# apache/datafusion-comet

Measured on AMD Instinct MI355X. Metric: rows/sec, TPC-H SF100 Q1 scan->filter->agg (HBM-resident Arrow columns), higher is better.
Workload: dtype i128 (Decimal128; 256-bit products) / i32 (Date32) / u8 (Utf8 keys); 1 GPU; TPC-H SF100 Q1 stage 1 (Filter -> Project, 3 decimal ops incl. one 256-bit multiply -> partial HashAggregate, 2 Utf8 keys, 8 aggregates) per GPU; rows_per_gpu=600037902, bytes_per_row_algorithmic=78, parallelism=row-range shards x1, jit_toolchain=hiprtc 9.0; comgr 3.0 /opt/rocm/lib/libamd_comgr.so.3

## Files before the change

### datafusion-comet_amd/csrc/codegen.hpp

```cpp
#pragma once
#include <map>
#include <memory>
#include <string>
#include <vector>

#include "plan.hpp"

namespace comet {

enum class SinkKind { Output, AggNoGroup, AggGrouped };

struct OutCol {
  DType type;
  bool nullable = true;
  bool packed_string = false;
  int gather_src = -1;
  int view_src = -1;
  enum FmtKind { FmtNone = 0, FmtInt = 1, FmtBool = 2, FmtDecimal = 3, FmtDecimalJava = 4, FmtDate = 5, FmtTimestamp = 6, FmtFloat64 = 7, FmtFloat32 = 8 };
  int fmt_kind = FmtNone;
  long long fmt_arg = 0;
  std::vector<int> concat_cols;
  std::vector<std::string> concat_lits;
  int case_mode = 0;
  std::string pad_pattern;
  bool pad_left = false;
};

struct DerivedCol {
  int kind = 0;
  int op = 0;
  std::string arg_a, arg_b;
  long long arg_k = 0;
  int columns() const { return kind == 3 ? 1 : 2; }
  int src = -1;
  std::vector<uint32_t> prog;
  std::vector<uint32_t> prog2;
  int limit = -1;
  DType type;
};

struct PipelineDesc {
  SinkKind sink = SinkKind::Output;
  bool has_filter = false;
  int R = 4;
  int NW = 0;
  int NK = 0;
  int NPW = 0;
  int lds_cap = 0;
  std::vector<DType> in_types;
  std::vector<DerivedCol> derived;
  std::vector<bool> in_used;
  std::vector<OutCol> out_cols;
  std::vector<std::pair<uint32_t, std::shared_ptr<QueryContext>>> site_contexts;
  std::shared_ptr<QueryContext> agg_ctx[2];
  bool agg_ctx_mixed[2] = {false, false}, agg_ctx_seen[2] = {false, false};
  struct BloomRef { ExprP node; int64_t subquery_id = -1; };
  std::vector<BloomRef> blooms;
  std::string source;
  std::vector<std::string> kernels;
  long long max_rows_exact = 0;
  int sort_key_bytes = 0;
  std::vector<int> sort_str_cols;
  bool join_build_only = false;
  bool join_outer_build = false;
  bool join_dedup_build = false;
  std::string explain;
  std::vector<std::string> op_names;
  std::vector<int> str_key_cols;
  struct FixSum { int word = 0; int aux_hi = 0, aux_lo = 0; };
  std::vector<FixSum> fix_sums;
  bool merges_states = false;
};
constexpr int kFixScaleArg = 6;
constexpr int kFixScaleArg2 = 4;
constexpr int kRowBaseArg = 3;
constexpr int kFixMaxSums = 8;
constexpr int kFixW = 158;
constexpr int kFixDefaultScale = -94;

PipelineDesc generate_pipeline(const Operator& root, const std::vector<bool>& in_has_validity,
                               const std::vector<DType>* source_types = nullptr, const std::vector<int>* str_fixed_len = nullptr,
                               const std::vector<int>* dict_id_col = nullptr);

PipelineDesc generate_sort_keys(const Operator& sort, const std::vector<DType>& types, const std::vector<bool>& has_validity);
ExprP bound(int idx, const DType& t);
ExprP shift_bound(const ExprP& e, int by, int from = 0);
struct JoinFusion {
  std::vector<DType> src_types;
  std::vector<bool> src_valid;
  std::vector<ExprP> cols;
  std::vector<ExprP> preds;
};
PipelineDesc generate_join(const Operator& join, const std::vector<DType>& left_types, const std::vector<DType>& right_types,
                           const std::vector<bool>& left_has_validity, const std::vector<bool>& right_has_validity,
                           const JoinFusion* probe_fusion = nullptr, const JoinFusion* build_fusion = nullptr);
void fold_chain(const Operator& top, const Operator& source, const std::vector<DType>& source_types, std::vector<ExprP>& cols, std::vector<ExprP>& preds);

constexpr int kOutPartials = 0;
constexpr int kOutCounts = 1;
constexpr int kOutErr = 2;
constexpr int kErrBytes = 512;
constexpr int kErrAuxWords = 22;
constexpr int kErrDetailWord = 24;
constexpr int kErrDetailStrBytes = 224;

struct ErrSite {
  enum Value : int { Unscaled128 = 0, Int64 = 1, F64 = 2, F32 = 3, Str = 4, DecimalBD = 5, F64Display = 6, Int64Plain = 7, NoValue = 8, F64Micros = 9, FunctionName = 10, IndexAndSize = 11 };
  std::string error_type;
  std::string error_class;
  std::string from_type, to_type;
  int precision = 0, scale = 0;
  int value = Unscaled128;
  std::string suffix;
};
uint32_t register_err_site(const ErrSite& s, int ordinal = 0);
bool lookup_err_site(uint32_t id, ErrSite& out);
std::string err_site_json(const ErrSite& s, uint64_t lo, uint64_t hi, const uint8_t* str, size_t str_avail, const QueryContext* ctx = nullptr);
std::string decimal_sum_overflow_json(int kind, const QueryContext* ctx);
void bloom_check_bytes(const uint8_t* p, size_t len);
constexpr int kOutFirstCol = 4;

}
```

### datafusion-comet_amd/csrc/device/comet_device.hpp

```cpp
#pragma once
#ifndef __HIPCC_RTC__
#include <hip/hip_runtime.h>
#endif
#include "kparams.h"

#ifndef STRFN
#define STRFN __device__ inline
#endif
#include "strfn.hpp"

template <class P>
__device__ bool rx_search(const unsigned int* w, P text, int n, int from, int& m0, int& m1);

namespace comet {

typedef long long i64;
typedef unsigned long long u64;
typedef int i32;
typedef unsigned int u32;
typedef short i16;
typedef unsigned short u16;
typedef signed char i8;
typedef unsigned char u8;
typedef __int128 i128;
// ... 1869 lines not shown

template <int NK, int NPW>
struct LSlot {
  u32 state;
  u32 ord;
  u64 key[NK];
  u64 acc[NPW];
  u64 pad[((1 + NK + NPW) % 2 == 0) ? 1 : 0];
};

template <class P>
struct GroupCtx {
  COMET_LDS LSlot<P::NK, P::NPW>* lds;
  COMET_LDS u32* lds_count;
  COMET_LDS u32* ord_slot;
  COMET_LDS u64* priv;
  Slot<P::NK, P::NW>* glb;
  u64 glb_cap;
  unsigned int* err;
  int part_mode = 0;
  COMET_LDS u32* part = nullptr;
  u64* recs = nullptr;
  u32 np = 0;
  mutable u32 inserted = 0;
  CDEV u32* counter() const { return &inserted; }
  CDEV bool table_full() const { return (__hip_atomic_load(err, __ATOMIC_RELAXED, __HIP_MEMORY_SCOPE_AGENT) & 32u) != 0; }
  CDEV void set_full() const { if (!table_full()) atomicOr(err, 32u); }
};

CDEV void flush_inserted(unsigned int* err, u32 inserted) {
  u32 v = inserted;
#pragma unroll
  for (int m = 32; m >= 1; m >>= 1) v += __shfl_xor(v, m, kWave);
  if (lane_id() == 0 && v) atomicAdd((unsigned long long*)err + 1, (unsigned long long)v);
}
constexpr u64 kMaxGlobalProbes = 128;
constexpr u32 kNoOrdinal = 0xffffffffu;

template <class P>
struct SlotInit {
  CDEV void operator()(u64* acc) const { P::init(acc); }
};

template <class P>
CDEV void lds_word_apply(COMET_LDS u64* w, int k, u64 v) {
  switch (P::pop(k)) {
    case G_ADD64: if (v) __hip_atomic_fetch_add(w, v, __ATOMIC_RELAXED, __HIP_MEMORY_SCOPE_WORKGROUP); break;
    case G_UMAX64: if (v) __hip_atomic_fetch_max(w, v, __ATOMIC_RELAXED, __HIP_MEMORY_SCOPE_WORKGROUP); break;
    case G_OR64: if (v) __hip_atomic_fetch_or(w, v, __ATOMIC_RELAXED, __HIP_MEMORY_SCOPE_WORKGROUP); break;
    case G_AND64: if (~v) __hip_atomic_fetch_and(w, v, __ATOMIC_RELAXED, __HIP_MEMORY_SCOPE_WORKGROUP); break;
    case G_XOR64: if (v) atomic_xor64<__HIP_MEMORY_SCOPE_WORKGROUP>(w, v); break;
    case G_IMIN64: __hip_atomic_fetch_min((COMET_LDS i64*)w, (i64)v, __ATOMIC_RELAXED, __HIP_MEMORY_SCOPE_WORKGROUP); break;
    case G_IMAX64: __hip_atomic_fetch_max((COMET_LDS i64*)w, (i64)v, __ATOMIC_RELAXED, __HIP_MEMORY_SCOPE_WORKGROUP); break;
    case G_FADD64: __hip_atomic_fetch_add((COMET_LDS double*)w, __longlong_as_double((i64)v), __ATOMIC_RELAXED, __HIP_MEMORY_SCOPE_WORKGROUP); break;
    default: break;
  }
}
template <class P>
CDEV u64 pword_combine(int k, u64 a, u64 b) {
  switch (P::pop(k)) {
    case G_ADD64: return a + b;
    case G_UMAX64: return a > b ? a : b;
    case G_OR64: return a | b;
    case G_AND64: return a & b;
    case G_XOR64: return a ^ b;
    case G_IMIN64: return (i64)b < (i64)a ? b : a;
    case G_IMAX64: return (i64)b > (i64)a ? b : a;
    case G_FADD64: return (u64)__double_as_longlong(fp_add(__longlong_as_double((i64)a), __longlong_as_double((i64)b)));
    default: return a;
  }
}

template <class P>
CDEV COMET_LDS LSlot<P::NK, P::NPW>* lds_find_or_insert(const GroupCtx<P>& g, const u64* key, u32& ordinal) {
  typedef COMET_LDS LSlot<P::NK, P::NPW> S;
  u32 h = (u32)hash_key<P::NK>(key) & (u32)(P::LDS_CAP - 1);
  for (int probes = 0; probes < 16;) {
    S* s = g.lds + h;
    u32 st = __hip_atomic_load(&s->state, __ATOMIC_RELAXED, __HIP_MEMORY_SCOPE_WORKGROUP);
    if (st == kSlotEmpty) {
      u32 expected = kSlotEmpty;
      if (__hip_atomic_compare_exchange_strong(&s->state, &expected, kSlotBusy, __ATOMIC_RELAXED, __ATOMIC_RELAXED,
                                               __HIP_MEMORY_SCOPE_WORKGROUP)) {
#pragma unroll
        for (int k = 0; k < P::NK; k++) s->key[k] = key[k];
#pragma unroll
        for (int k = 0; k < P::NPW; k++) s->acc[k] = P::pidentity(k);
        u32 ord = __hip_atomic_fetch_add(g.lds_count, 1u, __ATOMIC_RELAXED, __HIP_MEMORY_SCOPE_WORKGROUP);
        s->ord = ord;
        if (ord < (u32)P::GC) g.ord_slot[ord] = h;
        __hip_atomic_store(&s->state, kSlotReady, __ATOMIC_RELEASE, __HIP_MEMORY_SCOPE_WORKGROUP);
        ordinal = ord;
        return s;
      }
      continue;
    }
    if (st == kSlotBusy) continue;
    bool eq = true;
#pragma unroll
    for (int k = 0; k < P::NK; k++) eq &= (s->key[k] == key[k]);
    if (eq) {
      ordinal = s->ord;
      return s;
    }
    h = (h + 1) & (u32)(P::LDS_CAP - 1);
    probes++;
  }
  ordinal = kNoOrdinal;
  return nullptr;
}

template <class P>
CDEV void group_update(const GroupCtx<P>& g, bool active, const u64* key, const u64* pv) {
  if (!active) return;
  if (g.part_mode) {
    const u32 p = (u32)__umul64hi(hash_key<P::NK>(key), (u64)g.np);
    if (g.part_mode == 1) {
      __hip_atomic_fetch_add(g.part + p, 1u, __ATOMIC_RELAXED, __HIP_MEMORY_SCOPE_WORKGROUP);
      return;
    }
    u64 val[P::NW];
    P::fold(pv, val);
    const u32 pos = __hip_atomic_fetch_add(g.part + p, 1u, __ATOMIC_RELAXED, __HIP_MEMORY_SCOPE_WORKGROUP);
    u64* rec = g.recs + (u64)pos * (u64)(P::NK + P::NW);
#pragma unroll
    for (int k = 0; k < P::NK; k++) rec[k] = key[k];
#pragma unroll
    for (int k = 0; k < P::NW; k++) rec[P::NK + k] = val[k];
    return;
  }
  u32 ord = kNoOrdinal;
  COMET_LDS LSlot<P::NK, P::NPW>* ls = nullptr;
  if (P::LDS_CAP > 0) ls = lds_find_or_insert<P>(g, key, ord);
  if (ord < (u32)P::GC) {
    COMET_LDS u64* base = g.priv + (u32)(ord * P::NPW) * P::COPIES + (threadIdx.x & (P::COPIES - 1));
#pragma unroll
    for (int k = 0; k < P::NPW; k++) lds_word_apply<P>(base + k * P::COPIES, k, pv[k]);
    return;
  }
  if (ls) {
#pragma unroll
    for (int k = 0; k < P::NPW; k++) lds_word_apply<P>(&ls->acc[k], k, pv[k]);
    return;
  }
  if (g.table_full()) return;
  u64 val[P::NW];
  P::fold(pv, val);
  bool fresh = false;
  Slot<P::NK, P::NW>* s = table_find_or_insert<P::NK, P::NW>(g.glb, g.glb_cap, key, SlotInitWith<P>{val}, kMaxGlobalProbes, g.counter(), &fresh);
  if (!s) { g.set_full(); return; }
  if (!fresh) slot_apply<P, __HIP_MEMORY_SCOPE_AGENT>(&s->acc[0], val);
}

template <class P>
CDEV void agg_grouped_body(const CometKParams& prm) {
  typedef Slot<P::NK, P::NW> S;
  typedef LSlot<P::NK, P::NPW> LS;
  __shared__ LS s_tbl[P::LDS_CAP > 0 ? P::LDS_CAP : 1];
  __shared__ u64 s_priv[P::GC * P::NPW * P::COPIES];
  __shared__ u32 s_count;
  __shared__ u32 s_ord_slot[P::GC];
  if (P::LDS_CAP > 0) {
    for (int i = threadIdx.x; i < P::LDS_CAP; i += kBlock) s_tbl[i].state = kSlotEmpty;
  }
  for (int i = threadIdx.x; i < P::GC * P::NPW * P::COPIES; i += kBlock) s_priv[i] = P::pidentity((i / P::COPIES) % P::NPW);
  if (threadIdx.x == 0) s_count = 0;
  __syncthreads();
  GroupCtx<P> g;
  g.lds = (COMET_LDS LS*)s_tbl;
  g.lds_count = (COMET_LDS u32*)&s_count;
  g.ord_slot = (COMET_LDS u32*)s_ord_slot;
  g.priv = (COMET_LDS u64*)s_priv;
  g.glb = (S*)prm.out[0];
  g.glb_cap = (u64)prm.iarg[0];
  g.err = (unsigned int*)prm.out[2];
  u64 kacc[P::NKW > 0 ? P::NKW : 1];
  P::kinit(kacc);
  const i64 n = prm.n;
  const i64 tile = (i64)P::R * kBlock;
  const i64 stride = (i64)gridDim.x * tile;
  if constexpr (P::PIPELINED) {
    typename P::L cur, nxt;
    i64 base = (i64)blockIdx.x * tile;
    if (base < n) P::tile_load(prm, base, n, cur);
    for (u32 it = 0; base < n; base += stride, it++) {
      if (base + stride < n) P::tile_load(prm, base + stride, n, nxt);
      P::tile_grouped(prm, base, n, cur, g, kacc);
      cur = nxt;
      if ((it < 8 || (it & 7) == 7) && g.table_full()) break;
    }
  } else {
    u32 it = 0;
    for (i64 base = (i64)blockIdx.x * tile; base < n; base += stride, it++) {
      P::tile_grouped(prm, base, n, g, kacc);
      if ((it < 8 || (it & 7) == 7) && g.table_full()) break;
    }
  }
  __syncthreads();
  const u32 ngrp = s_count < (u32)P::GC ? s_count : (u32)P::GC;
  for (u32 t = threadIdx.x; t < ngrp * P::NPW; t += kBlock) {
    const u32 gi = t / P::NPW, k = t % P::NPW;
    u64 a = P::pidentity(k);
    for (int c = 0; c < P::COPIES; c++) a = pword_combine<P>(k, a, s_priv[(gi * P::NPW + k) * P::COPIES + c]);
    LS* ls = &s_tbl[s_ord_slot[gi]];
    ls->acc[k] = pword_combine<P>(k, ls->acc[k], a);
  }
  __syncthreads();
  for (int i = threadIdx.x; i < P::LDS_CAP; i += kBlock) {
    LS* ls = &s_tbl[i];
    if (ls->state == kSlotReady) {
      u64 key[P::NK], pw[P::NPW], val[P::NW];
#pragma unroll
      for (int k = 0; k < P::NK; k++) key[k] = ls->key[k];
#pragma unroll
      for (int k = 0; k < P::NPW; k++) pw[k] = ls->acc[k];
      P::fold(pw, val);
      bool fresh = false;
      S* gs = g.table_full() ? nullptr : table_find_or_insert<P::NK, P::NW>(g.glb, g.glb_cap, key, SlotInitWith<P>{val}, kMaxGlobalProbes, g.counter(), &fresh);
      if (!gs) g.set_full();
      else if (!fresh) slot_apply<P, __HIP_MEMORY_SCOPE_AGENT>(&gs->acc[0], val);
    }
  }
  flush_inserted(g.err, g.inserted);
  if (P::NKW > 0) {
#pragma unroll
    for (int m = 32; m >= 1; m >>= 1) {
#pragma unroll
      for (int k = 0; k < P::NKW; k++) {
        u64 o = shfl_xor_u64(kacc[k], m);
        kacc[k] = P::kop(k) == G_UMAX64 ? (o > kacc[k] ? o : kacc[k]) : (kacc[k] | o);
      }
    }
    if (lane_id() == 0) {
      unsigned long long* aux = (unsigned long long*)prm.out[2] + 2;
#pragma unroll
      for (int k = 0; k < P::NKW; k++) {
        if (P::kop(k) == G_UMAX64) atomicMax(aux + k, (unsigned long long)kacc[k]);
        else atomicOr(aux + k, (unsigned long long)kacc[k]);
      }
    }
  }
}


constexpr int kJoinPartMax = 16384;
constexpr int kJoinPartTotOff = kJoinPartMax + 16;
constexpr int kJoinPartCntOff = 2 * kJoinPartMax + 16;
template <class P>
struct AggPart {
  static constexpr int kSlotBytes = 8 + 8 * (P::NK + P::NW);
  static constexpr int kCap = kSlotBytes <= 48 ? 1024 : kSlotBytes <= 96 ? 512 : kSlotBytes <= 192 ? 256 : 128;
};

template <class P>
CDEV void agg_publish_kacc(const CometKParams& prm, u64* kacc) {
  if (P::NKW > 0) {
#pragma unroll
    for (int m = 32; m >= 1; m >>= 1) {
#pragma unroll
      for (int k = 0; k < P::NKW; k++) {
        u64 o = shfl_xor_u64(kacc[k], m);
        kacc[k] = P::kop(k) == G_UMAX64 ? (o > kacc[k] ? o : kacc[k]) : (kacc[k] | o);
      }
    }
    if (lane_id() == 0) {
      unsigned long long* aux = (unsigned long long*)prm.out[2] + 2;
#pragma unroll
      for (int k = 0; k < P::NKW; k++) {
        if (P::kop(k) == G_UMAX64) atomicMax(aux + k, (unsigned long long)kacc[k]);
        else atomicOr(aux + k, (unsigned long long)kacc[k]);
      }
    }
  }
}

template <class P, int MODE>
CDEV void agg_part_pass_body(const CometKParams& prm) {
  __shared__ u32 s_part[kJoinPartMax];
  __shared__ u32 s_wsum[kBlock / kWave];
  __shared__ u32 s_carry;
  const i64 n = prm.n, chunk = prm.iarg[5];
  const int np = (int)prm.iarg[2];
  u32* pstart = (u32*)prm.out[3];
  u32* cnt = pstart + kJoinPartCntOff + (i64)blockIdx.x * np;
  if (MODE == 1) {
    for (int p = threadIdx.x; p < np; p += kBlock) s_part[p] = 0;
  } else {
    const u32* tot = pstart + kJoinPartTotOff;
    if (threadIdx.x == 0) s_carry = 0;
    __syncthreads();
    for (int b0 = 0; b0 < np; b0 += kBlock) {
      const int p = b0 + (int)threadIdx.x;
      const u32 v = p < np ? tot[p] : 0u;
      u32 x = v;
#pragma unroll
      for (int d = 1; d < kWave; d <<= 1) {
        const u32 y = __shfl_up(x, d, kWave);
        if (lane_id() >= d) x += y;
      }
      if (lane_id() == kWave - 1) s_wsum[wave_id()] = x;
      __syncthreads();
      u32 excl = s_carry + x - v;
      for (int w = 0; w < wave_id(); w++) excl += s_wsum[w];
      if (p < np) {
        s_part[p] = excl + cnt[p];
        if (blockIdx.x == 0) pstart[p] = excl;
      }
      __syncthreads();
      if (threadIdx.x == kBlock - 1) s_carry = excl + v;
      __syncthreads();
// ... 1142 lines not shown
```

### datafusion-comet_amd/csrc/exec.cpp

```cpp
#include "exec.hpp"
#include "shuffle_format.hpp"

#include <cerrno>
#include <fcntl.h>
#include <unistd.h>
#include <chrono>
#include <condition_variable>
#include <cstdio>
#include <cstdlib>
#include <cmath>
#include <cstring>
#include <functional>
#include <map>
#include <mutex>

#include "exec_internal.hpp"

namespace comet {

static bool list_of_flat(const DType& t) { return t.id == TypeId::List && t.kids.size() == 1 && !t.kids[0].is_nested(); }
DevTable extend_struct_fields(const DevTable& in) {
  bool any = false;
  for (auto& t : in.types) any |= t.id == TypeId::Struct || list_of_flat(t);
  if (!any) return in;
// ... 652 lines not shown
        btypes.push_back(st[(size_t)col]);
      }
      std::vector<bool> none(st.size(), false), bnone(btypes.size(), true);
      PipelineDesc d1 = generate_sort_keys(so, st, none), d2 = generate_sort_keys(sb, btypes, bnone);
      if (d1.sort_key_bytes != d2.sort_key_bytes) throw CometError("internal: range boundary keys and row keys differ in width");
      if (compile_in_infer_) { jit_compile(d1.source); jit_compile(d2.source); }
    }
    explain_ += "  shuffle writer: " + std::to_string(op.shuffle_num_partitions) + " partition(s), codec " + std::to_string(op.shuffle_codec) + "\n";
    return {};
  }
  if (is_bloom_agg(op)) {
    if (op.children.size() != 1) throw CometError("HashAggregate expects exactly one child");
    const BloomAggSpec spec = bloom_agg_spec(op);
    std::vector<DType> st = infer_schema(*op.children[0]);
    if (op.agg_mode == AggMode::Partial) {
      auto sc = std::make_shared<Operator>();
      sc->kind = OpKind::Scan;
      sc->proto_tag = 100;
      sc->scan_fields = st;
      auto pr = std::make_shared<Operator>();
      pr->kind = OpKind::Projection;
      pr->proto_tag = 101;
      pr->children.push_back(sc);
      pr->project_list = op.agg_exprs[0].children;
      node_id_[pr.get()] = (int)node_id_.size();
      std::vector<DType> ext = extend_struct_field_types(st);
      std::vector<bool> none(ext.size(), false);
      PipelineDesc d = generate_pipeline(*pr, none, &ext);
      const DType& ct = d.out_cols.at(0).type;
      if (ct.id == TypeId::String || ct.id == TypeId::Bytes)
        throw CometError("bloom_filter_agg over a " + ct.str() + " child is not supported by the MI355X native engine: might_contain probes longs only, such a filter could not be used natively");
      if (!ct.is_integer()) throw CometError("bloom_filter_agg over " + ct.str() + " is not supported (Byte, Short, Int and Long are)");
      if (compile_in_infer_) jit_compile(d.source);
      explain_ += d.explain;
      bloom_proj_[&op] = pr;
    } else {
      const size_t sc = (size_t)std::max(0, op.initial_input_buffer_offset);
      if (sc >= st.size() || st[sc].id != TypeId::Bytes)
        throw CometError("bloom_filter_agg: the merging aggregate expects its Binary state in column " + std::to_string(sc) + " of its child");
    }
    explain_ += std::string("  bloom_filter_agg (") + (op.agg_mode == AggMode::Partial ? "Partial" : op.agg_mode == AggMode::Final ? "Final" : "PartialMerge") + "): V" +
                std::to_string(spec.version) + ", " + std::to_string(spec.k) + " hash function(s), " + std::to_string(spec.num_words * 64) + " bits\n";
    return {DType::of(TypeId::Bytes)};
  }
  if (op.kind == OpKind::NativeScan) {
    std::vector<DType> out;
    for (auto& f : op.required_schema) out.push_back(f.dtype);
    for (auto& f : op.partition_schema) out.push_back(f.dtype);
    explain_ += "  parquet scan: " + std::to_string(op.files.size()) + " file(s), " + std::to_string(out.size()) + " column(s)\n";
    return out;
  }
  if (op.kind == OpKind::HashJoin) {
    if (op.children.size() != 2) throw CometError("HashJoin expects two children");
    const size_t pi = op.build_side == BuildSide::Left ? 1 : 0;
    std::vector<DType> l, r;
    PipelineDesc d;
    bool fused = false;
    if (pi == 1) {
      l = infer_schema(*op.children[0]);
      fused = plan_fused_probe(op, l, d);
      if (!fused) r = infer_schema(*op.children[1]);
    } else {
      const std::string before = explain_;
      explain_.clear();
      r = infer_schema(*op.children[1]);
      const std::string right_explain = explain_;
      explain_ = before;
      fused = plan_fused_probe(op, r, d);
      if (!fused) l = infer_schema(*op.children[0]);
      explain_ += right_explain;
    }
    if (!fused) {
      std::vector<bool> lv(l.size(), false), rv(r.size(), false);
      FusedProbe fb;
      bool with_build = plan_fused_build(op, fb);
      if (with_build) {
        try {
          d = generate_join(op, l, r, lv, rv, nullptr, &fb.fu);
          fused_build_[&op] = fb;
        } catch (const CometError&) {
          with_build = false;
        }
      }
      if (!with_build) d = generate_join(op, l, r, lv, rv);
    }
    if (compile_in_infer_) jit_compile(d.source);
    explain_ += d.explain;
    if (fused) {
      const size_t nbuild = pi == 1 ? l.size() : r.size();
      std::vector<DType> probe_types;
      const size_t nprobe = fused_probe_.at(&op).fu.cols.size();
      if (d.out_cols.size() == nbuild + nprobe) {
        for (size_t c = 0; c < nprobe; c++) probe_types.push_back(d.out_cols[(pi == 1 ? nbuild : 0) + c].type);
      } else {
        probe_types.assign(nprobe, DType());
        if (pi == 0) for (size_t c = 0; c < nprobe && c < d.out_cols.size(); c++) probe_types[c] = d.out_cols[c].type;
      }
      (pi == 1 ? r : l) = probe_types;
    }
    if (op.smj) {
      Operator& so = *smj_sorts_.at(&op);
      so.sort_orders.clear();
      const bool by_right = op.join_type == JoinType::RightOuter;
      const std::vector<ExprP>& keys = by_right ? op.right_keys : op.left_keys;
      std::function<ExprP(const ExprP&)> shift = [&](const ExprP& e) -> ExprP {
        auto n = std::make_shared<Expr>(*e);
        if (e->kind == ExprKind::Bound) n->bound_index = e->bound_index + (int)l.size();
        for (auto& c : n->children) c = shift(c);
        return n;
      };
      for (size_t k = 0; k < keys.size(); k++) {
        Operator::SortKey sk;
        sk.child = by_right ? shift(keys[k]) : keys[k];
        if (k < op.smj_sort_options.size()) { sk.descending = op.smj_sort_options[k].first; sk.nulls_last = op.smj_sort_options[k].second; }
        so.sort_orders.push_back(sk);
      }
      explain_ += "  (sort-merge join: output ordered by the join keys)\n";
    }
    std::vector<DType> out;
    for (auto& c : d.out_cols) out.push_back(c.type);
    return out;
  }
  const Operator* src = &op;
  do {
    if (src->children.size() != 1) throw CometError(std::string(op_name(src->proto_tag)) + " expects exactly one child");
    src = src->children[0].get();
  } while (!is_source(*src, &op));
  std::vector<DType> st = extend_struct_field_types(infer_schema(*src));
  std::vector<bool> none(st.size(), false);
  PipelineDesc d = generate_pipeline(op, none, &st);
  if (compile_in_infer_) jit_compile(d.source);
  explain_ += d.explain;
  std::vector<DType> out;
  for (auto& c : d.out_cols) { out.push_back(c.type); out.back().virt_parent = out.back().virt_kid = -1; }
  return out;
}

ExecutionContext::~ExecutionContext() {
  mem_->owner = std::this_thread::get_id();
  for (auto& in : inputs_) {
    if (in.host && in.host->release) in.host->release(in.host);
    if (in.dev && in.dev->release) in.dev->release(in.dev);
  }
  for (auto& st : staging_)
    if (st && st->busy) {
      (void)hipEventSynchronize(st->busy);
      pool_put_event(device_id_, st->busy);
      st->busy = nullptr;
    }
  if (stream_) {
    (void)hipStreamSynchronize(stream_);
    for (auto& pr : timed_) { pool_put_event(device_id_, pr.first); pool_put_event(device_id_, pr.second); }
    for (hipEvent_t& e : aux_ev_) if (e) { pool_put_event(device_id_, e); e = nullptr; }
    for (auto& p : kt_pending_) { pool_put_event(device_id_, p.a); pool_put_event(device_id_, p.b); }
    kt_pending_.clear();
    pool_put_stream(device_id_, stream_);
  }
}

const std::string& ExecutionContext::explain() { return explain_; }

std::string ExecutionContext::check_only(OperatorP plan, uint64_t plan_hash) {
  size_t nscan = 0;
  std::function<void(const Operator&)> cnt = [&](const Operator& op) {
    if (op.kind == OpKind::Scan) nscan++;
    for (auto& c : op.children) cnt(*c);
  };
  cnt(*plan);
  std::vector<InputSource> ins(nscan);
  ExecutionContext ctx(plan, plan_hash, {}, ins, 8192, 0);
  return ctx.explain_;
}

PipelineDesc ExecutionContext::join_codegen(OperatorP plan, uint64_t plan_hash, const std::vector<bool>& has_valid) {
  const Operator& op = *plan;
  const Operator* leaf[2] = {nullptr, nullptr};
  for (size_t s = 0; s < 2 && op.kind == OpKind::HashJoin && op.children.size() == 2; s++) {
    const Operator* c = op.children[s].get();
    while ((c->kind == OpKind::Filter || c->kind == OpKind::Projection) && c->children.size() == 1) c = c->children[0].get();
    if (c->kind == OpKind::Scan) leaf[s] = c;
  }
  if (!leaf[0] || !leaf[1]) throw CometError("comet_plan_codegen: a HashJoin over two Scan leaves, or Filter / Projection chains over them, is expected");
  std::vector<InputSource> ins(2);
  ExecutionContext ctx(plan, plan_hash, {}, ins, 8192, 0);
  auto fit = ctx.fused_probe_.find(&op);
  auto fbit = ctx.fused_build_.find(&op);
  const bool build_left = op.build_side == BuildSide::Left;
  std::vector<DType> types[2];
  std::vector<bool> valid[2];
  size_t first = 0;
  for (size_t s = 0; s < 2; s++) {
    std::vector<bool> hv(leaf[s]->scan_fields.size(), false);
    for (size_t k = 0; k < hv.size(); k++) hv[k] = first + k < has_valid.size() && has_valid[first + k];
    first += hv.size();
    const bool is_build = (s == 0) == build_left;
    const bool fused = is_build ? fbit != ctx.fused_build_.end() : fit != ctx.fused_probe_.end();
    if (fused || op.children[s].get() == leaf[s]) {
      types[s] = leaf[s]->scan_fields;
      valid[s] = hv;
    } else {
      const PipelineDesc cd = generate_pipeline(*op.children[s], hv);
      for (auto& oc : cd.out_cols) {
        types[s].push_back(oc.type);
        valid[s].push_back(oc.nullable);
      }
    }
  }
  JoinFusion fu, fub;
  if (fit != ctx.fused_probe_.end()) { fu = fit->second.fu; fu.src_valid = valid[build_left ? 1 : 0]; }
  if (fbit != ctx.fused_build_.end()) { fub = fbit->second.fu; fub.src_valid = valid[build_left ? 0 : 1]; }
  return generate_join(op, types[0], types[1], valid[0], valid[1], fit != ctx.fused_probe_.end() ? &fu : nullptr, fbit != ctx.fused_build_.end() ? &fub : nullptr);
}

std::string ExecutionContext::compile_only(OperatorP plan, uint64_t plan_hash) {
  size_t nscan = 0;
  std::function<void(const Operator&)> cnt = [&](const Operator& op) {
    if (op.kind == OpKind::Scan) nscan++;
    for (auto& c : op.children) cnt(*c);
  };
  cnt(*plan);
  std::vector<InputSource> ins(nscan);
  ExecutionContext ctx(plan, plan_hash, {}, ins, 8192, 0);
  std::vector<bool> none(ctx.in_types_.size(), false);
  if (ctx.has_join_) {
    ctx.compile_in_infer_ = true;
    ctx.explain_.clear();
    ctx.infer_schema(*ctx.root_source_);
    if (ctx.plan_.get() != ctx.root_source_) {
      auto pv = planned_variant(*ctx.plan_, ctx.plan_hash_, none, true, &ctx.in_types_);
      ctx.explain_ += pv->desc.explain;
    }
  } else {
    planned_variant(*ctx.plan_, ctx.plan_hash_, none, true);
  }
  return ctx.explain_;
}

Variant ExecutionContext::node_variant(const Operator& node, const char* tag, const std::string& validity, const std::function<PipelineDesc()>& generate) {
  const std::string key = std::to_string(plan_hash_ ^ (0x9E3779B97F4A7C15ull * (uint64_t)(node_id_[&node] + 1))) + tag + validity;
  std::shared_ptr<PlannedVariant> pv;
  {
    std::lock_guard<std::mutex> lk(g_plan_mu);
    auto it = g_plan_cache.find(key);
    if (it != g_plan_cache.end()) pv = it->second;
  }
  if (!pv) {
    pv = std::make_shared<PlannedVariant>();
    pv->desc = generate();
    pv->code = jit_compile(pv->desc.source);
    std::lock_guard<std::mutex> lk(g_plan_mu);
    g_plan_cache[key] = pv;
  }
  Variant v;
  v.desc = pv->desc;
  note_sites(v.desc);
  v.mod = jit_load(pv->code);
  return v;
}

Variant& ExecutionContext::variant_for(const std::vector<bool>& has_valid, const std::vector<int>& str_fixed_len) {
  std::string key = validity_key(has_valid) + ":";
  bool any_fixed = false;
  for (int l : str_fixed_len) { key += std::to_string(l) + ","; any_fixed |= l >= 0; }
  auto it = variants_.find(key);
  if (it != variants_.end()) return it->second;
  auto pv = planned_variant(*plan_, plan_hash_, has_valid, true, has_join_ ? &in_types_ : nullptr, any_fixed ? &str_fixed_len : nullptr,
                            dict_id_col_.empty() ? nullptr : &dict_id_col_);
  Variant v;
  v.desc = pv->desc;
  note_sites(v.desc);
  v.mod = jit_load(pv->code);
  auto res = variants_.emplace(key, std::move(v));
  return res.first->second;
}

void ExecutionContext::launch(Variant& v, const char* kernel, int grid, CometKParams& prm, int block) {
  hipFunction_t fn = v.mod->fn(kernel);
  if (!v.desc.blooms.empty()) bind_blooms(v.desc, prm);
  void* args[] = {&prm};
  if (!g_kernel_times.load(std::memory_order_relaxed)) {
    HIP_CHECK(hipModuleLaunchKernel(fn, (unsigned)grid, 1, 1, (unsigned)block, 1, 1, 0, stream_, args, nullptr));
    return;
  }
  hipEvent_t a = pool_get_event(device_id_), b = pool_get_event(device_id_);
  HIP_CHECK(hipEventRecord(a, stream_));
  HIP_CHECK(hipModuleLaunchKernel(fn, (unsigned)grid, 1, 1, (unsigned)block, 1, 1, 0, stream_, args, nullptr));
  HIP_CHECK(hipEventRecord(b, stream_));
  kt_pending_.push_back({kernel, a, b});
}

std::atomic<int> g_kernel_times{getenv("COMET_KERNEL_TIMES") != nullptr && atoi(getenv("COMET_KERNEL_TIMES")) != 0 ? 1 : 0};

std::string ExecutionContext::kernel_times_json() {
  if (!kt_pending_.empty()) {
    HIP_CHECK(hipStreamSynchronize(stream_));
    for (auto& p : kt_pending_) {
      float ms = 0;
      if (hipEventElapsedTime(&ms, p.a, p.b) == hipSuccess) { kernel_times_[p.name].first += ms; kernel_times_[p.name].second++; }
      pool_put_event(device_id_, p.a);
      pool_put_event(device_id_, p.b);
    }
    kt_pending_.clear();
  }
  std::string s = "{";
  for (auto& kv : kernel_times_) {
    char buf[160];
// ... 384 lines not shown

void ExecutionContext::extend_derived(DevTable& in, const std::vector<DerivedCol>& derived) {
  for (const DerivedCol& dc : derived) {
    if (dc.kind == 3) { extend_derived_strfn(in, dc); continue; }
    if ((dc.kind != 1 && dc.kind != 2) || dc.src < 0 || (size_t)dc.src >= in.cols.size()) throw CometError("internal: unknown derived column");
    const DeviceColumnView sc = in.cols[(size_t)dc.src];
    const bool hv = in.has_valid[(size_t)dc.src];
    const int64_t rows = in.rows;
    if (!sc.data && rows) throw CometError("split over a Utf8 column without offsets is not supported");
    if (hv && sc.offset != 0) throw CometError("split over a sliced Utf8 column with NULLs is not supported yet");
    DevBuf prog, counts, tiles;
    auto list_offs = std::make_shared<DevBuf>();
    prog.ensure(dc.prog.size() * 4 + 16);
    HIP_CHECK(hipMemcpyAsync(prog.p, dc.prog.data(), dc.prog.size() * 4, hipMemcpyHostToDevice, stream_));
    DevBuf prog_group;
    const uint32_t* prog2 = nullptr;
    if (dc.kind == 2) {
      if (dc.prog2.empty()) prog2 = (const uint32_t*)prog.p;
      else {
        prog_group.ensure(dc.prog2.size() * 4 + 16);
        HIP_CHECK(hipMemcpyAsync(prog_group.p, dc.prog2.data(), dc.prog2.size() * 4, hipMemcpyHostToDevice, stream_));
        prog2 = (const uint32_t*)prog_group.p;
      }
    }
    HIP_CHECK(hipStreamSynchronize(stream_));
    counts.ensure((size_t)std::max<int64_t>(rows, 1) * 4 + 16);
    tiles.ensure((size_t)((rows + 1023) / 1024 + 2) * 8);
    list_offs->ensure((size_t)(rows + 2) * 4);
    HIP_CHECK(hipMemsetAsync(list_offs->p, 0, 8, stream_));
    const int32_t* offs = (const int32_t*)sc.data + sc.offset;
    const uint8_t* vbits = hv ? sc.valid : nullptr;
    if (comet_launch_split_count(offs, (const uint8_t*)sc.aux, vbits, sc.offset, rows, (const uint32_t*)prog.p, prog2, dc.limit, (uint32_t*)counts.p, stream_) != 0) throw CometError("split: launch failed");
    if (rows) pq_launch_u32_scan((const uint32_t*)counts.p, rows, (uint64_t*)tiles.p, (int32_t*)list_offs->p, stream_);
    int32_t total = 0;
    if (rows) read_small(&total, (char*)list_offs->p + (size_t)rows * 4, 4);
    if (total < 0) throw CometError("split: more than 2^31 pieces in one table");
    DevBuf views, lengths, etiles;
    auto eoffs = std::make_shared<DevBuf>(), ebytes = std::make_shared<DevBuf>();
    views.ensure((size_t)std::max<int32_t>(total, 1) * 16 + 16);
    lengths.ensure((size_t)std::max<int32_t>(total, 1) * 4 + 16);
    etiles.ensure((size_t)((total + 1023) / 1024 + 2) * 8);
    eoffs->ensure((size_t)(total + 2) * 4);
    HIP_CHECK(hipMemsetAsync(eoffs->p, 0, 8, stream_));
    if (comet_launch_split_write(offs, (const uint8_t*)sc.aux, vbits, sc.offset, rows, (const uint32_t*)prog.p, prog2, dc.limit, (const int32_t*)list_offs->p, views.p, stream_) != 0)
      throw CometError("split: launch failed");
    if (comet_launch_strview_lengths(views.p, nullptr, total, nullptr, 0, (uint32_t*)lengths.p, stream_) != 0) throw CometError("split: launch failed");
    if (total) pq_launch_u32_scan((const uint32_t*)lengths.p, total, (uint64_t*)etiles.p, (int32_t*)eoffs->p, stream_);
    int32_t nbytes = 0;
    if (total) read_small(&nbytes, (char*)eoffs->p + (size_t)total * 4, 4);
    if (nbytes < 0) throw CometError("Utf8 column exceeds 2 GiB of string data (LargeUtf8 is not supported)");
    ebytes->ensure((size_t)nbytes + 16);
    if (comet_launch_strview_copy(views.p, nullptr, offs, (const uint8_t*)sc.aux, total, nullptr, 0, 0, (const int32_t*)eoffs->p, (uint8_t*)ebytes->p, stream_) != 0)
      throw CometError("split: launch failed");
    HIP_CHECK(hipStreamSynchronize(stream_));
    DeviceColumnView elem;
    elem.data = eoffs->p;
    elem.aux = ebytes->p;
    DeviceColumnView lv;
    lv.data = list_offs->p;
    lv.valid = sc.valid;
    lv.offset = 0;
    lv.kids.push_back(elem);
    lv.kid_has_valid.push_back(false);
    lv.kid_rows = total;
    in.types.push_back(dc.type);
    in.cols.push_back(lv);
    in.has_valid.push_back(hv);
    DType et = dc.type.kids[0];
    et.virt_parent = (int)in.types.size() - 1;
    et.virt_kid = 0;
    in.types.push_back(et);
    in.cols.push_back(elem);
    in.has_valid.push_back(false);
    in.owners.push_back(list_offs);
    in.owners.push_back(eoffs);
    in.owners.push_back(ebytes);
    split_rows_ += rows;
  }
}


DevTable ExecutionContext::run_chain_to_device(const Operator& top, const DevTable& in_plain) {
  DevTable in = extend_struct_fields(in_plain);
  if (in.cols.size() > COMET_MAX_IN) throw CometError("too many columns (struct fields included) for one GPU pipeline");
  auto pv = planned_variant(top, plan_hash_ ^ (0x9E3779B97F4A7C15ull * (uint64_t)(node_id_[&top] + 1)), in.has_valid, true, &in.types);
  if (pv->desc.sink != SinkKind::Output) throw CometError("internal: run_chain_to_device on an aggregate chain");
  extend_derived(in, pv->desc.derived);
  if (in.cols.size() > COMET_MAX_IN) throw CometError("too many columns (derived columns included) for one GPU pipeline");
  Variant v;
  v.desc = pv->desc;
  note_sites(v.desc);
  v.mod = jit_load(pv->code);
  const PipelineDesc& d = v.desc;
  const int64_t n = in.rows;
  CometKParams prm;
  memset(&prm, 0, sizeof prm);
  prm.n = n;
  bind_inputs(prm, in.cols, in.has_valid);
  prm.out[kOutErr] = err_flags_.p;
  const size_t ncol = d.out_cols.size();
  std::vector<std::shared_ptr<DevBuf>> vals(ncol), vbytes(ncol);
  auto bind = [&](int64_t cap) {
    for (size_t j = 0; j < ncol; j++) {
      vals[j] = std::make_shared<DevBuf>();
      vals[j]->ensure((size_t)cap * out_width(d.out_cols[j]) + 16);
      prm.out[kOutFirstCol + 2 * j] = vals[j]->p;
      vbytes[j] = std::make_shared<DevBuf>();
      if (d.out_cols[j].nullable) {
        vbytes[j]->ensure((size_t)cap + 16);
        prm.out[kOutFirstCol + 2 * j + 1] = vbytes[j]->p;
      }
    }
  };
  int64_t out_rows = n;
  timed_begin();
  if (n == 0) {
    bind(1);
    out_rows = 0;
  } else if (d.has_filter) {
    bind(n);
    out_rows = launch_fused_filter(v, prm, n);
  } else {
    bind(n);
    launch(v, "k_emit", (int)std::min<int64_t>((n + 255) / 256, 256 * 8), prm);
  }
  timed_end();
  DevTable out = outputs_to_table(v, vals, vbytes, out_rows, [&](int c) { return std::make_pair(&in, c); });
  out.owners.push_back(v.mod);
  return out;
}

DevTable ExecutionContext::materialize(const Operator& op) {
  static const bool trace = getenv("COMET_TRACE_STAGES") != nullptr;
  Timer tm;
  struct Report {
    const Operator& op; Timer& tm; bool on;
    ~Report() { if (on) fprintf(stderr, "[comet] materialize %s: %.3f ms (incl. children)\n", op_name(op.proto_tag), tm.ns() / 1e6); }
  } report{op, tm, trace};
  if (op.kind == OpKind::Scan) {
    const size_t input = scan_input_.at(&op);
    DevTable t;
    t.types = op.scan_fields;
    if (inputs_[input].kind == 0) {
      int64_t rows = 0;
      if (pull_host_table(input, op.scan_fields, INT64_MAX, t.cols, t.has_valid, rows)) t.rows = rows;
      if (t.cols.empty()) {
        t.cols.assign(op.scan_fields.size(), DeviceColumnView());
        t.has_valid.assign(op.scan_fields.size(), false);
      }
      HIP_CHECK(hipStreamSynchronize(stream_));
    } else {
      std::shared_ptr<void> keep;
      int64_t rows = 0;
      if (pull_device_table(input, op.scan_fields, t.cols, t.has_valid, rows, keep)) {
        t.rows = rows;
        t.owners.push_back(keep);
        std::vector<DeviceColumnView> c2;
        std::vector<bool> v2;
        std::shared_ptr<void> k2;
        int64_t r2 = 0;
        if (pull_device_table(input, op.scan_fields, c2, v2, r2, k2) && r2 > 0)
          throw CometError("a device input stream feeding a join must deliver a single batch");
      } else {
        t.cols.assign(op.scan_fields.size(), DeviceColumnView());
        t.has_valid.assign(op.scan_fields.size(), false);
      }
    }
    input_rows += t.rows;
    return t;
  }
  if (op.kind == OpKind::NativeScan) {
    DevTable t = scan_parquet(op);
    input_rows += t.rows;
    return t;
  }
  if (op.kind == OpKind::HashJoin) {
    auto fit = fused_probe_.find(&op);
    auto fbit = fused_build_.find(&op);
    DevTable j;
    if (fit != fused_probe_.end() || fbit != fused_build_.end()) {
      const bool build_left = op.build_side == BuildSide::Left;
      const bool fb_on = fbit != fused_build_.end(), fp_on = fit != fused_probe_.end();
      DevTable b = materialize(fb_on ? *fbit->second.source : *op.children[build_left ? 0 : 1]);
      DevTable s = materialize(fp_on ? *fit->second.source : *op.children[build_left ? 1 : 0]);
      JoinFusion fu, fub;
      if (fp_on) { fu = fit->second.fu; fu.src_valid = s.has_valid; }
      if (fb_on) { fub = fbit->second.fu; fub.src_valid = b.has_valid; join_fused_builds_++; }
      const char* sfx = fp_on && fb_on ? ":FB" : fp_on ? ":F" : ":B";
      j = build_left ? hash_join_impl(op, op, b, s, sfx, fp_on ? &fu : nullptr, fb_on ? &fub : nullptr) : hash_join_impl(op, op, s, b, sfx, fp_on ? &fu : nullptr, fb_on ? &fub : nullptr);
    } else {
      DevTable l = materialize(*op.children[0]);
      DevTable r = materialize(*op.children[1]);
      j = hash_join(op, l, r);
    }
    if (!op.smj || !smj_needs_sort_.count(&op)) return j;
    return sort_table(*smj_sorts_.at(&op), j);
  }
  if (op.kind == OpKind::Sort) {
    DevTable in = materialize(*op.children[0]);
    return sort_table(op, in);
  }
  if (op.kind == OpKind::Limit) {
    DevTable in = materialize(*op.children[0]);
    const int64_t off = std::min<int64_t>(std::max(0, op.offset), in.rows);
    const int64_t end = op.limit < 0 ? in.rows : std::min<int64_t>(in.rows, op.limit);
    return take_rows(in, nullptr, off, std::max<int64_t>(0, end - off), nullptr);
  }
  if (op.kind == OpKind::ShuffleWriter) return write_shuffle(op);
  if (op.kind == OpKind::Expand) {
    DevTable in = materialize(*op.children[0]);
    return expand(op, in);
  }
  if (op.kind == OpKind::Explode) {
    DevTable in = materialize(*op.children[0]);
    return explode(op, in);
  }
  if (op.kind == OpKind::Window) {
    DevTable in = materialize(*op.children[0]);
    return window(op, in);
  }
  if (is_bloom_agg(op)) {
    DevTable in = materialize(*op.children[0]);
    return bloom_aggregate(op, in);
  }
  if (op.kind == OpKind::HashAgg) return nested_aggregate(op);
  const Operator* src = &op;
  do src = src->children[0].get(); while (!is_source(*src, &op));
  DevTable in = materialize(*src);
  DevTable out = run_chain_to_device(op, in);
  HIP_CHECK(hipStreamSynchronize(stream_));
  return out;
}



DevTable ExecutionContext::nested_aggregate(const Operator& agg) {
  std::vector<size_t> idx;
  std::function<void(const Operator&)> walk = [&](const Operator& op) {
    if (op.kind == OpKind::Scan) idx.push_back(scan_input_.at(&op));
    for (auto& c : op.children) walk(*c);
  };
  walk(agg);
  std::vector<InputSource> sub_inputs;
  for (size_t i : idx) {
    sub_inputs.push_back(inputs_[i]);
    inputs_[i].host = nullptr;
    inputs_[i].dev = nullptr;
    inputs_[i].exhausted = true;
  }
  OperatorP sub_plan(const_cast<Operator*>(&agg), [](Operator*) {});
  static const bool trace = getenv("COMET_TRACE_STAGES") != nullptr;
  Timer tm;
  auto mark = [&](const char* what) { if (trace) fprintf(stderr, "[comet] nested aggregate: %s at %.3f ms\n", what, tm.ns() / 1e6); };
  auto subp = std::make_unique<ExecutionContext>(sub_plan, plan_hash_ ^ (0x9E3779B97F4A7C15ull * (uint64_t)(node_id_[&agg] + 1)), config_, sub_inputs, 0, device_id_);
  ExecutionContext& sub = *subp;
  struct Gone { std::unique_ptr<ExecutionContext>& p; decltype(mark)& m; ~Gone() { p.reset(); m("context released"); } } gone{subp, mark};
  mark("context built");
  if (sub.sink_ != SinkKind::AggGrouped && sub.sink_ != SinkKind::AggNoGroup) throw CometError("internal: nested aggregate without an aggregate sink");
  sub.device_result_ = true;
  sub.blooms_ = blooms_;
  sub.start();
  mark("started");
  sub.run_to_completion();
  mark("input consumed");
  DevTable t;
  if (sub.sink_ == SinkKind::AggNoGroup) {
    sub.finish_aggregate();
    if (sub.ready_.empty()) throw CometError("internal: ungrouped aggregate produced no row");
    t = host_batch_to_table(sub.ready_.front());
    sub.ready_.clear();
  } else {
    t = sub.grouped_to_device();
  }
  mark("groups emitted");
  input_rows += sub.input_rows;
  part_merges_ += sub.part_merges_;
  sub.collect_timings();
  last_kernel_ms += sub.last_kernel_ms;
  last_kernel_launches += sub.last_kernel_launches;
  if (!sub.kt_pending_.empty() || !sub.kernel_times_.empty()) {
    sub.kernel_times_json();
    for (auto& kv : sub.kernel_times_) { kernel_times_[kv.first].first += kv.second.first; kernel_times_[kv.first].second += kv.second.second; }
  }
  return t;
}

DevTable ExecutionContext::host_batch_to_table(const HostBatch& b) {
  DevTable t;
  t.rows = b.rows;
  auto up = [&](const std::vector<uint8_t>& v) -> const void* {
    auto d = std::make_shared<DevBuf>();
    d->ensure(v.size() + 16);
    if (!v.empty()) HIP_CHECK(hipMemcpy(d->p, v.data(), v.size(), hipMemcpyHostToDevice));
    t.owners.push_back(d);
    return d->p;
  };
  for (const HostColumn& c : b.cols) {
    DeviceColumnView v;
    v.data = up(c.values);
    const bool is_str = c.type.id == TypeId::String || c.type.id == TypeId::Bytes;
    if (is_str) v.aux = up(c.data);
    const bool hv = c.null_count > 0 && !c.validity.empty();
    if (hv) v.valid = (const uint8_t*)up(c.validity);
    t.types.push_back(c.type);
    t.cols.push_back(v);
    t.has_valid.push_back(hv);
  }
// ... 28 lines not shown
  } else if (t.id == TypeId::Bool) {
    fetch(c.values, v.data, (size_t)((rows + 7) / 8));
  } else {
    fetch(c.values, v.data, (size_t)rows * (size_t)fixed_width(t));
  }
  HIP_CHECK(hipStreamSynchronize(st));
  if (!c.validity.empty()) {
    int64_t nulls = 0;
    for (int64_t i = 0; i < rows; i++) nulls += !((c.validity[(size_t)(i >> 3)] >> (i & 7)) & 1);
    c.null_count = nulls;
    if (!nulls) c.validity.clear();
  }
  return c;
}
namespace {
std::vector<uint8_t> slice_bits(const std::vector<uint8_t>& b, int64_t off, int64_t len) {
  std::vector<uint8_t> o((size_t)((len + 7) / 8), 0);
  for (int64_t i = 0; i < len; i++)
    if ((b[(size_t)((off + i) >> 3)] >> ((off + i) & 7)) & 1) o[(size_t)(i >> 3)] |= (uint8_t)(1u << (i & 7));
  return o;
}
HostColumn slice_column(const HostColumn& c, int64_t off, int64_t len) {
  if (off == 0 && len == c.length) return c;
  HostColumn o;
  o.type = c.type;
  o.length = len;
  if (!c.validity.empty()) {
    o.validity = slice_bits(c.validity, off, len);
    for (int64_t i = 0; i < len; i++) o.null_count += !((o.validity[(size_t)(i >> 3)] >> (i & 7)) & 1);
    if (!o.null_count) o.validity.clear();
  }
  const TypeId id = c.type.id;
  if (id == TypeId::Struct) {
    for (auto& k : c.children) o.children.push_back(slice_column(k, off, len));
  } else if (id == TypeId::List || id == TypeId::Map || id == TypeId::String || id == TypeId::Bytes) {
    const int32_t* src = (const int32_t*)c.values.data();
    o.values.resize((size_t)(len + 1) * 4);
    int32_t* w = (int32_t*)o.values.data();
    for (int64_t i = 0; i <= len; i++) w[i] = src[off + i] - src[off];
    if (id == TypeId::List || id == TypeId::Map) o.children.push_back(slice_column(c.children.at(0), src[off], src[off + len] - src[off]));
    else o.data.assign(c.data.begin() + src[off], c.data.begin() + src[off + len]);
  } else if (id == TypeId::Bool) {
    o.values = slice_bits(c.values, off, len);
  } else {
    const size_t w = (size_t)fixed_width(c.type);
    o.values.assign(c.values.begin() + (size_t)off * w, c.values.begin() + (size_t)(off + len) * w);
  }
  return o;
}
}

void ExecutionContext::table_to_host_batches(const DevTable& t) {
  if (t.rows == 0) return;
  const size_t ncol = t.cols.size();
  std::vector<HostColumn> nested(ncol);
  for (size_t j = 0; j < ncol; j++)
    if (t.types[j].is_nested()) nested[j] = download_column(t.cols[j], t.types[j], t.has_valid[j], t.rows, stream_);
  std::vector<std::vector<uint8_t>> hv(ncol), hb(ncol);
  std::vector<std::vector<uint8_t>> hd(ncol);
  struct Piece { const void* src; std::vector<uint8_t>* dst; size_t bytes; };
  auto fetch = [&](std::vector<Piece>& pieces) {
    size_t total = 0, longest = 0;
    for (auto& pc : pieces) { pc.dst->resize(pc.bytes); total += (pc.bytes + 15) & ~(size_t)15; longest = std::max(longest, pc.bytes); }
    if (pieces.empty()) return;
    static const bool batched = getenv("COMET_EXPORT_BATCHED") == nullptr || atoi(getenv("COMET_EXPORT_BATCHED")) != 0;
    if (batched && total > 0 && total <= ((size_t)1 << 20) && pieces.size() <= 256) {
      struct Desc { const uint8_t* src; uint8_t* dst; uint64_t len; };
      const size_t head = (pieces.size() * sizeof(Desc) + 63) & ~(size_t)63;
      export_host_.ensure(head + total + 64);
      Desc* d = (Desc*)export_host_.p;
      size_t at = head;
      for (size_t k = 0; k < pieces.size(); k++) {
        d[k].src = (const uint8_t*)pieces[k].src;
        d[k].dst = (uint8_t*)export_host_.p + at;
        d[k].len = pieces[k].bytes;
        at += (pieces[k].bytes + 15) & ~(size_t)15;
      }
      if (comet_launch_copy_small(export_host_.p, (int)pieces.size(), (uint64_t)longest, stream_) != 0) throw CometError("result export: launch failed");
      HIP_CHECK(hipStreamSynchronize(stream_));
      for (size_t k = 0; k < pieces.size(); k++)
        if (pieces[k].bytes) memcpy(pieces[k].dst->data(), d[k].dst, pieces[k].bytes);
      return;
    }
    for (auto& pc : pieces)
      if (pc.bytes) HIP_CHECK(hipMemcpyAsync(pc.dst->data(), pc.src, pc.bytes, hipMemcpyDeviceToHost, stream_));
    HIP_CHECK(hipStreamSynchronize(stream_));
  };
  std::vector<Piece> pieces;
  for (size_t j = 0; j < ncol; j++) {
    const DType& ty = t.types[j];
    if (ty.is_nested()) continue;
    const bool is_str = ty.id == TypeId::String || ty.id == TypeId::Bytes;
    size_t bytes = is_str ? (size_t)(t.rows + 1) * 4 : ty.id == TypeId::Bool ? (size_t)((t.rows + 7) / 8) : (size_t)t.rows * fixed_width(ty);
    pieces.push_back({t.cols[j].data, &hv[j], bytes});
    if (t.has_valid[j]) pieces.push_back({t.cols[j].valid, &hb[j], (size_t)((t.rows + 7) / 8)});
  }
  fetch(pieces);
  pieces.clear();
  for (size_t j = 0; j < ncol; j++) {
    if (t.types[j].id == TypeId::String || t.types[j].id == TypeId::Bytes) {
      const int32_t* offs = (const int32_t*)hv[j].data();
      if (offs[t.rows] > 0) pieces.push_back({t.cols[j].aux, &hd[j], (size_t)offs[t.rows]});
    }
  }
  fetch(pieces);
  check_device_errors();
  const int64_t bs = batch_size_ > 0 ? batch_size_ : t.rows;
  auto getbit = [](const std::vector<uint8_t>& b, int64_t i) { return (b[(size_t)(i >> 3)] >> (i & 7)) & 1; };
  for (int64_t off = 0; off < t.rows; off += bs) {
    const int64_t len = std::min(bs, t.rows - off);
    HostBatch b;
    b.rows = len;
    for (size_t j = 0; j < ncol; j++) {
      if (t.types[j].is_nested()) { b.cols.push_back(slice_column(nested[j], off, len)); continue; }
      HostColumn c;
      c.type = t.types[j];
      c.length = len;
      if (c.type.id == TypeId::String || c.type.id == TypeId::Bytes) {
        const int32_t* offs = (const int32_t*)hv[j].data();
        c.values.resize((size_t)(len + 1) * 4);
        int32_t* o = (int32_t*)c.values.data();
        for (int64_t i = 0; i <= len; i++) o[i] = offs[off + i] - offs[off];
        c.data.assign(hd[j].begin() + offs[off], hd[j].begin() + offs[off + len]);
      } else if (c.type.id == TypeId::Bool) {
        c.values.assign((size_t)((len + 7) / 8), 0);
        for (int64_t i = 0; i < len; i++)
          if (getbit(hv[j], off + i)) c.values[(size_t)(i >> 3)] |= (uint8_t)(1u << (i & 7));
      } else {
        int w = fixed_width(c.type);
        c.values.assign(hv[j].begin() + (size_t)off * w, hv[j].begin() + (size_t)(off + len) * w);
      }
      if (t.has_valid[j]) {
        int64_t nulls = 0;
        std::vector<uint8_t> bm((size_t)((len + 7) / 8), 0);
        for (int64_t i = 0; i < len; i++) {
          if (getbit(hb[j], off + i)) bm[(size_t)(i >> 3)] |= (uint8_t)(1u << (i & 7));
          else nulls++;
        }
        c.null_count = nulls;
        if (nulls) c.validity = std::move(bm);
      }
      b.cols.push_back(std::move(c));
    }
    ready_.push_back(std::move(b));
  }
}

void ExecutionContext::run_to_completion() {
  if (has_join_) {
    DevTable src = extend_struct_fields(materialize(*root_source_));
    if (plan_.get() == root_source_) throw CometError("internal: bare join root");
    if (sink_ == SinkKind::AggGrouped) prepare_dict_keys(src);
    single_chunk_hint_ = true;
    process_chunk(src.cols, src.has_valid, src.rows);
    HIP_CHECK(hipStreamSynchronize(stream_));
    return;
  }
  while (true) {
    bool more = inputs_[0].kind == 0 ? pull_host_chunk() : pull_device_batch();
    if (!more) break;
  }
}

void ExecutionContext::start() {
  if (!started_) {
    HIP_CHECK(hipSetDevice(device_id_));
    stream_ = pool_get_stream(device_id_);
    err_flags_.ensure(kErrBytes);
    HIP_CHECK(hipMemsetAsync(err_flags_.p, 0, kErrBytes, stream_));
    started_ = true;
  } else {
    HIP_CHECK(hipSetDevice(device_id_));
  }
}

namespace {
struct ExportedDeviceColumn {
  std::vector<std::shared_ptr<void>> owners;
  const void* buffers[3];
};
void release_device_array(ArrowArray* a) {
  delete (ExportedDeviceColumn*)a->private_data;
  a->release = nullptr;
}
void release_fmt_schema(ArrowSchema* s) {
  delete (std::string*)s->private_data;
  s->release = nullptr;
}
}

void ExecutionContext::set_memory_manager(int64_t (*acquire)(void*, int64_t), void (*release)(void*, int64_t), void* ctx, long long task_id) {
  mem_->acquire = acquire;
  mem_->release = release;
  mem_->ctx = ctx;
  mem_->task_id = task_id;
}
void ExecutionContext::memory_stats(int64_t out[4]) {
  out[0] = mem_->host_used.load();
  out[1] = mem_->host_peak.load();
  out[2] = mem_->dev_used.load();
  out[3] = mem_->dev_peak.load();
}

int64_t ExecutionContext::execute_device(ArrowDeviceArray** out_arrays, ArrowSchema** out_schemas, int n_out) {
  mem_->owner = std::this_thread::get_id();
  AccountScope account(mem_);
  mem_->flush();
  Timer t;
  start();
  if (sink_ == SinkKind::AggNoGroup)
    throw CometError("comet_execute_plan_device: an ungrouped aggregate result is one row and is exported through comet_execute_plan");
  if (finished_) return -1;
  DevTable tab;
  if (sink_ == SinkKind::AggGrouped) {
    device_result_ = true;
    run_to_completion();
    tab = grouped_to_device();
  } else {
    tab = materialize(*plan_);
  }
  HIP_CHECK(hipStreamSynchronize(stream_));
  check_device_errors();
  collect_timings();
  finished_ = true;
  if ((size_t)n_out != tab.cols.size())
    throw CometError("Output column count mismatch: expected " + std::to_string(n_out) + ", got " + std::to_string(tab.cols.size()));
  for (size_t c = 0; c < tab.types.size(); c++)
    if (tab.types[c].is_nested()) throw CometError("executePlan (device arrays): nested column of type " + tab.types[c].str() + " — nested results are exported through host batches");
  for (int j = 0; j < n_out; j++) {
    const DType& ty = tab.types[(size_t)j];
    const bool is_str = ty.id == TypeId::String || ty.id == TypeId::Bytes;
    if (tab.cols[(size_t)j].offset != 0) throw CometError("comet_execute_plan_device: input column with a non-zero Arrow offset passed through");
    auto* ec = new ExportedDeviceColumn();
    ec->owners = tab.owners;
    ec->buffers[0] = tab.has_valid[(size_t)j] ? tab.cols[(size_t)j].valid : nullptr;
    ec->buffers[1] = tab.cols[(size_t)j].data;
    ec->buffers[2] = is_str ? tab.cols[(size_t)j].aux : nullptr;
    ArrowDeviceArray* d = out_arrays[j];
    memset(d, 0, sizeof *d);
    d->array.length = tab.rows;
    d->array.null_count = tab.has_valid[(size_t)j] ? -1 : 0;
    d->array.n_buffers = is_str ? 3 : 2;
    d->array.buffers = ec->buffers;
    d->array.private_data = ec;
    d->array.release = release_device_array;
    d->device_id = device_id_;
    d->device_type = ARROW_DEVICE_ROCM;
    d->sync_event = nullptr;
    ArrowSchema* s = out_schemas[j];
    memset(s, 0, sizeof *s);
    auto* fmt = new std::string(expected_format(ty));
    s->format = fmt->c_str();
    s->name = "";
    s->flags = ARROW_FLAG_NULLABLE;
    s->private_data = fmt;
    s->release = release_fmt_schema;
  }
  output_rows_ += tab.rows;
  elapsed_compute_ns_ += t.ns();
  return tab.rows;
}

void ExecutionContext::resolve_subqueries() {
  if (subqueries_resolved_) return;
  subqueries_resolved_ = true;
  uint64_t sig = 0xcbf29ce484222325ull;
  auto mix = [&](const void* p, size_t n) { for (size_t k = 0; k < n; k++) sig = (sig ^ ((const uint8_t*)p)[k]) * 0x100000001b3ull; };
  for (auto& e : plan_->subqueries) {
    if (e->kind != ExprKind::Subquery) continue;
    const int64_t id = e->lit_i64;
    bool is_null = true;
    std::string v;
    bool found = false;
    auto it = subquery_values_.find(id);
    if (it != subquery_values_.end()) { is_null = it->second.first; v = it->second.second; found = true; }
    else if (subquery_provider_) found = subquery_provider_(id, e->dtype, is_null, v);
    if (!found) throw CometError("Subquery " + std::to_string(id) + " is not registered with this plan (CometScalarSubquery.setSubquery / comet_plan_set_subquery)");
    auto need = [&](size_t n) { if (!is_null && v.size() < n) throw CometError("Subquery " + std::to_string(id) + ": the value has " + std::to_string(v.size()) + " bytes, its type needs " + std::to_string(n)); };
    e->kind = ExprKind::Literal;
    e->proto_tag = 2;
    e->lit_null = is_null;
    e->lit_i64 = 0;
    int64_t i = 0;
    double d = 0;
    switch (e->dtype.id) {
      case TypeId::Bool: need(1); e->lit_bool = !is_null && v[0] != 0; e->lit_case = 1; break;
      case TypeId::Int8: case TypeId::Int16: case TypeId::Int32: case TypeId::Date: case TypeId::Int64: case TypeId::Timestamp: case TypeId::TimestampNtz:
        need(8);
        if (!is_null) memcpy(&i, v.data(), 8);
        e->lit_i64 = i;
        e->lit_case = e->dtype.id == TypeId::Int8 ? 2 : e->dtype.id == TypeId::Int16 ? 3 : (e->dtype.id == TypeId::Int32 || e->dtype.id == TypeId::Date) ? 4 : 5;
        break;
      case TypeId::Float: case TypeId::Double:
        need(8);
        if (!is_null) memcpy(&d, v.data(), 8);
        e->lit_f64 = e->dtype.id == TypeId::Float ? (double)(float)d : d;
        e->lit_case = e->dtype.id == TypeId::Float ? 6 : 7;
        break;
      case TypeId::Decimal: e->lit_dec = is_null ? 0 : decode_decimal_be(v); e->lit_case = 10; break;
      case TypeId::String: case TypeId::Bytes: e->lit_bytes = is_null ? std::string() : v; e->lit_case = e->dtype.id == TypeId::String ? 8 : 9; break;
      default: throw CometError("Unsupported scalar subquery data type " + e->dtype.str());
    }
    mix(&id, 8);
    mix(&is_null, 1);
    if (e->bloom_arg) {
      if (e->dtype.id != TypeId::Bytes) throw CometError("might_contain: the bloom filter subquery must be Binary, got " + e->dtype.str());
      if (!is_null) bloom_check_bytes((const uint8_t*)e->lit_bytes.data(), e->lit_bytes.size());
      if (!blooms_) blooms_ = std::make_shared<BloomRegistry>();
      blooms_->subquery_nodes[id] = e;
      continue;
    }
    mix(v.data(), v.size());
  }
  if (!plan_->subqueries.empty()) plan_hash_ ^= sig * 0x9E3779B97F4A7C15ull;
}

int64_t ExecutionContext::execute(ArrowArray** out_arrays, ArrowSchema** out_schemas, int n_out) {
  mem_->owner = std::this_thread::get_id();
  if (!subqueries_resolved_) resolve_subqueries();
  AccountScope account(mem_);
  mem_->flush();
// ... 73 lines not shown
```

### datafusion-comet_amd/csrc/exec.hpp

```cpp
#pragma once
#include <mutex>
#include <thread>
#include <atomic>
#include <hip/hip_runtime_api.h>

#include <deque>
#include <functional>
#include <map>
#include <set>
#include <memory>
#include <string>
#include <vector>

#include "arrow_abi.hpp"
#include "codegen.hpp"
#include "jit.hpp"
#include "kparams.h"
#include "plan.hpp"

namespace comet {
double process_clock_ms();

struct MemAccount {
  int64_t (*acquire)(void* ctx, int64_t bytes) = nullptr;
  void (*release)(void* ctx, int64_t bytes) = nullptr;
  void* ctx = nullptr;
  long long task_id = 0;
  int64_t dev_limit = 0;
  std::atomic<int64_t> host_used{0}, host_peak{0}, dev_used{0}, dev_peak{0}, pending_release{0};
  std::thread::id owner;
  void grow_host(int64_t n);
  void shrink_host(int64_t n);
  void grow_dev(int64_t n);
  void shrink_dev(int64_t n);
  void flush();
  void detach();
  std::mutex cb_mu;
  bool detached = false;
};
struct AccountScope {
  std::shared_ptr<MemAccount> prev;
  explicit AccountScope(std::shared_ptr<MemAccount> a);
  ~AccountScope();
};

struct DevBuf {
  void* p = nullptr;
  size_t cap = 0;
  int dev = 0;
  std::shared_ptr<MemAccount> acct;
  void ensure(size_t n);
  void release();
  ~DevBuf() { release(); }
  DevBuf() = default;
  DevBuf(const DevBuf&) = delete;
  DevBuf& operator=(const DevBuf&) = delete;
};
struct PinnedBuf {
  void* p = nullptr;
  size_t cap = 0;
  std::shared_ptr<MemAccount> acct;
  void ensure(size_t n);
  void release();
  ~PinnedBuf() { release(); }
  PinnedBuf() = default;
  PinnedBuf(const PinnedBuf&) = delete;
  PinnedBuf& operator=(const PinnedBuf&) = delete;
};

struct HostColumn {
  DType type;
  int64_t length = 0;
  int64_t null_count = 0;
  std::vector<uint8_t> validity;
  std::vector<uint8_t> values;
  std::vector<uint8_t> data;
  std::vector<HostColumn> children;
};
struct HostBatch {
  int64_t rows = 0;
  std::vector<HostColumn> cols;
};

struct InputSource {
  int kind = 0;
  ArrowArrayStream* host = nullptr;
  ArrowDeviceArrayStream* dev = nullptr;
  bool exhausted = false;
};

struct DeviceColumnView {
  const void* data = nullptr;
  const uint8_t* valid = nullptr;
  const void* aux = nullptr;
  int64_t offset = 0;
  int fixed_len = -1;
  std::vector<DeviceColumnView> kids;
  std::vector<char> kid_has_valid;
  int64_t kid_rows = 0;
};

struct DevTable {
  int64_t rows = 0;
  std::vector<DType> types;
  std::vector<DeviceColumnView> cols;
  std::vector<bool> has_valid;
  std::vector<std::shared_ptr<void>> owners;
};

struct Staging {
  std::vector<std::unique_ptr<PinnedBuf>> stage_vals, stage_valid, stage_aux;
  std::vector<std::unique_ptr<DevBuf>> dev_vals, dev_valid, dev_aux;
  std::vector<int> dict_index_width;
  std::vector<std::shared_ptr<void>> nested_keep;
  hipEvent_t busy = nullptr;
};

struct Variant {
  PipelineDesc desc;
  std::shared_ptr<LoadedModule> mod;
};

struct BloomAggSpec { int version = 1, k = 1; int64_t num_words = 0; };
BloomAggSpec bloom_agg_spec(const Operator& hash_agg);
bool is_bloom_agg(const Operator& op);
struct BloomRegistry {
  std::map<int64_t, ExprP> subquery_nodes;
  std::map<const Expr*, std::shared_ptr<struct DevBuf>> buffers;
  std::vector<ExprP> keep;
};

void scan_pool_parallel(size_t n, const std::function<void(size_t)>& fn);
std::string parquet_prune_report(const Operator& native_scan, bool page_index, bool bloom_filters = true);
std::vector<uint8_t> parquet_host_plain_values(const Operator& native_scan, size_t column);
void scan_pool_submit(std::function<void()> fn);

extern std::atomic<int> g_kernel_times;

class ExecutionContext {
 public:
  ExecutionContext(OperatorP plan, uint64_t plan_hash, std::vector<std::pair<std::string, std::string>> config,
                   std::vector<InputSource> inputs, int batch_size, int device_id);
  ~ExecutionContext();

  int64_t execute(ArrowArray** out_arrays, ArrowSchema** out_schemas, int n_out);
  int64_t execute_device(ArrowDeviceArray** out_arrays, ArrowSchema** out_schemas, int n_out);
  std::string metrics_proto();
  void set_memory_manager(int64_t (*acquire)(void*, int64_t), void (*release)(void*, int64_t), void* ctx, long long task_id);
  typedef std::function<bool(int64_t id, const DType& type, bool& is_null, std::string& value)> SubqueryProvider;
  void set_subquery_provider(SubqueryProvider p) { subquery_provider_ = std::move(p); }
  void set_subquery_value(int64_t id, bool is_null, std::string value) { subquery_values_[id] = {is_null, std::move(value)}; }
  void resolve_subqueries();
  void memory_stats(int64_t out[4]);
  std::shared_ptr<MemAccount> memory_account() const { return mem_; }
  const std::string& explain();
  static std::string compile_only(OperatorP plan, uint64_t plan_hash);
  static std::string check_only(OperatorP plan, uint64_t plan_hash);
  static PipelineDesc join_codegen(OperatorP plan, uint64_t plan_hash, const std::vector<bool>& has_valid);

  std::string last_error;
  int last_error_kind = 0;

  double last_kernel_ms = 0;
  int64_t last_kernel_launches = 0;
  std::string kernel_times_json();
  double last_aux_ms = 0;
  int64_t last_aux_launches = 0;
  int64_t input_rows = 0;

 private:
  void run_to_completion();
  void start();
  std::vector<std::vector<int>> fixed_len_hint_;
  Variant& variant_for(const std::vector<bool>& has_valid, const std::vector<int>& str_fixed_len);
  void process_chunk(const std::vector<DeviceColumnView>& cols, const std::vector<bool>& has_valid, int64_t n);
  void finish_aggregate();
  void finish_grouped();
  DevTable grouped_to_device();
  std::vector<DType> infer_schema(const Operator& op);
  DevTable materialize(const Operator& op);
  DevTable scan_parquet(const Operator& native_scan);
  friend struct ParquetScan;
  friend struct HashJoinRun;
  int64_t launch_fused_filter(Variant& v, CometKParams& prm, int64_t n);
  DevTable run_chain_to_device(const Operator& top, const DevTable& in);
  void extend_derived(DevTable& in, const std::vector<DerivedCol>& derived);
  void extend_derived_strfn(DevTable& in, const DerivedCol& dc);
  DevTable hash_join(const Operator& j, const DevTable& l, const DevTable& r);
  DevTable hash_join_impl(const Operator& node, const Operator& j, const DevTable& l, const DevTable& r, const std::string& key_suffix,
                          const JoinFusion* fused_probe = nullptr, const JoinFusion* fused_build = nullptr);
  struct FusedProbe { const Operator* source = nullptr; JoinFusion fu; };
  bool plan_fused_probe(const Operator& join, const std::vector<DType>& build_types, PipelineDesc& desc);
  bool plan_fused_build(const Operator& join, FusedProbe& fb);
  DevTable sort_table(const Operator& s, const DevTable& in);
  Variant node_variant(const Operator& node, const char* tag, const std::string& validity, const std::function<PipelineDesc()>& generate);
  std::shared_ptr<DevBuf> sort_key_planes(const Operator& s, const DevTable& in, int& W, std::vector<int64_t>* str_len = nullptr, bool measure_only = false);
  DevTable literal_table(const std::vector<std::vector<ExprP>>& rows, const std::vector<DType>& types);
  DevTable take_rows(const DevTable& in, const uint32_t* dev_perm, int64_t first, int64_t rows, std::shared_ptr<DevBuf> perm_owner);
  DevTable nested_aggregate(const Operator& agg);
  DevTable write_shuffle(const Operator& sw);
  DevTable expand(const Operator& ex, const DevTable& in);
  DevTable explode(const Operator& ex, const DevTable& in);
  DevTable window(const Operator& w, const DevTable& in);
  DevTable bloom_aggregate(const Operator& agg, const DevTable& in);
  const void* bloom_buffer(const PipelineDesc::BloomRef& ref);
  void bind_blooms(const PipelineDesc& d, CometKParams& prm);
  void prepare_dict_keys(DevTable& src);
  static bool is_source(const Operator& op, const Operator* chain_top);
  typedef std::function<std::pair<const DevTable*, int>(int)> GatherSource;
  DevTable outputs_to_table(Variant& v, const std::vector<std::shared_ptr<DevBuf>>& vals, const std::vector<std::shared_ptr<DevBuf>>& valid_bytes,
                            int64_t rows, const GatherSource& gather_source = nullptr);
  DeviceColumnView take_column(const DeviceColumnView& src, const DType& t, bool has_valid, const uint32_t* idx, const uint8_t* ok_bytes, int64_t rows, bool& out_has_valid,
                               std::vector<std::shared_ptr<void>>& owners);
  void take_utf8(const DeviceColumnView& src, const uint32_t* idx, const uint8_t* ok_bytes, const uint8_t* src_valid_bits, int64_t rows,
                 DeviceColumnView& out, std::vector<std::shared_ptr<void>>& owners);
  void table_to_host_batches(const DevTable& t);
  DevTable host_batch_to_table(const HostBatch& b);
  bool pull_host_chunk();
  bool pull_device_batch();
  bool pull_host_table(size_t input, const std::vector<DType>& types, int64_t max_rows, std::vector<DeviceColumnView>& views,
                       std::vector<bool>& has_valid, int64_t& rows);
  bool pull_device_table(size_t input, const std::vector<DType>& types, std::vector<DeviceColumnView>& views, std::vector<bool>& has_valid,
                         int64_t& rows, std::shared_ptr<void>& keepalive);
  void validate_input_schema(size_t input, const std::vector<DType>& types);
  void export_batch(HostBatch& b, ArrowArray** out_arrays, ArrowSchema** out_schemas, int n_out);
  void check_device_errors();
  void raise_device_errors(uint32_t flags);
  void note_sites(const PipelineDesc& d) {
    site_ctx_last_.clear();
    for (auto& kv : d.site_contexts) {
      site_ctx_last_[kv.first] = kv.second;
      auto it = site_ctx_.find(kv.first);
      if (it == site_ctx_.end()) site_ctx_[kv.first] = kv.second;
      else if (it->second != kv.second && !(it->second && kv.second && it->second->sql_text == kv.second->sql_text && it->second->start_index == kv.second->start_index &&
                                            it->second->stop_index == kv.second->stop_index))
        site_ctx_ambiguous_.insert(kv.first);
    }
    for (int k = 0; k < 2; k++) if (d.agg_ctx[k]) agg_ctx_[k] = d.agg_ctx[k];
  }
  const QueryContext* site_context(uint32_t id) const {
    auto a = site_ctx_last_.find(id);
    if (a != site_ctx_last_.end()) return a->second.get();
    if (site_ctx_ambiguous_.count(id)) return nullptr;
    auto b = site_ctx_.find(id);
    return b == site_ctx_.end() ? nullptr : b->second.get();
  }
  std::map<uint32_t, std::shared_ptr<QueryContext>> site_ctx_last_;
  std::set<uint32_t> site_ctx_ambiguous_;
  std::shared_ptr<QueryContext> agg_ctx_[2];
  std::map<uint32_t, std::shared_ptr<QueryContext>> site_ctx_;
  void read_small(void* dst, const void* dev_src, size_t n);
  void write_small(void* dev_dst, const void* src, size_t n);
  void timed_begin();
  void timed_end();
  void collect_timings();
  void launch(Variant& v, const char* kernel, int grid, CometKParams& prm, int block = 256);

  OperatorP plan_;
  uint64_t plan_hash_ = 0;
  std::vector<std::pair<std::string, std::string>> config_;
  std::vector<InputSource> inputs_;
  int batch_size_;
  int device_id_;
  int64_t chunk_rows_;
  hipStream_t stream_ = nullptr;
  std::vector<std::pair<hipEvent_t, hipEvent_t>> timed_;
  size_t timed_done_ = 0;
  struct KtPending { std::string name; hipEvent_t a, b; };
  std::vector<KtPending> kt_pending_;
  std::map<std::string, std::pair<double, int64_t>> kernel_times_;
  hipEvent_t aux_ev_[2] = {nullptr, nullptr};
  int aux_n_ = 0;
  bool started_ = false, finished_ = false;
  std::vector<DType> in_types_;
  std::map<std::string, Variant> variants_;
  Variant* agg_variant_ = nullptr;
  std::string explain_;
  SinkKind sink_ = SinkKind::Output;
  bool has_join_ = false;
  SubqueryProvider subquery_provider_;
  std::map<int64_t, std::pair<bool, std::string>> subquery_values_;
  bool subqueries_resolved_ = false;
  int64_t strfn_rows_ = 0;
  int64_t split_rows_ = 0;
  bool materialize_root_ = false;
  bool compile_in_infer_ = false;
  std::vector<const Operator*> nested_aggs_;
  struct ExpandPart {
    OperatorP proj;
    std::vector<int> out_col;
    std::vector<int> null_cols;
  };
  struct ExpandInfo {
    std::vector<ExpandPart> parts;
    std::vector<OutCol> out_cols;
  };
  std::map<const Operator*, ExpandInfo> expand_info_;
  std::map<const Operator*, OperatorP> bloom_proj_;
  std::shared_ptr<BloomRegistry> blooms_;
  std::map<const Operator*, OperatorP> explode_proj_;
  std::map<const Operator*, OperatorP> window_psort_, window_osort_;
  std::map<const Operator*, OperatorP> range_sort_, range_bsort_;
  std::shared_ptr<void> planes_owner_;
  std::map<const Operator*, OperatorP> shuffle_projs_;
  int64_t shuffle_bytes_written_ = 0, shuffle_data_size_ = 0, shuffle_staged_peak_ = 0;
  double shuffle_repart_ns_ = 0, shuffle_write_ns_ = 0;
  std::vector<int> dict_id_col_;
  bool device_result_ = false;
  DevTable dict_src_;
  std::map<const Operator*, FusedProbe> fused_probe_;
  std::map<const Operator*, FusedProbe> fused_build_;
  int64_t ramp_rows_ = 0;
  bool fuse_probe_ = true;
  int fuse_build_ = 1;
  std::set<const Operator*> smj_needs_sort_;
  std::map<const Operator*, OperatorP> smj_sorts_;
  const Operator* root_source_ = nullptr;
  std::map<const Operator*, int> node_id_;
  std::map<const Operator*, size_t> scan_input_;
  int64_t join_build_rows_ = 0, join_probe_rows_ = 0, join_keymap_bytes_ = 0, join_direct_maps_ = 0, join_bucket_tables_ = 0, join_bitmap_only_ = 0, join_mono_tables_ = 0, join_fused_builds_ = 0;
  int small_write_slot_ = 0;
  bool single_chunk_hint_ = false, part_result_ready_ = false;
  DevTable part_result_;
  int64_t part_merges_ = 0;
  bool try_partitioned_merge(Variant& v, CometKParams& prm, int64_t n);
  struct DevPending {
    std::vector<DeviceColumnView> views;
    std::vector<bool> has_valid;
    int64_t rows = 0;
    std::shared_ptr<void> keep;
    bool valid = false;
  };
  DevPending dev_pending_;
  bool dev_stream_done_ = false;
  int64_t dev_chunks_seen_ = 0;
  int64_t bytes_scanned_ = 0;
  int64_t row_groups_pruned_ = 0;
  int64_t row_groups_pruned_bloom_ = 0;
  std::shared_ptr<MemAccount> mem_ = std::make_shared<MemAccount>();
  int64_t rows_pruned_page_index_ = 0;
  int64_t pages_inflated_on_device_ = 0;

  std::vector<std::unique_ptr<Staging>> staging_;
  int stage_parity_ = 0;
  std::vector<bool> schema_checked_;
  std::vector<std::vector<std::string>> scan_cast_from_;

  DevBuf partials_;
  int64_t n_partials_ = 0;
  int64_t agg_rows_seen_ = 0;
  std::vector<int> fix_scales_;
  bool fix_has_state_ = false;
  int fix_attempts_ = 0;
  uint64_t groups_committed_ = 0;
  long long packed_fix_scales(const PipelineDesc& d, int first = 0);
  bool adjust_fix_scales(const PipelineDesc& d, const uint64_t* aux, std::vector<int>& shift_right);
  DevBuf err_flags_;
  PinnedBuf result_host_;
  PinnedBuf small_host_;
  PinnedBuf export_host_;
  DevBuf group_table_, group_backup_;
  int64_t group_cap_ = 0;
  bool group_table_clear_ = false;
  DevBuf scratch_mask_, scratch_counts_;
  std::vector<std::unique_ptr<DevBuf>> out_vals_, out_valid_;
  DevBuf emit_arena_;

  std::deque<HostBatch> ready_;
  int64_t output_rows_ = 0;
  double elapsed_compute_ns_ = 0;
};

}
```

### datafusion-comet_amd/csrc/exec_input.cpp

```cpp
#include "exec_internal.hpp"
#include <emmintrin.h>
#include <mutex>
#include <set>
#include <tuple>

namespace comet {

static void stream_copy(void* dst, const void* src, size_t n) {
  char* d = (char*)dst;
  const char* s = (const char*)src;
  if (n < 4096) { memcpy(d, s, n); return; }
  const size_t head = (size_t)(-(intptr_t)d) & 15;
  if (head) { memcpy(d, s, head); d += head; s += head; n -= head; }
  size_t blocks = n / 64;
  for (; blocks; blocks--, d += 64, s += 64) {
    const __m128i a = _mm_loadu_si128((const __m128i*)s), b = _mm_loadu_si128((const __m128i*)(s + 16)), c = _mm_loadu_si128((const __m128i*)(s + 32)),
                  e = _mm_loadu_si128((const __m128i*)(s + 48));
    _mm_stream_si128((__m128i*)d, a);
    _mm_stream_si128((__m128i*)(d + 16), b);
    _mm_stream_si128((__m128i*)(d + 32), c);
    _mm_stream_si128((__m128i*)(d + 48), e);
  }
  _mm_sfence();
  if (n & 63) memcpy(d, s, n & 63);
}

void ExecutionContext::validate_input_schema(size_t input, const std::vector<DType>& types) {
  if (schema_checked_.size() <= input) schema_checked_.resize(input + 1, false);
  if (schema_checked_[input]) return;
  InputSource& in = inputs_[input];
  ArrowSchema sch;
  memset(&sch, 0, sizeof sch);
  int rc = in.kind == 0 ? in.host->get_schema(in.host, &sch) : in.dev->get_schema(in.dev, &sch);
  if (rc != 0 || !sch.release) throw CometError("input stream: get_schema failed");
  std::string err;
  if (in.kind == 1 && (size_t)sch.n_children == types.size()) {
    if (fixed_len_hint_.size() <= input) fixed_len_hint_.resize(input + 1);
    fixed_len_hint_[input].assign(types.size(), -1);
    for (size_t c = 0; c < types.size(); c++) {
      const char* md = sch.children[c]->metadata;
      if (!md || types[c].id != TypeId::String) continue;
      int32_t npairs;
      memcpy(&npairs, md, 4);
      const char* q = md + 4;
      for (int32_t k = 0; k < npairs && k < 4096; k++) {
        int32_t kl, vl;
        memcpy(&kl, q, 4);
        if (kl < 0 || kl > (1 << 20)) break;
        const char* key = q + 4;
        memcpy(&vl, key + kl, 4);
        if (vl < 0 || vl > (1 << 24)) break;
        const char* val = key + kl + 4;
        if (kl == 20 && !memcmp(key, "comet:utf8_fixed_len", 20) && vl > 0 && vl < 4) {
          const int L = atoi(std::string(val, (size_t)vl).c_str());
          if (L >= 0 && L <= 15) fixed_len_hint_[input][c] = L;
        }
        q = val + vl;
      }
    }
  }
  if ((size_t)sch.n_children != types.size()) {
    err = "Scan declares " + std::to_string(types.size()) + " field(s) but the input stream has " + std::to_string(sch.n_children);
  } else {
    for (size_t c = 0; c < types.size() && err.empty(); c++) {
      const ArrowSchema* f = sch.children[c];
      const char* fmt = f->dictionary ? f->dictionary->format : f->format;
      if (types[c].is_nested()) {
        if (in.kind == 0 && nested_schema_matches(f, types[c])) continue;
        err = "Scan input column " + std::to_string(c) + " (Arrow format '" + (fmt ? fmt : "?") + "') does not match the declared " + types[c].str() +
              (in.kind == 0 ? " field by field (nested input columns are not cast)" : ": nested columns of device-resident inputs are not supported");
        break;
      }
      if (format_matches(fmt, types[c])) continue;
      if (in.kind == 0 && !f->dictionary && scan_cast_supported(parse_src_format(fmt), types[c])) {
        if (scan_cast_from_.size() <= input) scan_cast_from_.resize(input + 1);
        scan_cast_from_[input].resize(types.size());
        scan_cast_from_[input][c] = fmt;
        continue;
      }
      err = "Scan input column " + std::to_string(c) + " has Arrow format '" + (fmt ? fmt : "?") + "' but the plan declares " + types[c].str() +
            " (this cast of a scan input is not supported by the MI355X native engine" + (in.kind == 0 ? ")" : "; device-resident inputs are never cast)");
    }
  }
  sch.release(&sch);
  if (!err.empty()) throw CometError(err);
  schema_checked_[input] = true;
}

bool ExecutionContext::pull_host_table(size_t input, const std::vector<DType>& in_types_, int64_t max_rows,
                                       std::vector<DeviceColumnView>& views, std::vector<bool>& has_valid, int64_t& rows_out) {
  InputSource& in = inputs_[input];
  rows_out = 0;
  if (in.exhausted) return false;
  validate_input_schema(input, in_types_);
  const size_t slot = input * 2 + (size_t)(stage_parity_ & 1);
  if (staging_.size() <= slot) staging_.resize(slot + 1);
  if (!staging_[slot]) staging_[slot].reset(new Staging());
  Staging& stg = *staging_[slot];
  if (stg.busy) {
    HIP_CHECK(hipEventSynchronize(stg.busy));
    pool_put_event(device_id_, stg.busy);
    stg.busy = nullptr;
  }
  auto& stage_vals_ = stg.stage_vals;
  auto& stage_valid_ = stg.stage_valid;
  auto& stage_aux_ = stg.stage_aux;
  auto& dev_vals_ = stg.dev_vals;
  auto& dev_valid_ = stg.dev_valid;
  auto& dev_aux_ = stg.dev_aux;
  const size_t nc = in_types_.size();
  if (stage_vals_.size() != nc) {
    stage_vals_.resize(nc);
    stage_valid_.resize(nc);
    stage_aux_.resize(nc);
    dev_vals_.resize(nc);
    dev_valid_.resize(nc);
    dev_aux_.resize(nc);
    for (size_t c = 0; c < nc; c++) {
      stage_vals_[c].reset(new PinnedBuf());
      stage_valid_[c].reset(new PinnedBuf());
      stage_aux_[c].reset(new PinnedBuf());
      dev_vals_[c].reset(new DevBuf());
      dev_valid_[c].reset(new DevBuf());
      dev_aux_[c].reset(new DevBuf());
    }
  }
  int64_t rows = 0;
  has_valid.assign(nc, false);
  std::vector<ArrowArray> held;
  while (rows < max_rows) {
    ArrowArray arr;
    memset(&arr, 0, sizeof arr);
    int rc = in.host->get_next(in.host, &arr);
    if (rc != 0) {
      const char* m = in.host->get_last_error ? in.host->get_last_error(in.host) : nullptr;
      for (auto& a : held) if (a.release) a.release(&a);
      throw CometError(std::string("input ArrowArrayStream.get_next failed: ") + (m ? m : "unknown error"));
    }
    if (!arr.release) {
      in.exhausted = true;
      break;
    }
    if ((size_t)arr.n_children != nc) {
      std::string msg = "input batch has " + std::to_string(arr.n_children) + " columns, Scan declares " + std::to_string(nc);
      arr.release(&arr);
      for (auto& a : held) if (a.release) a.release(&a);
      throw CometError(msg);
    }
    rows += arr.length;
    held.push_back(arr);
  }
  if (rows == 0) {
    for (auto& a : held) if (a.release) a.release(&a);
// ... 219 lines not shown
        int uniform = -2;
        int32_t* dst = so + j.at;
        for (int64_t i = 0; i < col->length; i++) {
          const int64_t o = off_at(col, i);
          dst[i] = j.pos + (int32_t)(o - base);
          const int len = (int)(off_at(col, i + 1) - o);
          if (uniform == -2) uniform = len;
          else if (uniform != len) uniform = -1;
        }
        j.uniform = uniform;
        const size_t nb = (size_t)(off_at(col, col->length) - base);
        if (nb) stream_copy((char*)stage_aux_[c]->p + j.pos, (const char*)col->buffers[2] + base, nb);
      };
      if (rows >= (1 << 20) && sjobs.size() > 1) {
        const size_t parts = std::min<size_t>(16, sjobs.size());
        scan_pool_parallel(parts, [&](size_t pidx) {
          for (size_t k = pidx; k < sjobs.size(); k += parts) run_job(sjobs[k]);
        });
      } else {
        for (auto& j : sjobs) run_job(j);
      }
      int uniform = -2;
      for (auto& j : sjobs) {
        if (j.col->length == 0) continue;
        if (uniform == -2) uniform = j.uniform;
        else if (uniform != j.uniform) uniform = -1;
      }
      if (has_valid[c])
        for (auto& j : sjobs) {
          if (j.col->null_count != 0 && j.col->buffers[0]) bit_append((uint8_t*)stage_valid_[c]->p, j.at, (const uint8_t*)j.col->buffers[0], j.col->offset, j.col->length);
          else bit_fill_ones((uint8_t*)stage_valid_[c]->p, j.at, j.col->length);
        }
      so[rows] = pos;
      dev_vals_[c]->ensure((size_t)(rows + 1) * 4 + 16);
      dev_aux_[c]->ensure(total_bytes + 16);
      HIP_CHECK(hipMemcpyAsync(dev_vals_[c]->p, stage_vals_[c]->p, (size_t)(rows + 1) * 4, hipMemcpyHostToDevice, stream_));
      if (total_bytes) HIP_CHECK(hipMemcpyAsync(dev_aux_[c]->p, stage_aux_[c]->p, total_bytes, hipMemcpyHostToDevice, stream_));
      if (has_valid[c]) {
        size_t kb = (size_t)((rows + 7) / 8);
        dev_valid_[c]->ensure(kb + 16);
        HIP_CHECK(hipMemcpyAsync(dev_valid_[c]->p, stage_valid_[c]->p, kb, hipMemcpyHostToDevice, stream_));
      }
      aux_bytes[c] = total_bytes;
      str_uniform_[c] = (uniform >= 0 && uniform <= 15) ? uniform : -1;
      continue;
    }
    const int w = fixed_width(t);
    size_t vbytes = w ? (size_t)rows * w : (size_t)((rows + 7) / 8);
    stage_vals_[c]->ensure(vbytes + 16);
    if (has_valid[c]) stage_valid_[c]->ensure((size_t)((rows + 7) / 8) + 16);
    int64_t at = 0;
    struct CopyJob { char* dst; const char* src; size_t n; };
    std::vector<CopyJob> jobs;
    for (auto& a : held) {
      const ArrowArray* col = a.children[c];
      if (col->dictionary) throw CometError("dictionary-encoded input columns are not unpacked on the GPU path yet");
      const int64_t len = col->length, off = col->offset;
      if (len != a.length) throw CometError("ragged input batch");
      if (cast_from[c].cls != SrcFmt::Unknown) {
        if (col->null_count != 0 && col->buffers[0]) bit_append((uint8_t*)stage_valid_[c]->p, at, (const uint8_t*)col->buffers[0], off, len);
        else bit_fill_ones((uint8_t*)stage_valid_[c]->p, at, len);
        if (!w) throw CometError("casting a scan input to Boolean is not supported");
        const char* src = (const char*)col->buffers[1] + (size_t)off * (size_t)cast_from[c].width;
        char* dst = (char*)stage_vals_[c]->p + (size_t)at * w;
        uint8_t* vb = (uint8_t*)stage_valid_[c]->p;
        for (int64_t i = 0; i < len; i++) {
          const int64_t bit = at + i;
          const bool ok = ((vb[bit >> 3] >> (bit & 7)) & 1) && scan_cast_value(cast_from[c], src, i, t, dst + (size_t)i * w);
          if (!ok) {
            vb[bit >> 3] &= (uint8_t)~(1u << (bit & 7));
            memset(dst + (size_t)i * w, 0, (size_t)w);
          }
        }
        at += len;
        continue;
      }
      if (w) {
        jobs.push_back({(char*)stage_vals_[c]->p + (size_t)at * w, (const char*)col->buffers[1] + (size_t)off * w, (size_t)len * w});
      } else {
        bit_append((uint8_t*)stage_vals_[c]->p, at, (const uint8_t*)col->buffers[1], off, len);
      }
      if (has_valid[c]) {
        if (col->null_count != 0 && col->buffers[0]) bit_append((uint8_t*)stage_valid_[c]->p, at, (const uint8_t*)col->buffers[0], off, len);
        else bit_fill_ones((uint8_t*)stage_valid_[c]->p, at, len);
      }
      at += len;
    }
    if (vbytes >= ((size_t)8 << 20)) {
      std::vector<CopyJob> pieces;
      const size_t kPiece = (size_t)4 << 20;
      for (auto& j : jobs)
        for (size_t o = 0; o < j.n; o += kPiece) pieces.push_back({j.dst + o, j.src + o, std::min(kPiece, j.n - o)});
      jobs.swap(pieces);
    }
    if (vbytes >= ((size_t)8 << 20) && jobs.size() > 1) {
      const size_t parts = std::min<size_t>(16, jobs.size());
      scan_pool_parallel(parts, [&](size_t pidx) {
        for (size_t j = pidx; j < jobs.size(); j += parts) stream_copy(jobs[j].dst, jobs[j].src, jobs[j].n);
      });
    } else {
      for (auto& j : jobs) stream_copy(j.dst, j.src, j.n);
    }
    dev_vals_[c]->ensure(vbytes + 16);
    HIP_CHECK(hipMemcpyAsync(dev_vals_[c]->p, stage_vals_[c]->p, vbytes, hipMemcpyHostToDevice, stream_));
    if (has_valid[c]) {
      size_t kb = (size_t)((rows + 7) / 8);
      dev_valid_[c]->ensure(kb + 16);
      HIP_CHECK(hipMemcpyAsync(dev_valid_[c]->p, stage_valid_[c]->p, kb, hipMemcpyHostToDevice, stream_));
    }
  }
  for (auto& a : held) if (a.release) a.release(&a);
  views.assign(nc, DeviceColumnView());
  for (size_t c = 0; c < nc; c++) {
    if (in_types_[c].is_nested()) { views[c] = nested_views[c]; continue; }
    views[c].data = dev_vals_[c]->p;
    views[c].valid = has_valid[c] ? (const uint8_t*)dev_valid_[c]->p : nullptr;
    views[c].aux = dev_aux_[c]->p;
    views[c].fixed_len = str_uniform_[c];
  }
  rows_out = rows;
  return true;
}

bool ExecutionContext::pull_host_chunk() {
  std::vector<DeviceColumnView> views;
  std::vector<bool> has_valid;
  int64_t rows = 0;
  if (ramp_rows_ <= 0) ramp_rows_ = std::max<int64_t>(chunk_rows_ / 4, std::min<int64_t>(chunk_rows_, 65536));
  const int64_t want_rows = std::min<int64_t>(chunk_rows_, ramp_rows_);
  ramp_rows_ = std::min<int64_t>(chunk_rows_, ramp_rows_ * 2);
  if (!pull_host_table(0, in_types_, want_rows, views, has_valid, rows)) return false;
  if (rows > 0) {
    process_chunk(views, has_valid, rows);
    Staging& stg = *staging_[(size_t)(stage_parity_ & 1)];
    stg.busy = pool_get_event(device_id_);
    HIP_CHECK(hipEventRecord(stg.busy, stream_));
    stage_parity_ ^= 1;
  }
  return !inputs_[0].exhausted;
}


namespace {
struct UniformKey {
  const void* off; int64_t rows; int32_t len; int32_t first;
  bool operator<(const UniformKey& o) const { return std::tie(off, rows, len, first) < std::tie(o.off, o.rows, o.len, o.first); }
};
std::mutex g_uniform_mu;
std::set<UniformKey> g_uniform_ok;
bool uniform_verdict_known(const void* off, int64_t rows, int32_t len, int32_t first) {
  std::lock_guard<std::mutex> g(g_uniform_mu);
  return g_uniform_ok.count(UniformKey{off, rows, len, first}) != 0;
}
void remember_uniform_verdict(const void* off, int64_t rows, int32_t len, int32_t first) {
  std::lock_guard<std::mutex> g(g_uniform_mu);
  if (g_uniform_ok.size() >= 4096) g_uniform_ok.clear();
  g_uniform_ok.insert(UniformKey{off, rows, len, first});
}
}

bool ExecutionContext::pull_device_table(size_t input, const std::vector<DType>& types, std::vector<DeviceColumnView>& views,
                                         std::vector<bool>& has_valid, int64_t& rows, std::shared_ptr<void>& keepalive) {
  InputSource& in = inputs_[input];
  rows = 0;
  if (in.exhausted) return false;
  static const bool trace = getenv("COMET_TRACE_STAGES") != nullptr;
  Timer tm;
  validate_input_schema(input, types);
  const double t_schema = tm.ns();
  auto da = std::make_shared<ArrowDeviceArray>();
  memset(da.get(), 0, sizeof(ArrowDeviceArray));
  int rc = in.dev->get_next(in.dev, da.get());
  if (trace) fprintf(stderr, "[comet] device input %zu: get_schema %.3f ms, get_next %.3f ms\n", input, t_schema / 1e6, (tm.ns() - t_schema) / 1e6);
  if (rc != 0) {
    const char* m = in.dev->get_last_error ? in.dev->get_last_error(in.dev) : nullptr;
    throw CometError(std::string("input ArrowDeviceArrayStream.get_next failed: ") + (m ? m : "unknown error"));
  }
  if (!da->array.release) {
    in.exhausted = true;
    return false;
  }
  keepalive = std::shared_ptr<void>(da.get(), [da](void*) mutable {
    if (da->array.release) da->array.release(&da->array);
  });
  if (da->device_type != ARROW_DEVICE_ROCM && da->device_type != ARROW_DEVICE_ROCM_HOST)
    throw CometError("device input stream must carry ARROW_DEVICE_ROCM memory");
  if (da->sync_event) HIP_CHECK(hipStreamWaitEvent(stream_, *(hipEvent_t*)da->sync_event, 0));
  const size_t nc = types.size();
  if ((size_t)da->array.n_children != nc) throw CometError("device batch column count does not match Scan fields");
  views.assign(nc, DeviceColumnView());
  has_valid.assign(nc, false);
  for (size_t c = 0; c < nc; c++) {
    const ArrowArray* col = da->array.children[c];
    if (col->dictionary) throw CometError("dictionary-encoded device columns are not supported yet");
    views[c].data = col->buffers[1];
    views[c].offset = col->offset;
    if (types[c].id == TypeId::String || types[c].id == TypeId::Bytes) views[c].aux = col->buffers[2];
    if (types[c].id == TypeId::Decimal && (((uintptr_t)col->buffers[1]) & 15))
      throw CometError("device Decimal128 buffers must be 16-byte aligned");
    if (col->null_count != 0 && col->buffers[0]) {
      has_valid[c] = true;
      views[c].valid = (const uint8_t*)col->buffers[0];
    }
  }
  rows = da->array.length;
  std::vector<size_t> scols;
  for (size_t c = 0; c < nc && rows > 0; c++)
    if (types[c].id == TypeId::String) scols.push_back(c);
  if (!scols.empty() && scols.size() <= 16) {
    small_host_.ensure(4096);
    int32_t* ends = (int32_t*)small_host_.p;
    for (size_t k = 0; k < scols.size(); k++) {
      const ArrowArray* col = da->array.children[scols[k]];
      const int32_t* off = (const int32_t*)col->buffers[1] + col->offset;
      HIP_CHECK(hipMemcpyAsync(ends + 2 * k, off, 4, hipMemcpyDeviceToHost, stream_));
      HIP_CHECK(hipMemcpyAsync(ends + 2 * k + 1, off + rows, 4, hipMemcpyDeviceToHost, stream_));
    }
    HIP_CHECK(hipStreamSynchronize(stream_));
    std::vector<int32_t> first(scols.size()), len(scols.size(), -1);
    std::vector<bool> declared(scols.size(), false);
    uint32_t* flags = (uint32_t*)err_flags_.p + (kErrBytes / 4 - 16);
    HIP_CHECK(hipMemsetAsync(flags, 0, 64, stream_));
    bool any = false;
    if (!aux_ev_[0]) { aux_ev_[0] = pool_get_event(device_id_); aux_ev_[1] = pool_get_event(device_id_); }
    HIP_CHECK(hipEventRecord(aux_ev_[0], stream_));
    int aux_launched = 0;
    for (size_t k = 0; k < scols.size(); k++) {
      first[k] = ends[2 * k];
      const int64_t total = (int64_t)ends[2 * k + 1] - ends[2 * k];
      const int hint = input < fixed_len_hint_.size() && scols[k] < fixed_len_hint_[input].size() ? fixed_len_hint_[input][scols[k]] : -1;
      const ArrowArray* col = da->array.children[scols[k]];
      const int32_t* off = (const int32_t*)col->buffers[1] + col->offset;
      if (hint >= 0) {
        if (total != (int64_t)hint * rows)
          throw CometError("device input column " + std::to_string(scols[k]) + " is declared comet:utf8_fixed_len=" + std::to_string(hint) + " but holds " +
                           std::to_string(total) + " bytes in " + std::to_string(rows) + " rows");
        if ((int64_t)first[k] != (int64_t)col->offset * hint) continue;
        if (uniform_verdict_known(off, rows, hint, first[k])) {
          views[scols[k]].fixed_len = hint;
          continue;
        }
        if (comet_launch_utf8_uniform(off, rows, hint, flags + k, stream_) != 0) continue;
        aux_launched++;
        len[k] = hint;
        declared[k] = true;
        any = true;
        continue;
      }
      if (total % rows != 0 || total / rows > 15 || total < 0) continue;
      if (comet_launch_utf8_uniform(off, rows, (int32_t)(total / rows), flags + k, stream_) != 0) continue;
      aux_launched++;
      len[k] = (int32_t)(total / rows);
      any = true;
    }
    if (any) {
      HIP_CHECK(hipEventRecord(aux_ev_[1], stream_));
      uint32_t f[16];
      read_small(f, flags, 64);
      float aux = 0;
      if (hipEventElapsedTime(&aux, aux_ev_[0], aux_ev_[1]) == hipSuccess) { last_aux_ms += aux; last_aux_launches += aux_launched; }
      HIP_CHECK(hipMemsetAsync(flags, 0, 64, stream_));
      for (size_t k = 0; k < scols.size(); k++) {
        if (len[k] < 0) continue;
        const size_t c = scols[k];
        const ArrowArray* col = da->array.children[c];
        if (declared[k]) {
          if (f[k] != 0)
            throw CometError("device input column " + std::to_string(c) + " is declared comet:utf8_fixed_len=" + std::to_string(len[k]) +
                             " but its offsets are not " + std::to_string(len[k]) + " bytes apart (the byte total alone matches)");
          remember_uniform_verdict((const int32_t*)col->buffers[1] + col->offset, rows, len[k], first[k]);
          views[c].fixed_len = len[k];
          continue;
        }
        if (f[k] != 0) continue;
        if ((int64_t)first[k] != (int64_t)col->offset * len[k]) continue;
        views[c].fixed_len = len[k];
      }
    }
  }
  return true;
}

bool ExecutionContext::pull_device_batch() {
  DevPending cur;
  if (dev_pending_.valid) {
    cur = std::move(dev_pending_);
    dev_pending_ = DevPending();
  } else {
    if (dev_stream_done_ || !pull_device_table(0, in_types_, cur.views, cur.has_valid, cur.rows, cur.keep)) return false;
  }
  if (sink_ == SinkKind::AggGrouped && dev_chunks_seen_ == 0 && !dev_stream_done_) {
    dev_pending_.valid = pull_device_table(0, in_types_, dev_pending_.views, dev_pending_.has_valid, dev_pending_.rows, dev_pending_.keep);
    if (!dev_pending_.valid) dev_stream_done_ = true;
    single_chunk_hint_ = !dev_pending_.valid;
  } else {
    single_chunk_hint_ = false;
  }
  dev_chunks_seen_++;
  process_chunk(cur.views, cur.has_valid, cur.rows);
  HIP_CHECK(hipStreamSynchronize(stream_));
  return true;
}


}
```

### datafusion-comet_amd/csrc/exec_internal.hpp

```cpp
#pragma once
#include "exec.hpp"
#include "shuffle_format.hpp"
#include "fix_scale.hpp"

#include <cerrno>
#include <fcntl.h>
#include <unistd.h>
#include <chrono>
#include <condition_variable>
#include <cstdio>
#include <cstdlib>
#include <cmath>
#include <cstring>
#include <functional>
#include <map>
#include <mutex>

extern "C" int comet_launch_dict_gather_fixed(const void* idx, int iw, const uint8_t* idx_valid, const uint8_t* dict, const uint8_t* dict_valid,
                                              int width, int64_t n, uint8_t* out, uint8_t* out_valid_bytes, void* stream);
extern "C" int comet_launch_dict_gather_str_len(const void* idx, int iw, const uint8_t* idx_valid, const int32_t* dict_offs, const uint8_t* dict_valid,
                                                int64_t n, uint32_t* lengths, uint8_t* out_valid_bytes, void* stream);
extern "C" int comet_launch_dict_gather_str_copy(const void* idx, int iw, const uint8_t* valid_bytes, const int32_t* dict_offs, const uint8_t* dict_bytes,
                                                 int64_t n, const int32_t* out_offs, uint8_t* out_bytes, void* stream);
extern "C" void pq_launch_u32_scan(const uint32_t* in, int64_t n, uint64_t* tiles, int32_t* out, void* st);
extern "C" void pq_launch_pack(const uint8_t* bytes, uint8_t* bitmap, int64_t n, void* st);
extern "C" int comet_launch_window_default(int width, const uint8_t* inside, int64_t n, const void* value, void* data, uint8_t* ok_bytes, void* stream);
extern "C" int comet_launch_window_widen(int width, const void* src, const uint8_t* valid_bits, int64_t n, void* out128, void* hi128, uint32_t* ok, void* stream);
extern "C" int comet_launch_scan128(const void* in128, int64_t n, void* tiles, void* out128, void* stream);
extern "C" int comet_launch_window_running_extreme(const void* vals128, const uint32_t* ok, const int32_t* sp, int64_t n, int backward, int is_max, void* local, void* tiles, void* out_v,
                                                   uint8_t* out_has, void* stream);
extern "C" int comet_launch_window_minmax(int is_max, int lo_kind, int64_t lo_off, int hi_kind, int64_t hi_off, const void* vals128, const uint32_t* ok, const void* P, const uint8_t* Ph,
                                          const void* Q, const uint8_t* Qh, const int32_t* sp, const int32_t* sg, const uint32_t* first_part, const uint32_t* first_peer, int64_t n,
                                          int out_width, void* out, uint8_t* out_ok, void* stream);
extern "C" int comet_launch_window_range_bounds(int width, const void* keys, const uint8_t* valid, const int32_t* sp, const uint32_t* first_part, int64_t n, int desc, int nulls_first,
                                                int has_lo, int64_t dlo, int has_hi, int64_t dhi, int32_t* out_lo, int32_t* out_hi, void* stream);
extern "C" int comet_launch_window_valid_flags(const uint8_t* valid, int64_t n, uint32_t* flags, void* stream);
extern "C" int comet_launch_window_pick(int mode, int64_t nth, int lo_kind, int64_t lo_off, int hi_kind, int64_t hi_off, const int32_t* C, const int32_t* sp, const int32_t* sg,
                                        const uint32_t* first_part, const uint32_t* first_peer, int64_t n, uint32_t* idx, uint8_t* ok, void* stream);
extern "C" int comet_launch_window_agg(int fn, int lo_kind, int64_t lo_off, int hi_kind, int64_t hi_off, const void* S128, const void* SH128, const int32_t* C, const int32_t* sp, const int32_t* sg, const uint32_t* first_part,
                                       const uint32_t* first_peer, int64_t n, const void* bound16, const void* scaler16, const void* avg_bound16, void* out, uint8_t* out_ok,
                                       void* stream);
extern "C" int comet_launch_window_fexp(int width, const void* src, const uint8_t* valid_bits, int64_t n, uint64_t* hi_lo, void* stream);
extern "C" int comet_launch_scan192_f64(int width, const void* src, const uint8_t* valid_bits, int64_t n, int scale, int slice, void* tiles, void* out192, void* stream);
extern "C" int comet_launch_scan128_fclass(int width, const void* src, const uint8_t* valid_bits, int64_t n, void* tiles, void* out128, void* stream);
extern "C" int comet_launch_window_fagg(int fn, int lo_kind, int64_t lo_off, int hi_kind, int64_t hi_off, const void* S192, int windows, const void* K128, int scale, const int32_t* sp, const int32_t* sg,
                                        const uint32_t* first_part, const uint32_t* first_peer, int64_t n, double* out, uint8_t* out_ok, void* stream);
extern "C" int comet_launch_window_flags(const uint8_t* part_planes, int Wp, const uint8_t* order_planes, int Wo, int64_t n, uint32_t* fpart, uint32_t* fpeer, void* stream);
extern "C" int comet_launch_window_first(const uint32_t* fpart, const int32_t* sp, const uint32_t* fpeer, const int32_t* sg, int64_t n, uint32_t* first_part,
                                         uint32_t* first_peer, void* stream);
extern "C" int comet_launch_window_rank(int kind, int64_t arg, const int32_t* sp, const int32_t* sg, const uint32_t* first_part, const uint32_t* first_peer, int64_t n,
                                        void* out, void* stream);
extern "C" int comet_launch_window_offset(int64_t shift, const int32_t* sp, const uint32_t* first_part, int64_t n, uint32_t* idx, uint8_t* ok, void* stream);
extern "C" int comet_launch_window_offset_valid(const uint32_t* idx, const uint8_t* ok, const uint8_t* src_valid_bits, int64_t n, uint8_t* out_ok, void* stream);
struct CometConcatArgs {
  int32_t n;
  int32_t lit_len[8];
  const int32_t* offs[8];
  const uint8_t* bytes[8];
  int64_t first[8];
};
extern "C" int comet_launch_concat_lengths(const CometConcatArgs* a, const uint32_t* rows, const uint8_t* ok_bytes, int64_t n, uint32_t* lengths, void* stream);
extern "C" int comet_launch_concat_copy(const CometConcatArgs* a, const uint32_t* rows, const uint8_t* ok_bytes, int64_t n, const int32_t* out_offs, uint8_t* out_bytes, void* stream);
extern "C" int comet_launch_strcase_lengths(const void* views, const uint8_t* ok_bytes, const int32_t* src_offs, const uint8_t* src_bytes, int64_t n, int mode, uint32_t* lengths, void* stream);
extern "C" int comet_launch_strcase_write(const void* views, const uint8_t* ok_bytes, const int32_t* src_offs, const uint8_t* src_bytes, int64_t n, int mode, const int32_t* out_offs,
                                          uint8_t* out_bytes, void* stream);
extern "C" int comet_launch_join_part_scan(uint32_t* cnt, int g, int np, uint32_t* tot, uint32_t limit, uint64_t* over, void* stream);
extern "C" int comet_launch_popcount128(const void* blocks, int64_t n, uint32_t* counts, void* stream);
extern "C" int comet_launch_strfmt_lengths(int kind, long long arg, const void* vals128, const uint8_t* ok_bytes, int64_t n, uint32_t* lengths, void* stream);
extern "C" int comet_launch_strfmt_write(int kind, long long arg, const void* vals128, const uint8_t* ok_bytes, int64_t n, const int32_t* out_offs, uint8_t* out_bytes, void* stream);
extern "C" int comet_launch_strfn_len(int op, const int32_t* offs, const uint8_t* bytes, const uint8_t* valid_bits, int64_t valid_first, int64_t n, const uint8_t* a, int32_t na, const uint8_t* b,
                                      int32_t nb, int64_t k, uint32_t* lengths, uint32_t* too_long, void* stream);
extern "C" int comet_launch_strfn_write(int op, const int32_t* offs, const uint8_t* bytes, const uint8_t* valid_bits, int64_t valid_first, int64_t n, const uint8_t* a, int32_t na, const uint8_t* b,
                                        int32_t nb, int64_t k, const int32_t* out_offs, uint8_t* out, void* stream);
extern "C" int comet_launch_split_count(const int32_t* offs, const uint8_t* bytes, const uint8_t* valid_bits, int64_t valid_first, int64_t n, const uint32_t* prog, const uint32_t* prog2, int32_t limit,
                                        uint32_t* counts, void* stream);
extern "C" int comet_launch_split_write(const int32_t* offs, const uint8_t* bytes, const uint8_t* valid_bits, int64_t valid_first, int64_t n, const uint32_t* prog, const uint32_t* prog2, int32_t limit,
                                        const int32_t* list_offs, void* views, void* stream);
extern "C" int comet_launch_strview_lengths(const void* views, const uint8_t* ok_bytes, int64_t n, const uint8_t* pattern, int32_t pattern_bytes, uint32_t* lengths, void* stream);
extern "C" int comet_launch_strview_copy(const void* views, const uint8_t* ok_bytes, const int32_t* src_offs, const uint8_t* src_bytes, int64_t n, const uint8_t* pattern,
                                         int32_t pattern_bytes, int pad_left, const int32_t* out_offs, uint8_t* out_bytes, void* stream);
extern "C" int comet_launch_str16_lengths(const void* packed, const uint8_t* ok_bytes, int64_t n, uint32_t* lengths, void* stream);
extern "C" int comet_launch_str16_copy(const void* packed, const int32_t* offsets, int64_t n, uint8_t* bytes, void* stream);
extern "C" int comet_launch_str_max_len(const int32_t* offs, int64_t n, uint32_t* out_max, void* stream);
extern "C" int comet_launch_str_dict_build(const int32_t* offs, const uint8_t* bytes, const uint8_t* valid_bits, int64_t n, uint32_t* table, int64_t slots,
                                           int64_t* rep, void* stream);
extern "C" int comet_launch_str_dict_lookup(const int32_t* build_offs, const uint8_t* build_bytes, const uint32_t* table, int64_t slots, const int32_t* offs,
                                            const uint8_t* bytes, const uint8_t* valid_bits, int64_t n, int64_t* rep, uint8_t* ok, void* stream);
extern "C" int64_t comet_partition_tiles(int64_t n);
extern "C" int64_t comet_partition_scratch_bytes(int64_t n, int32_t P);
extern "C" int comet_launch_fill(int width, void* dst, int64_t n, const void* value, void* stream);
extern "C" int comet_launch_copy_small(const void* descs, int n, uint64_t longest, void* stream);
extern "C" int comet_launch_murmur3(int type_id, int precision, const void* values, const uint8_t* validity, const void* aux, int64_t n, uint32_t* hashes, void* stream);
extern "C" int comet_launch_pmod(const uint32_t* hashes, int64_t n, int32_t np, int32_t* out, void* stream);
extern "C" int comet_launch_partition_indices(const int32_t* pids, int64_t n, int32_t P, uint64_t* hist, uint32_t* bad, int64_t* starts,
                                              uint32_t* row_indices, void* stream);
extern "C" int comet_launch_take(int width, const void* src, const uint32_t* idx, int64_t n, void* dst, void* stream);
extern "C" int comet_launch_take_utf8_lengths(const int32_t* offs, const uint32_t* idx, const uint8_t* ok_bytes, const uint8_t* src_valid_bits, int64_t n,
                                              uint32_t* lengths, void* stream);
extern "C" int comet_launch_explode_counts(const int32_t* offs, const uint8_t* valid_bits, int64_t n, int outer, uint32_t* counts, void* stream);
extern "C" int comet_launch_explode_indices(const int32_t* offs, const uint8_t* valid_bits, const uint8_t* elem_valid_bits, int64_t n, const int32_t* out_offs, uint32_t* row_idx,
                                            uint32_t* elem_idx, uint8_t* has_elem, int32_t* pos, uint8_t* elem_ok, void* stream);
extern "C" int comet_launch_take_list_indices(const int32_t* offs, const uint32_t* idx, int64_t n, const int32_t* out_offs, uint32_t* elem_idx, void* stream);
extern "C" int comet_launch_take_utf8_copy(const int32_t* offs, const uint8_t* bytes, const uint32_t* idx, const uint8_t* ok_bytes, const uint8_t* src_valid_bits,
                                           int64_t n, const int32_t* out_offs, uint8_t* out_bytes, void* stream);
extern "C" void pq_launch_u32_scan(const uint32_t* in, int64_t n, uint64_t* tiles, int32_t* out, void* st);
extern "C" int comet_launch_sort_small(const uint8_t* planes, int64_t n, const uint32_t* cand, int m, const int* plane_idx, int nv, uint32_t* out, void* stream);
extern "C" int comet_launch_sort_iota(uint32_t* perm, int64_t n, uint32_t first, void* stream);
extern "C" int comet_launch_sort_gather_digit(const uint8_t* plane, const uint32_t* perm, int64_t n, int32_t* digit, void* stream);
extern "C" int comet_launch_range_partition_ids(const uint8_t* planes, int64_t n, int W, const uint8_t* bkeys, int B, int32_t* pids, void* stream);
extern "C" int comet_launch_sort_plane_varies(const uint8_t* planes, int64_t n, int W, uint32_t* flags, void* stream);
extern "C" int comet_launch_sort_hist256(const uint8_t* plane, const uint32_t* cand, int64_t m, uint64_t* hist, void* stream);
extern "C" int comet_launch_sort_select(const uint8_t* plane, const uint32_t* cand, int64_t m, int dstar, uint32_t* sure, uint32_t* next_cand, uint32_t* counters,
                                        void* stream);
extern "C" int comet_launch_fix_rescale(uint64_t* base, int64_t count, int64_t stride_words, int32_t word_off, int32_t shift, void* stream);
extern "C" int comet_launch_utf8_uniform(const int32_t* offsets, int64_t n, int32_t L, uint32_t* flag, void* stream);

namespace comet {
HostColumn download_column(const DeviceColumnView& v, const DType& t, bool has_valid, int64_t rows, hipStream_t st);

namespace detail {
void plan_execution_begins();
void plan_execution_ends();
int plans_executing();

hipStream_t pool_get_stream(int dev);
void pool_put_stream(int dev, hipStream_t s);
hipEvent_t pool_get_event(int dev);
void pool_put_event(int dev, hipEvent_t e);

int fixed_width(const DType& t);
inline int out_width(const OutCol& oc) { return (oc.view_src >= 0 || oc.fmt_kind) ? 16 : (oc.gather_src >= 0 || !oc.concat_cols.empty()) ? 4 : oc.packed_string ? 16 : (oc.type.id == TypeId::Bool ? 1 : fixed_width(oc.type)); }
void bit_append(uint8_t* dst, int64_t dst_off, const uint8_t* src, int64_t src_off, int64_t n);
bool nested_schema_matches(const ArrowSchema* f, const DType& t);
void append_nested_rows(HostColumn& dst, const ArrowArray* a, const DType& t, int64_t off, int64_t len);
void bit_fill_ones(uint8_t* dst, int64_t dst_off, int64_t n);
bool format_matches(const char* fmt, const DType& t);
struct SrcFmt {
  enum Cls { Unknown, Int, UInt, F32, F64, Date32, Date64, Ts, Dec, Utf8, LargeUtf8, Bool } cls = Unknown;
  int width = 0;
  int64_t per_second = 0;
  int p = 0, s = 0;
};
SrcFmt parse_src_format(const char* fmt);
bool scan_cast_supported(const SrcFmt& f, const DType& t);
bool scan_cast_value(const SrcFmt& f, const char* src, int64_t i, const DType& t, char* dst);
const Operator* find_scan(const Operator* op);
std::string validity_key(const std::vector<bool>& v);
void bind_inputs(CometKParams& prm, const std::vector<DeviceColumnView>& cols, const std::vector<bool>& has_valid, size_t first_slot = 0);
u128 pow10_u128_host(int p);
struct Timer {
  std::chrono::steady_clock::time_point t0 = std::chrono::steady_clock::now();
  double ns() const { return (double)std::chrono::duration_cast<std::chrono::nanoseconds>(std::chrono::steady_clock::now() - t0).count(); }
};

struct PlannedVariant {
  PipelineDesc desc;
  std::shared_ptr<CodeObject> code;
};
extern std::mutex g_plan_mu;
extern std::map<std::string, std::shared_ptr<PlannedVariant>> g_plan_cache;
std::shared_ptr<PlannedVariant> planned_variant(const Operator& plan, uint64_t plan_hash, const std::vector<bool>& has_valid, bool compile,
                                                const std::vector<DType>* source_types = nullptr, const std::vector<int>* str_fixed_len = nullptr,
                                                const std::vector<int>* dict_id_col = nullptr);

}
using namespace detail;
}
```

### datafusion-comet_amd/csrc/exec_pipeline.cpp

```cpp
#include "exec_internal.hpp"

namespace comet {
void ExecutionContext::process_chunk(const std::vector<DeviceColumnView>& cols, const std::vector<bool>& has_valid, int64_t n) {
  if (n == 0) return;
  std::vector<int> fixed_lens(cols.size(), -1);
  for (size_t i = 0; i < cols.size(); i++) fixed_lens[i] = cols[i].fixed_len;
  Variant& v = variant_for(has_valid, fixed_lens);
  const PipelineDesc& d = v.desc;
  if (d.max_rows_exact && input_rows + n > d.max_rows_exact)
    throw CometError("decimal or integer sum over more rows than its static no-overflow proof allows (" + std::to_string(d.max_rows_exact) + ")");
  CometKParams prm;
  memset(&prm, 0, sizeof prm);
  prm.n = n;
  bind_inputs(prm, cols, has_valid);
  err_flags_.ensure(kErrBytes);
  prm.out[kOutErr] = err_flags_.p;
  if (!has_join_) input_rows += n;
  if (d.sink == SinkKind::AggNoGroup || d.sink == SinkKind::AggGrouped) {
    prm.iarg[kRowBaseArg] = agg_rows_seen_;
    agg_rows_seen_ += n;
  }

  if (d.sink == SinkKind::AggNoGroup) {
    if (agg_variant_ && agg_variant_->desc.NW != d.NW) throw CometError("internal: accumulator layout differs between variants");
    agg_variant_ = &v;
    const int64_t tile = (int64_t)d.R * 256;
    int grid = (int)std::min<int64_t>((n + tile - 1) / tile, 256 * 8);
    size_t need = (size_t)(n_partials_ + grid) * d.NW * 8;
    if (need > partials_.cap) {
      DevBuf bigger;
      bigger.ensure(std::max(need * 2, (size_t)(4096 * d.NW * 8)));
      if (n_partials_) HIP_CHECK(hipMemcpyAsync(bigger.p, partials_.p, (size_t)n_partials_ * d.NW * 8, hipMemcpyDeviceToDevice, stream_));
      HIP_CHECK(hipStreamSynchronize(stream_));
      std::swap(partials_.p, bigger.p);
      std::swap(partials_.cap, bigger.cap);
    }
    prm.out[kOutPartials] = (char*)partials_.p + (size_t)n_partials_ * d.NW * 8;
    for (int attempt = 0;; attempt++) {
      prm.iarg[kFixScaleArg] = packed_fix_scales(d), prm.iarg[kFixScaleArg2] = packed_fix_scales(d, 4);
      timed_begin();
      launch(v, "k_agg", grid, prm);
      timed_end();
      if (d.fix_sums.empty()) break;
      uint64_t aux[2 + 2 * kFixMaxSums];
      read_small(aux, err_flags_.p, sizeof aux);
      std::vector<int> shift;
      if (attempt >= 3 || !adjust_fix_scales(d, aux + 2, shift)) break;
      for (size_t f = 0; f < shift.size(); f++)
        if (shift[f] > 0 && n_partials_ > 0 &&
            comet_launch_fix_rescale((uint64_t*)partials_.p, n_partials_, d.NW, d.fix_sums[f].word, shift[f], stream_) != 0)
          throw CometError("float sum rescale: launch failed");
    }
    fix_has_state_ = fix_has_state_ || !d.fix_sums.empty();
    n_partials_ += grid;
    return;
  }

  if (d.sink == SinkKind::AggGrouped) {
    if (agg_variant_ && (agg_variant_->desc.NW != d.NW || agg_variant_->desc.NK != d.NK))
      throw CometError("internal: group slot layout differs between variants");
    agg_variant_ = &v;
    if (try_partitioned_merge(v, prm, n)) return;
    const size_t slot_bytes = 8 + 8 * (size_t)(d.NK + d.NW);
    auto alloc_table = [&](DevBuf& buf, int64_t cap) {
      buf.ensure((size_t)cap * slot_bytes);
      HIP_CHECK(hipMemsetAsync(buf.p, 0, (size_t)cap * slot_bytes, stream_));
    };
    if (group_cap_ == 0) {
      int64_t want = 1 << 16;
      if (d.merges_states) {
        while (want < 2 * n && want < ((int64_t)1 << 26)) want <<= 1;
      } else if (n <= ((int64_t)1 << 24)) {
        while (want < 2 * n && want < ((int64_t)1 << 22)) want <<= 1;
      }
      group_cap_ = want;
      alloc_table(group_table_, group_cap_);
      group_table_clear_ = true;
      HIP_CHECK(hipMemsetAsync((char*)err_flags_.p + 8, 0, 8, stream_));
    }
    const int64_t tile = (int64_t)d.R * 256;
    int grid_mult = 4;
    if (const char* e = getenv("COMET_GROUPED_GRID_MULT")) grid_mult = std::max(1, atoi(e));
    int grid = (int)std::min<int64_t>((n + tile - 1) / tile, 256 * grid_mult);
    const int64_t per_block_cap = ((int64_t)1 << 19) - 2 * tile;
    grid = (int)std::max<int64_t>(grid, (n + per_block_cap - 1) / per_block_cap);
    while (true) {
      const bool clear = group_table_clear_;
      if (!clear) {
        group_backup_.ensure((size_t)group_cap_ * slot_bytes);
        HIP_CHECK(hipMemcpyAsync(group_backup_.p, group_table_.p, (size_t)group_cap_ * slot_bytes, hipMemcpyDeviceToDevice, stream_));
      }
      prm.out[0] = group_table_.p;
      prm.iarg[0] = group_cap_;
      prm.iarg[kFixScaleArg] = packed_fix_scales(d), prm.iarg[kFixScaleArg2] = packed_fix_scales(d, 4);
      timed_begin();
      launch(v, "k_gagg", grid, prm);
      timed_end();
      uint64_t head[2 + (kErrBytes - 16) / 8];
      uint32_t flags[4];
      read_small(head, err_flags_.p, d.fix_sums.empty() ? 16 : sizeof head);
      memcpy(flags, head, 16);
      uint64_t groups_now;
      memcpy(&groups_now, &flags[2], 8);
      const bool full = (flags[0] & 32u) != 0;
      if (!full && !d.fix_sums.empty() && fix_attempts_ < 3) {
        std::vector<int> shift;
        if (adjust_fix_scales(d, head + 2, shift)) {
          fix_attempts_++;
          if (clear) HIP_CHECK(hipMemsetAsync(group_table_.p, 0, (size_t)group_cap_ * slot_bytes, stream_));
          else HIP_CHECK(hipMemcpyAsync(group_table_.p, group_backup_.p, (size_t)group_cap_ * slot_bytes, hipMemcpyDeviceToDevice, stream_));
          uint32_t restore[4] = {flags[0], flags[1], 0, 0};
          memcpy(&restore[2], &groups_committed_, 8);
          write_small(err_flags_.p, restore, 16);
          for (size_t f = 0; f < shift.size(); f++)
            if (shift[f] > 0 && comet_launch_fix_rescale((uint64_t*)group_table_.p, group_cap_, (int64_t)(slot_bytes / 8), 1 + d.NK + d.fix_sums[f].word, shift[f], stream_) != 0)
              throw CometError("float sum rescale: launch failed");
          continue;
        }
      }
      if (!full && (int64_t)groups_now * 2 <= group_cap_) { groups_committed_ = groups_now; group_table_clear_ = false; break; }
      int64_t new_cap = group_cap_ * 8;
      if (full) {
        int64_t need = 1 << 16;
        while (need < 2 * n && need < ((int64_t)1 << 28)) need <<= 1;
        new_cap = std::max(new_cap, std::min(group_cap_ * 64, need));
      }
      if (new_cap > ((int64_t)1 << 28)) throw CometError("group table would exceed 2^28 slots");
      DevBuf bigger;
      alloc_table(bigger, new_cap);
      uint32_t zero4[4] = {flags[0] & ~32u, flags[1], 0, 0};
      write_small(err_flags_.p, zero4, 16);
      CometKParams rp;
      memset(&rp, 0, sizeof rp);
      rp.out[0] = bigger.p;
      rp.iarg[0] = new_cap;
      rp.out[2] = err_flags_.p;
      rp.out[3] = full ? group_backup_.p : group_table_.p;
      rp.iarg[1] = group_cap_;
      if (!(full && clear)) launch(v, "k_grehash", (int)std::min<int64_t>((group_cap_ + 255) / 256, 256 * 8), rp);
      HIP_CHECK(hipStreamSynchronize(stream_));
      std::swap(group_table_.p, bigger.p);
      std::swap(group_table_.cap, bigger.cap);
      group_cap_ = new_cap;
      if (!full) { groups_committed_ = groups_now; group_table_clear_ = false; break; }
    }
    fix_attempts_ = 0;
    fix_has_state_ = fix_has_state_ || !d.fix_sums.empty();
    if (std::find(d.kernels.begin(), d.kernels.end(), std::string("k_gpick")) != d.kernels.end()) {
      prm.out[0] = group_table_.p;
      prm.iarg[0] = group_cap_;
      timed_begin();
      launch(v, "k_gpick", (int)std::min<int64_t>((group_cap_ + 255) / 256, 256 * 8), prm);
      timed_end();
    }
    return;
  }

  if (d.sink == SinkKind::Output) {
    for (auto& oc : d.out_cols)
      if (oc.gather_src >= 0 || oc.view_src >= 0 || oc.fmt_kind || !oc.concat_cols.empty()) throw CometError("internal: gathered Utf8 outputs must go through the materialising path");
    const size_t ncol = d.out_cols.size();
    int64_t out_rows = n;
    if (out_vals_.size() < ncol) {
      out_vals_.resize(ncol);
      out_valid_.resize(ncol);
      for (size_t j = 0; j < ncol; j++) {
        if (!out_vals_[j]) out_vals_[j].reset(new DevBuf());
        if (!out_valid_[j]) out_valid_[j].reset(new DevBuf());
      }
    }
    auto bind_outputs = [&](int64_t rows_cap) {
      for (size_t j = 0; j < ncol; j++) {
        int w = d.out_cols[j].type.id == TypeId::Bool ? 1 : fixed_width(d.out_cols[j].type);
        out_vals_[j]->ensure((size_t)rows_cap * w + 16);
        prm.out[kOutFirstCol + 2 * j] = out_vals_[j]->p;
        if (d.out_cols[j].nullable) {
          out_valid_[j]->ensure((size_t)rows_cap + 16);
          prm.out[kOutFirstCol + 2 * j + 1] = out_valid_[j]->p;
        }
      }
    };
    timed_begin();
    if (d.has_filter) {
      bind_outputs(n);
      out_rows = launch_fused_filter(v, prm, n);
    } else {
      bind_outputs(n);
      int grid = (int)std::min<int64_t>((n + 255) / 256, 256 * 8);
      launch(v, "k_emit", grid, prm);
    }
    timed_end();
    check_device_errors();
    if (out_rows == 0) return;
    std::vector<std::vector<uint8_t>> hv(ncol), hk(ncol);
    for (size_t j = 0; j < ncol; j++) {
      int w = d.out_cols[j].type.id == TypeId::Bool ? 1 : fixed_width(d.out_cols[j].type);
      hv[j].resize((size_t)out_rows * w);
      HIP_CHECK(hipMemcpyAsync(hv[j].data(), out_vals_[j]->p, hv[j].size(), hipMemcpyDeviceToHost, stream_));
      if (d.out_cols[j].nullable) {
        hk[j].resize((size_t)out_rows);
        HIP_CHECK(hipMemcpyAsync(hk[j].data(), out_valid_[j]->p, hk[j].size(), hipMemcpyDeviceToHost, stream_));
      }
    }
    HIP_CHECK(hipStreamSynchronize(stream_));
    const int64_t bs = batch_size_ > 0 ? batch_size_ : out_rows;
    for (int64_t off = 0; off < out_rows; off += bs) {
      int64_t len = std::min(bs, out_rows - off);
      HostBatch b;
      b.rows = len;
      for (size_t j = 0; j < ncol; j++) {
        HostColumn c;
        c.type = d.out_cols[j].type;
        c.length = len;
        if (c.type.id == TypeId::Bool) {
          c.values.assign((size_t)((len + 7) / 8), 0);
          for (int64_t i = 0; i < len; i++)
            if (hv[j][(size_t)(off + i)]) c.values[(size_t)(i >> 3)] |= (uint8_t)(1u << (i & 7));
        } else {
          int w = fixed_width(c.type);
          c.values.assign(hv[j].begin() + (size_t)off * w, hv[j].begin() + (size_t)(off + len) * w);
        }
        if (d.out_cols[j].nullable) {
          int64_t nulls = 0;
          std::vector<uint8_t> bm((size_t)((len + 7) / 8), 0);
          for (int64_t i = 0; i < len; i++) {
            if (hk[j][(size_t)(off + i)]) bm[(size_t)(i >> 3)] |= (uint8_t)(1u << (i & 7));
            else nulls++;
          }
          c.null_count = nulls;
          if (nulls) c.validity = std::move(bm);
        }
        b.cols.push_back(std::move(c));
      }
      ready_.push_back(std::move(b));
    }
    return;
  }
  throw CometError("internal: unsupported sink");
}

void ExecutionContext::read_small(void* dst, const void* dev_src, size_t n) {
  if (n > 4096) throw CometError("internal: read_small of " + std::to_string(n) + " bytes (its staging holds 4096)");
  small_host_.ensure(4096);
  HIP_CHECK(hipMemcpyAsync(small_host_.p, dev_src, n, hipMemcpyDeviceToHost, stream_));
  HIP_CHECK(hipStreamSynchronize(stream_));
  memcpy(dst, small_host_.p, n);
}
void ExecutionContext::write_small(void* dev_dst, const void* src, size_t n) {
  if (n > 2048) throw CometError("internal: write_small of " + std::to_string(n) + " bytes (its staging holds 2048)");
  small_host_.ensure(4096);
  if (n <= 128) {
    if (small_write_slot_ == 16) {
      HIP_CHECK(hipStreamSynchronize(stream_));
      small_write_slot_ = 0;
// ... 420 lines not shown
```

### datafusion-comet_amd/csrc/kernels_static.hip

```cpp
#include <hip/hip_runtime.h>

#include "device/comet_device.hpp"

using namespace comet;

template <class F>
__global__ __launch_bounds__(256) void mm3_kernel(const void* values, const u8* validity, i64 n, u32* hashes, F f) {
  for (i64 i = (i64)blockIdx.x * 256 + threadIdx.x; i < n; i += (i64)gridDim.x * 256) {
    if (validity && !((validity[i >> 3] >> (i & 7)) & 1)) continue;
    hashes[i] = f(values, i, hashes[i]);
  }
}

struct HashBool { __device__ u32 operator()(const void* v, i64 i, u32 s) const { return mm3_hash_i32((((const u8*)v)[i >> 3] >> (i & 7)) & 1, s); } };
struct HashI8 { __device__ u32 operator()(const void* v, i64 i, u32 s) const { return mm3_hash_i32((i32)((const i8*)v)[i], s); } };
struct HashI16 { __device__ u32 operator()(const void* v, i64 i, u32 s) const { return mm3_hash_i32((i32)((const i16*)v)[i], s); } };
struct HashI32 { __device__ u32 operator()(const void* v, i64 i, u32 s) const { return mm3_hash_i32(((const i32*)v)[i], s); } };
struct HashI64 { __device__ u32 operator()(const void* v, i64 i, u32 s) const { return mm3_hash_i64(((const i64*)v)[i], s); } };
struct HashF32 { __device__ u32 operator()(const void* v, i64 i, u32 s) const { return mm3_hash_f32(((const float*)v)[i], s); } };
struct HashF64 { __device__ u32 operator()(const void* v, i64 i, u32 s) const { return mm3_hash_f64(((const double*)v)[i], s); } };
struct HashDecSmall { __device__ u32 operator()(const void* v, i64 i, u32 s) const { return mm3_hash_i64(((const i64*)v)[2 * i], s); } };
struct HashDecWide { __device__ u32 operator()(const void* v, i64 i, u32 s) const { return mm3_hash_i128(((const i128*)v)[i], s); } };
struct HashUtf8 {
  const u8* bytes;
  __device__ u32 operator()(const void* v, i64 i, u32 s) const {
    const i32* off = (const i32*)v;
    return mm3_hash_bytes(bytes + off[i], off[i + 1] - off[i], s);
  }
};

__global__ __launch_bounds__(256) void pmod_kernel(const u32* hashes, i64 n, i32 np, i32* out) {
  for (i64 i = (i64)blockIdx.x * 256 + threadIdx.x; i < n; i += (i64)gridDim.x * 256) out[i] = pmod(hashes[i], np);
}

__global__ __launch_bounds__(256) void utf8_uniform_kernel(const i32* off, i64 n, i32 L, u32* flag) {
  bool bad = false;
  const i32 o0 = off[0];
  const i64 total = n + 1;
  i64 head = 0;
  while (head < total && ((((uintptr_t)(off + head)) & 15) != 0)) head++;
  const int4* v4 = (const int4*)(off + head);
  const i64 ngroups = (total - head) / 4;
  constexpr int U = 4;
  for (i64 g0 = ((i64)blockIdx.x * 256 + threadIdx.x) * U; g0 < ngroups; g0 += (i64)gridDim.x * 256 * U) {
    int4 v[U];
#pragma unroll
    for (int u = 0; u < U; u++) v[u] = g0 + u < ngroups ? v4[g0 + u] : make_int4(0, 0, 0, 0);
#pragma unroll
    for (int u = 0; u < U; u++) {
      if (g0 + u < ngroups) {
        const i64 i = head + 4 * (g0 + u);
        const i32 e = o0 + (i32)(i * L);
        bad |= (v[u].x != e) | (v[u].y != e + L) | (v[u].z != e + 2 * L) | (v[u].w != e + 3 * L);
      }
    }
  }
  if (blockIdx.x == 0) {
    for (i64 i = threadIdx.x; i < head; i += 256) bad |= off[i] != o0 + (i32)(i * L);
    for (i64 i = head + ngroups * 4 + threadIdx.x; i < total; i += 256) bad |= off[i] != o0 + (i32)(i * L);
  }
  if (__any(bad) && lane_id() == 0) atomicOr(flag, 1u);
}

__device__ __forceinline__ i64 dict_index(const void* idx, int iw, i64 i) {
  switch (iw) {
    case 1: return ((const i8*)idx)[i];
    case 2: return ((const i16*)idx)[i];
    case 4: return ((const i32*)idx)[i];
    default: return ((const i64*)idx)[i];
  }
}
__global__ __launch_bounds__(256) void dict_gather_fixed_kernel(const void* idx, int iw, const u8* idx_valid, const u8* dict, const u8* dict_valid,
                                                                int width, i64 n, u8* out, u8* out_valid_bytes) {
  for (i64 i = (i64)blockIdx.x * 256 + threadIdx.x; i < n; i += (i64)gridDim.x * 256) {
    bool ok = !idx_valid || ((idx_valid[i >> 3] >> (i & 7)) & 1);
    i64 k = ok ? dict_index(idx, iw, i) : 0;
    if (ok && dict_valid) ok = (dict_valid[k >> 3] >> (k & 7)) & 1;
    for (int b = 0; b < width; b++) out[i * width + b] = ok ? dict[k * width + b] : 0;
    out_valid_bytes[i] = ok ? 1 : 0;
  }
}
__global__ __launch_bounds__(256) void dict_gather_str_len_kernel(const void* idx, int iw, const u8* idx_valid, const i32* dict_offs, const u8* dict_valid,
                                                                  i64 n, u32* lengths, u8* out_valid_bytes) {
  for (i64 i = (i64)blockIdx.x * 256 + threadIdx.x; i < n; i += (i64)gridDim.x * 256) {
    bool ok = !idx_valid || ((idx_valid[i >> 3] >> (i & 7)) & 1);
    i64 k = ok ? dict_index(idx, iw, i) : 0;
    if (ok && dict_valid) ok = (dict_valid[k >> 3] >> (k & 7)) & 1;
    lengths[i] = ok ? (u32)(dict_offs[k + 1] - dict_offs[k]) : 0;
    out_valid_bytes[i] = ok ? 1 : 0;
  }
}
__global__ __launch_bounds__(256) void dict_gather_str_copy_kernel(const void* idx, int iw, const u8* valid_bytes, const i32* dict_offs, const u8* dict_bytes,
                                                                   i64 n, const i32* out_offs, u8* out_bytes) {
  for (i64 i = (i64)blockIdx.x * 256 + threadIdx.x; i < n; i += (i64)gridDim.x * 256) {
    if (!valid_bytes[i]) continue;
    i64 k = dict_index(idx, iw, i);
    const u8* src = dict_bytes + dict_offs[k];
    i32 len = dict_offs[k + 1] - dict_offs[k];
    u8* dst = out_bytes + out_offs[i];
    for (i32 b = 0; b < len; b++) dst[b] = src[b];
  }
}

static int grid_for(i64 n) {
  i64 g = (n + 255) / 256;
  return (int)(g < 1 ? 1 : (g > 256 * 8 ? 256 * 8 : g));
}

extern "C" int comet_launch_murmur3(int type_id, int precision, const void* values, const uint8_t* validity, const void* aux,
                                    int64_t n, uint32_t* hashes, void* stream) {
  hipStream_t st = (hipStream_t)stream;
  if (n <= 0) return 0;
  int g = grid_for(n);
  switch (type_id) {
    case 0: hipLaunchKernelGGL(mm3_kernel<HashBool>, g, 256, 0, st, values, validity, (i64)n, hashes, HashBool()); break;
    case 1: hipLaunchKernelGGL(mm3_kernel<HashI8>, g, 256, 0, st, values, validity, (i64)n, hashes, HashI8()); break;
    case 2: hipLaunchKernelGGL(mm3_kernel<HashI16>, g, 256, 0, st, values, validity, (i64)n, hashes, HashI16()); break;
    case 3: case 12: hipLaunchKernelGGL(mm3_kernel<HashI32>, g, 256, 0, st, values, validity, (i64)n, hashes, HashI32()); break;
    case 4: case 9: case 11: hipLaunchKernelGGL(mm3_kernel<HashI64>, g, 256, 0, st, values, validity, (i64)n, hashes, HashI64()); break;
    case 5: hipLaunchKernelGGL(mm3_kernel<HashF32>, g, 256, 0, st, values, validity, (i64)n, hashes, HashF32()); break;
    case 6: hipLaunchKernelGGL(mm3_kernel<HashF64>, g, 256, 0, st, values, validity, (i64)n, hashes, HashF64()); break;
    case 7: case 8: {
      HashUtf8 h;
      h.bytes = (const u8*)aux;
      hipLaunchKernelGGL(mm3_kernel<HashUtf8>, g, 256, 0, st, values, validity, (i64)n, hashes, h);
      break;
    }
    case 10:
      if (precision <= 18) hipLaunchKernelGGL(mm3_kernel<HashDecSmall>, g, 256, 0, st, values, validity, (i64)n, hashes, HashDecSmall());
      else hipLaunchKernelGGL(mm3_kernel<HashDecWide>, g, 256, 0, st, values, validity, (i64)n, hashes, HashDecWide());
      break;
    default: return -1;
  }
  return hipGetLastError() == hipSuccess ? 0 : -1;
}

__global__ __launch_bounds__(256) void fix_rescale_kernel(u64* base, i64 count, i64 stride, i32 word_off, i32 shift) {
  for (i64 i = (i64)blockIdx.x * 256 + threadIdx.x; i < count; i += (i64)gridDim.x * 256) {
    u64* t = base + i * stride + word_off;
    const u64 w[3] = {t[0], t[1], t[2]};
    const u64 sign = (w[2] >> 63) ? ~0ull : 0ull;
    u64 r[3];
    const int ws = shift >> 6, bs = shift & 63;
#pragma unroll
    for (int k = 0; k < 3; k++) {
      const u64 lo = k + ws < 3 ? w[k + ws] : sign;
      const u64 hi = k + ws + 1 < 3 ? w[k + ws + 1] : sign;
      r[k] = bs ? (lo >> bs) | (hi << (64 - bs)) : lo;
    }
    t[0] = r[0]; t[1] = r[1]; t[2] = r[2];
  }
}
extern "C" int comet_launch_fix_rescale(uint64_t* base, int64_t count, int64_t stride_words, int32_t word_off, int32_t shift, void* stream) {
  if (count <= 0 || shift <= 0) return 0;
  hipLaunchKernelGGL(fix_rescale_kernel, grid_for(count), 256, 0, (hipStream_t)stream, (u64*)base, (i64)count, (i64)stride_words, word_off, shift > 191 ? 191 : shift);
  return hipGetLastError() == hipSuccess ? 0 : 1;
}

template <class T>
__global__ __launch_bounds__(256) void calib_read_kernel(const T* p, i64 n, u64* sink) {
  u64 acc = 0;
  for (i64 i = (i64)blockIdx.x * 256 + threadIdx.x; i < n; i += (i64)gridDim.x * 256) {
    const T v = p[i];
    const u32* w = (const u32*)&v;
#pragma unroll
    for (int k = 0; k < (int)(sizeof(T) / 4); k++) acc += w[k];
  }
  if (acc == 0x123456789abcdefull) *sink = acc;
}
struct CalibB16 { u32 w[4]; };
__global__ __launch_bounds__(256) void calib_read_lo8_kernel(const u64* p, i64 n, u64* sink) {
  u64 acc = 0;
  for (i64 i = (i64)blockIdx.x * 256 + threadIdx.x; i < n; i += (i64)gridDim.x * 256) acc += p[2 * i];
  if (acc == 0x123456789abcdefull) *sink = acc;
}
extern "C" int comet_calib_read(const void* p, int64_t n_bytes, int32_t lane_bytes, uint64_t* sink, void* stream) {
  hipStream_t st = (hipStream_t)stream;
  const int grid = 256 * 8;
  if (lane_bytes == 4) hipLaunchKernelGGL(calib_read_kernel<u32>, grid, 256, 0, st, (const u32*)p, (i64)(n_bytes / 4), (u64*)sink);
  else if (lane_bytes == 8) hipLaunchKernelGGL(calib_read_kernel<u64>, grid, 256, 0, st, (const u64*)p, (i64)(n_bytes / 8), (u64*)sink);
  else if (lane_bytes == 16) hipLaunchKernelGGL(calib_read_kernel<CalibB16>, grid, 256, 0, st, (const CalibB16*)p, (i64)(n_bytes / 16), (u64*)sink);
  else if (lane_bytes == 816) hipLaunchKernelGGL(calib_read_lo8_kernel, grid, 256, 0, st, (const u64*)p, (i64)(n_bytes / 16), (u64*)sink);
  else return -1;
  return hipGetLastError() == hipSuccess ? 0 : -1;
}

extern "C" int comet_launch_utf8_uniform(const int32_t* offsets, int64_t n, int32_t L, uint32_t* flag, void* stream) {
  if (n <= 0) return 0;
  hipLaunchKernelGGL(utf8_uniform_kernel, grid_for(n), 256, 0, (hipStream_t)stream, offsets, (i64)n, L, flag);
  return hipGetLastError() == hipSuccess ? 0 : -1;
}

extern "C" int comet_launch_dict_gather_fixed(const void* idx, int iw, const uint8_t* idx_valid, const uint8_t* dict, const uint8_t* dict_valid,
                                              int width, int64_t n, uint8_t* out, uint8_t* out_valid_bytes, void* stream) {
  if (n <= 0) return 0;
  hipLaunchKernelGGL(dict_gather_fixed_kernel, grid_for(n), 256, 0, (hipStream_t)stream, idx, iw, idx_valid, dict, dict_valid, width, (i64)n, out, out_valid_bytes);
  return hipGetLastError() == hipSuccess ? 0 : -1;
}
extern "C" int comet_launch_dict_gather_str_len(const void* idx, int iw, const uint8_t* idx_valid, const int32_t* dict_offs, const uint8_t* dict_valid,
                                                int64_t n, uint32_t* lengths, uint8_t* out_valid_bytes, void* stream) {
  if (n <= 0) return 0;
  hipLaunchKernelGGL(dict_gather_str_len_kernel, grid_for(n), 256, 0, (hipStream_t)stream, idx, iw, idx_valid, dict_offs, dict_valid, (i64)n, lengths, out_valid_bytes);
  return hipGetLastError() == hipSuccess ? 0 : -1;
}
extern "C" int comet_launch_dict_gather_str_copy(const void* idx, int iw, const uint8_t* valid_bytes, const int32_t* dict_offs, const uint8_t* dict_bytes,
                                                 int64_t n, const int32_t* out_offs, uint8_t* out_bytes, void* stream) {
  if (n <= 0) return 0;
  hipLaunchKernelGGL(dict_gather_str_copy_kernel, grid_for(n), 256, 0, (hipStream_t)stream, idx, iw, valid_bytes, dict_offs, dict_bytes, (i64)n, out_offs, out_bytes);
  return hipGetLastError() == hipSuccess ? 0 : -1;
}

struct CometCopyDesc { const uint8_t* src; uint8_t* dst; uint64_t len; };
__global__ __launch_bounds__(256) void copy_small_kernel(const CometCopyDesc* __restrict__ descs) {
  const CometCopyDesc d = descs[blockIdx.y];
  const u64 lo = (u64)blockIdx.x << 14, hi = lo + 16384 < d.len ? lo + 16384 : d.len;
  if (lo >= d.len) return;
  if ((((u64)d.src | (u64)d.dst) & 3u) == 0) {
    const u64 words = (hi - lo) >> 2;
    const u32* s4 = (const u32*)(d.src + lo);
    u32* d4 = (u32*)(d.dst + lo);
    for (u64 i = threadIdx.x; i < words; i += 256) d4[i] = s4[i];
    for (u64 i = lo + (words << 2) + threadIdx.x; i < hi; i += 256) d.dst[i] = d.src[i];
  } else {
    for (u64 i = lo + threadIdx.x; i < hi; i += 256) d.dst[i] = d.src[i];
  }
}
extern "C" int comet_launch_copy_small(const void* descs, int n, uint64_t longest, void* stream) {
  if (n <= 0 || !longest) return 0;
  hipLaunchKernelGGL(copy_small_kernel, dim3((unsigned)((longest + 16383) >> 14), (unsigned)n), 256, 0, (hipStream_t)stream, (const CometCopyDesc*)descs);
  return hipGetLastError() == hipSuccess ? 0 : -1;
}

extern "C" int comet_launch_pmod(const uint32_t* hashes, int64_t n, int32_t np, int32_t* out, void* stream) {
  if (n <= 0) return 0;
  hipLaunchKernelGGL(pmod_kernel, grid_for(n), 256, 0, (hipStream_t)stream, hashes, (i64)n, np, out);
  return hipGetLastError() == hipSuccess ? 0 : -1;
}

struct Q6Static {
  static constexpr int R = 4;
  static constexpr int NW = 3;
  static constexpr bool PIPELINED = false;
  static __device__ __forceinline__ void init(u64* a) { a[0] = a[1] = a[2] = 0; }
  static __device__ __forceinline__ void combine(u64* a, const u64* b) {
    acc_add64(a, b);
    acc_add128(a + 1, b + 1);
  }
  static __device__ __forceinline__ void tile(const CometKParams& prm, i64 base, i64 n, u64* acc) {
    bool k[R];
    i64 idx[R];
    i32 sd[R];
    i64 disc[R], qty[R], price[R];
#pragma unroll
    for (int r = 0; r < R; r++) { idx[r] = base + (i64)r * kBlock + threadIdx.x; k[r] = idx[r] < n; }
#pragma unroll
    for (int r = 0; r < R; r++) if (k[r]) sd[r] = ld<i32>(prm.in[3], idx[r]);
#pragma unroll
    for (int r = 0; r < R; r++) if (k[r]) k[r] = sd[r] >= (i32)prm.iarg[1] && sd[r] < (i32)prm.iarg[2];
#pragma unroll
    for (int r = 0; r < R; r++) if (k[r]) disc[r] = ld_dec_lo(prm.in[2], idx[r]);
#pragma unroll
    for (int r = 0; r < R; r++) if (k[r]) k[r] = disc[r] >= prm.iarg[3] && disc[r] <= prm.iarg[4];
#pragma unroll
    for (int r = 0; r < R; r++) if (k[r]) qty[r] = ld_dec_lo(prm.in[0], idx[r]);
#pragma unroll
    for (int r = 0; r < R; r++) if (k[r]) k[r] = qty[r] < prm.iarg[5];
#pragma unroll
    for (int r = 0; r < R; r++) if (k[r]) price[r] = ld_dec_lo(prm.in[1], idx[r]);
#pragma unroll
    for (int r = 0; r < R; r++) if (k[r]) {
      acc[0] += 1;
      acc_feed_i128(acc + 1, (i128)price[r] * (i128)disc[r]);
    }
  }
  static __device__ __forceinline__ void kexport(const CometKParams&, const u64*) {}
  static __device__ __forceinline__ void finalize(const CometKParams& prm, const u64* acc) {
    ((i128*)prm.out[4])[0] = mk128(acc[2], acc[1]);
    ((u8*)prm.out[5])[0] = 1;
    ((u8*)prm.out[6])[0] = acc[0] == 0 ? 1 : 0;
  }
};

extern "C" __global__ __launch_bounds__(256) void comet_q6_static_agg(const CometKParams prm) { agg_nogroup_body<Q6Static>(prm); }
extern "C" __global__ __launch_bounds__(256) void comet_q6_static_final(const CometKParams prm) { agg_nogroup_final_body<Q6Static>(prm); }

__global__ __launch_bounds__(256) void popcount128_kernel(const uint4* blocks, long long n, unsigned int* counts) {
  for (long long k = (long long)blockIdx.x * 256 + threadIdx.x; k < n; k += (long long)gridDim.x * 256) {
    const uint4 w = blocks[k];
    counts[k] = (unsigned int)(__popc(w.x) + __popc(w.y) + __popc(w.z) + __popc(w.w));
  }
}
extern "C" int comet_launch_popcount128(const void* blocks, int64_t n, uint32_t* counts, void* stream) {
  if (n > 0) {
    const long long g = (n + 255) / 256;
    hipLaunchKernelGGL(popcount128_kernel, dim3((unsigned)(g < 256 * 16 ? g : 256 * 16)), dim3(256), 0, (hipStream_t)stream, (const uint4*)blocks, (long long)n, counts);
  }
  return hipGetLastError() == hipSuccess ? 0 : -1;
}

__global__ __launch_bounds__(256) void join_part_scan_kernel(unsigned int* cnt, int g, int np, unsigned int* tot, unsigned int limit, unsigned long long* over) {
  const int p = (int)(blockIdx.x * 256 + threadIdx.x);
  if (p >= np) return;
  unsigned int run = 0;
  int b = 0;
  for (; b + 8 <= g; b += 8) {
    unsigned int c[8];
#pragma unroll
    for (int k = 0; k < 8; k++) c[k] = cnt[(long long)(b + k) * np + p];
#pragma unroll
    for (int k = 0; k < 8; k++) {
      cnt[(long long)(b + k) * np + p] = run;
      run += c[k];
    }
  }
  for (; b < g; b++) {
    const unsigned int c = cnt[(long long)b * np + p];
    cnt[(long long)b * np + p] = run;
    run += c;
  }
  tot[p] = run;
  if (run > limit) *(volatile unsigned long long*)over = 1ull;
}
extern "C" int comet_launch_join_part_scan(uint32_t* cnt, int g, int np, uint32_t* tot, uint32_t limit, uint64_t* over, void* stream) {
  if (g > 0 && np > 0)
    hipLaunchKernelGGL(join_part_scan_kernel, dim3((unsigned)((np + 255) / 256)), dim3(256), 0, (hipStream_t)stream, cnt, g, np, tot, (unsigned int)limit, (unsigned long long*)over);
  return hipGetLastError() == hipSuccess ? 0 : -1;
}
```

### datafusion-comet_amd/csrc/kparams.h

```cpp
#ifndef COMET_KPARAMS_H
#define COMET_KPARAMS_H

#define COMET_MAX_IN 24
#define COMET_MAX_OUT 48

#define COMET_ERR_BYTES 512
#define COMET_ERR_AUX_WORDS 22
#define COMET_ERR_DETAIL_WORD 24
#define COMET_ERR_DETAIL_STR_BYTES 224

typedef struct CometCol {
  const void* data;
  const unsigned char* valid;
  const void* aux;
  long long offset;
} CometCol;

typedef struct CometKParams {
  long long n;
  long long iarg[7];
  CometCol in[COMET_MAX_IN];
  void* out[COMET_MAX_OUT];
} CometKParams;

#endif
```

Measured before the change: 71.46 billion rows/s.

## Speculate Utf8 fixed key lengths from memo and verify on a side stream

Previously each device batch read the string offset endpoints to the host and ran a blocking uniform-offset check before the aggregate kernel could start. Now the fixed length of each key column is memoized per plan, input and column, and later runs take it as a guess. The aggregate kernel checks the offset endpoints itself and raises an error bit if they do not match, which voids the speculation; the full uniformity check can run beside it on a separate stream. The check kernel is also rewritten to batch several columns in one launch, with wider unrolling and nontemporal vector loads. The cost is extra complexity and a full re-run of the chunk when a guess turns out wrong.

```diff
diff --git a/datafusion-comet_amd/csrc/codegen.hpp b/datafusion-comet_amd/csrc/codegen.hpp
--- a/datafusion-comet_amd/csrc/codegen.hpp
+++ b/datafusion-comet_amd/csrc/codegen.hpp
@@ -4,6 +4,7 @@
 #include <string>
 #include <vector>
 
+#include "kparams.h"
 #include "plan.hpp"
 
 namespace comet {
@@ -73,6 +74,9 @@
 };
 constexpr int kFixScaleArg = 6;
 constexpr int kFixScaleArg2 = 4;
+constexpr int kGuardArg = 1;
+constexpr int kGuardMaxCols = 6;
+constexpr uint32_t kErrGuardBit = 1u << 30;
 constexpr int kRowBaseArg = 3;
 constexpr int kFixMaxSums = 8;
 constexpr int kFixW = 158;
@@ -100,6 +104,7 @@
 constexpr int kOutCounts = 1;
 constexpr int kOutErr = 2;
 constexpr int kErrBytes = 512;
+constexpr int kUtf8RecBytes = COMET_UTF8_MAX_COLS * COMET_UTF8_REC_WORDS * 4;
 constexpr int kErrAuxWords = 22;
 constexpr int kErrDetailWord = 24;
 constexpr int kErrDetailStrBytes = 224;
diff --git a/datafusion-comet_amd/csrc/device/comet_device.hpp b/datafusion-comet_amd/csrc/device/comet_device.hpp
--- a/datafusion-comet_amd/csrc/device/comet_device.hpp
+++ b/datafusion-comet_amd/csrc/device/comet_device.hpp
@@ -2045,10 +2045,30 @@
   if (!fresh) slot_apply<P, __HIP_MEMORY_SCOPE_AGENT>(&s->acc[0], val);
 }
 
+constexpr int kGuardArg = 1;
+constexpr unsigned int kErrUtf8Guard = 1u << 30;
+CDEV bool utf8_guard_ok(const CometKParams& prm, u64 guard) {
+  const int cnt = (int)(guard & 7);
+  bool ok = true;
+  for (int k = 0; k < cnt; k++) {
+    const u32 f = (u32)(guard >> (3 + 9 * k)) & 511u;
+    const CometCol& col = prm.in[f & 31u];
+    const i64 L = (i64)(f >> 5);
+    const COMET_GLOBAL i32* off = (const COMET_GLOBAL i32*)col.data + col.offset;
+    const i64 first = off[0], last = off[prm.n];
+    ok = ok && first == col.offset * L && last - first == L * prm.n;
+  }
+  return ok;
+}
+
 template <class P>
 CDEV void agg_grouped_body(const CometKParams& prm) {
   typedef Slot<P::NK, P::NW> S;
   typedef LSlot<P::NK, P::NPW> LS;
+  if (prm.iarg[kGuardArg] != 0 && !utf8_guard_ok(prm, (u64)prm.iarg[kGuardArg])) {
+    if (blockIdx.x == 0 && threadIdx.x == 0) atomicOr((unsigned int*)prm.out[2], kErrUtf8Guard);
+    return;
+  }
   __shared__ LS s_tbl[P::LDS_CAP > 0 ? P::LDS_CAP : 1];
   __shared__ u64 s_priv[P::GC * P::NPW * P::COPIES];
   __shared__ u32 s_count;
diff --git a/datafusion-comet_amd/csrc/exec.cpp b/datafusion-comet_amd/csrc/exec.cpp
--- a/datafusion-comet_amd/csrc/exec.cpp
+++ b/datafusion-comet_amd/csrc/exec.cpp
@@ -828,6 +828,12 @@
     (void)hipStreamSynchronize(stream_);
     for (auto& pr : timed_) { pool_put_event(device_id_, pr.first); pool_put_event(device_id_, pr.second); }
     for (hipEvent_t& e : aux_ev_) if (e) { pool_put_event(device_id_, e); e = nullptr; }
+    if (check_stream_) {
+      (void)hipStreamSynchronize(check_stream_);
+      pool_put_stream(device_id_, check_stream_);
+      check_stream_ = nullptr;
+    }
+    if (check_fork_ev_) { pool_put_event(device_id_, check_fork_ev_); check_fork_ev_ = nullptr; }
     for (auto& p : kt_pending_) { pool_put_event(device_id_, p.a); pool_put_event(device_id_, p.b); }
     kt_pending_.clear();
     pool_put_stream(device_id_, stream_);
@@ -1518,7 +1524,7 @@
     } else {
       std::shared_ptr<void> keep;
       int64_t rows = 0;
-      if (pull_device_table(input, op.scan_fields, t.cols, t.has_valid, rows, keep)) {
+      if (pull_device_table(input, op.scan_fields, t.cols, t.has_valid, rows, keep, &op == root_source_ ? &root_spec_ : nullptr)) {
         t.rows = rows;
         t.owners.push_back(keep);
         std::vector<DeviceColumnView> c2;
@@ -1853,7 +1859,13 @@
     if (plan_.get() == root_source_) throw CometError("internal: bare join root");
     if (sink_ == SinkKind::AggGrouped) prepare_dict_keys(src);
     single_chunk_hint_ = true;
-    process_chunk(src.cols, src.has_valid, src.rows);
+    process_chunk(src.cols, src.has_valid, src.rows, &root_spec_);
+    if (root_spec_.voided) {
+      root_spec_.apply_checked(src.cols);
+      root_spec_.voided = false;
+      if (sink_ == SinkKind::AggGrouped) prepare_dict_keys(src);
+      process_chunk(src.cols, src.has_valid, src.rows);
+    }
     HIP_CHECK(hipStreamSynchronize(stream_));
     return;
   }
@@ -1867,7 +1879,7 @@
   if (!started_) {
     HIP_CHECK(hipSetDevice(device_id_));
     stream_ = pool_get_stream(device_id_);
-    err_flags_.ensure(kErrBytes);
+    err_flags_.ensure(kErrBytes + kUtf8RecBytes);
     HIP_CHECK(hipMemsetAsync(err_flags_.p, 0, kErrBytes, stream_));
     started_ = true;
   } else {
diff --git a/datafusion-comet_amd/csrc/exec.hpp b/datafusion-comet_amd/csrc/exec.hpp
--- a/datafusion-comet_amd/csrc/exec.hpp
+++ b/datafusion-comet_amd/csrc/exec.hpp
@@ -100,6 +100,16 @@
   int64_t kid_rows = 0;
 };
 
+struct Utf8Pending {
+  bool active = false;
+  bool voided = false;
+  std::vector<int> checked_len;
+  void apply_checked(std::vector<DeviceColumnView>& views) const;
+  size_t input = 0;
+  std::vector<size_t> col;
+  std::vector<CometUtf8Check> chk;
+};
+
 struct DevTable {
   int64_t rows = 0;
   std::vector<DType> types;
@@ -173,7 +183,7 @@
   void start();
   std::vector<std::vector<int>> fixed_len_hint_;
   Variant& variant_for(const std::vector<bool>& has_valid, const std::vector<int>& str_fixed_len);
-  void process_chunk(const std::vector<DeviceColumnView>& cols, const std::vector<bool>& has_valid, int64_t n);
+  void process_chunk(const std::vector<DeviceColumnView>& cols, const std::vector<bool>& has_valid, int64_t n, Utf8Pending* spec = nullptr);
   void finish_aggregate();
   void finish_grouped();
   DevTable grouped_to_device();
@@ -221,7 +231,11 @@
   bool pull_host_table(size_t input, const std::vector<DType>& types, int64_t max_rows, std::vector<DeviceColumnView>& views,
                        std::vector<bool>& has_valid, int64_t& rows);
   bool pull_device_table(size_t input, const std::vector<DType>& types, std::vector<DeviceColumnView>& views, std::vector<bool>& has_valid,
-                         int64_t& rows, std::shared_ptr<void>& keepalive);
+                         int64_t& rows, std::shared_ptr<void>& keepalive, Utf8Pending* spec = nullptr);
+  void verify_utf8_lengths(size_t input, int64_t rows, const std::vector<size_t>& scols, std::vector<CometUtf8Check>& chk, std::vector<DeviceColumnView>& views);
+  void run_utf8_check(const CometUtf8Check* cols, int n, uint32_t* rec);
+  uint32_t* utf8_records() { return (uint32_t*)((char*)err_flags_.p + kErrBytes); }
+  void launch_utf8_check_beside(const Utf8Pending& spec);
   void validate_input_schema(size_t input, const std::vector<DType>& types);
   void export_batch(HostBatch& b, ArrowArray** out_arrays, ArrowSchema** out_schemas, int n_out);
   void check_device_errors();
@@ -270,7 +284,6 @@
   std::vector<KtPending> kt_pending_;
   std::map<std::string, std::pair<double, int64_t>> kernel_times_;
   hipEvent_t aux_ev_[2] = {nullptr, nullptr};
-  int aux_n_ = 0;
   bool started_ = false, finished_ = false;
   std::vector<DType> in_types_;
   std::map<std::string, Variant> variants_;
@@ -330,8 +343,11 @@
     int64_t rows = 0;
     std::shared_ptr<void> keep;
     bool valid = false;
+    Utf8Pending spec;
   };
   DevPending dev_pending_;
+  Utf8Pending root_spec_;
+  bool utf8_predictable_plan() const { return sink_ == SinkKind::AggGrouped && (!has_join_ || (root_source_ && root_source_->kind == OpKind::Scan)); }
   bool dev_stream_done_ = false;
   int64_t dev_chunks_seen_ = 0;
   int64_t bytes_scanned_ = 0;
@@ -356,6 +372,9 @@
   long long packed_fix_scales(const PipelineDesc& d, int first = 0);
   bool adjust_fix_scales(const PipelineDesc& d, const uint64_t* aux, std::vector<int>& shift_right);
   DevBuf err_flags_;
+  DevBuf err_snapshot_;
+  hipStream_t check_stream_ = nullptr;
+  hipEvent_t check_fork_ev_ = nullptr;
   PinnedBuf result_host_;
   PinnedBuf small_host_;
   PinnedBuf export_host_;
diff --git a/datafusion-comet_amd/csrc/exec_input.cpp b/datafusion-comet_amd/csrc/exec_input.cpp
--- a/datafusion-comet_amd/csrc/exec_input.cpp
+++ b/datafusion-comet_amd/csrc/exec_input.cpp
@@ -1,4 +1,5 @@
 #include "exec_internal.hpp"
+#include "utf8_memo.hpp"
 #include <emmintrin.h>
 #include <mutex>
 #include <set>
@@ -524,15 +525,38 @@
   std::lock_guard<std::mutex> g(g_uniform_mu);
   return g_uniform_ok.count(UniformKey{off, rows, len, first}) != 0;
 }
+bool uniform_verdict_seen(const void* off, int64_t rows, int32_t len) {
+  std::lock_guard<std::mutex> g(g_uniform_mu);
+  auto it = g_uniform_ok.lower_bound(UniformKey{off, rows, len, INT32_MIN});
+  return it != g_uniform_ok.end() && it->off == off && it->rows == rows && it->len == len;
+}
 void remember_uniform_verdict(const void* off, int64_t rows, int32_t len, int32_t first) {
   std::lock_guard<std::mutex> g(g_uniform_mu);
   if (g_uniform_ok.size() >= 4096) g_uniform_ok.clear();
   g_uniform_ok.insert(UniformKey{off, rows, len, first});
 }
-}
+Utf8LengthMemo g_utf8_memo;
+}
+
+bool utf8_speculate() {
+  static const bool on = !(getenv("COMET_UTF8_SPECULATE") && atoi(getenv("COMET_UTF8_SPECULATE")) == 0);
+  return on;
+}
+bool utf8_check_stream() {
+  static const bool on = getenv("COMET_UTF8_CHECK_STREAM") ? atoi(getenv("COMET_UTF8_CHECK_STREAM")) != 0 : kUtf8CheckStreamDefault;
+  return on;
+}
+int utf8_check_blocks() {
+  static const int per_cu = getenv("COMET_UTF8_CHECK_BLOCKS_PER_CU") ? std::max(1, std::min(8, atoi(getenv("COMET_UTF8_CHECK_BLOCKS_PER_CU")))) : kUtf8CheckBlocksPerCuDefault;
+  return 256 * per_cu;
+}
+void Utf8Pending::apply_checked(std::vector<DeviceColumnView>& views) const {
+  for (size_t k = 0; k < col.size() && k < checked_len.size(); k++) views[col[k]].fixed_len = checked_len[k];
+}
+void utf8_memo_forget(uint64_t plan_hash, size_t input, size_t column) { g_utf8_memo.forget(plan_hash, input, column); }
 
 bool ExecutionContext::pull_device_table(size_t input, const std::vector<DType>& types, std::vector<DeviceColumnView>& views,
-                                         std::vector<bool>& has_valid, int64_t& rows, std::shared_ptr<void>& keepalive) {
+                                         std::vector<bool>& has_valid, int64_t& rows, std::shared_ptr<void>& keepalive, Utf8Pending* spec) {
   InputSource& in = inputs_[input];
   rows = 0;
   if (in.exhausted) return false;
@@ -579,78 +603,111 @@
   std::vector<size_t> scols;
   for (size_t c = 0; c < nc && rows > 0; c++)
     if (types[c].id == TypeId::String) scols.push_back(c);
-  if (!scols.empty() && scols.size() <= 16) {
-    small_host_.ensure(4096);
-    int32_t* ends = (int32_t*)small_host_.p;
+  if (!scols.empty() && scols.size() <= COMET_UTF8_MAX_COLS) {
+    std::vector<CometUtf8Check> chk(scols.size());
+    bool predictable = spec != nullptr && utf8_speculate() && utf8_predictable_plan() && scols.size() <= (size_t)kGuardMaxCols;
     for (size_t k = 0; k < scols.size(); k++) {
       const ArrowArray* col = da->array.children[scols[k]];
-      const int32_t* off = (const int32_t*)col->buffers[1] + col->offset;
-      HIP_CHECK(hipMemcpyAsync(ends + 2 * k, off, 4, hipMemcpyDeviceToHost, stream_));
-      HIP_CHECK(hipMemcpyAsync(ends + 2 * k + 1, off + rows, 4, hipMemcpyDeviceToHost, stream_));
-    }
-    HIP_CHECK(hipStreamSynchronize(stream_));
-    std::vector<int32_t> first(scols.size()), len(scols.size(), -1);
-    std::vector<bool> declared(scols.size(), false);
-    uint32_t* flags = (uint32_t*)err_flags_.p + (kErrBytes / 4 - 16);
-    HIP_CHECK(hipMemsetAsync(flags, 0, 64, stream_));
-    bool any = false;
-    if (!aux_ev_[0]) { aux_ev_[0] = pool_get_event(device_id_); aux_ev_[1] = pool_get_event(device_id_); }
-    HIP_CHECK(hipEventRecord(aux_ev_[0], stream_));
-    int aux_launched = 0;
-    for (size_t k = 0; k < scols.size(); k++) {
-      first[k] = ends[2 * k];
-      const int64_t total = (int64_t)ends[2 * k + 1] - ends[2 * k];
       const int hint = input < fixed_len_hint_.size() && scols[k] < fixed_len_hint_[input].size() ? fixed_len_hint_[input][scols[k]] : -1;
-      const ArrowArray* col = da->array.children[scols[k]];
-      const int32_t* off = (const int32_t*)col->buffers[1] + col->offset;
+      chk[k].offsets = (const int*)col->buffers[1];
+      chk[k].rows = rows;
+      chk[k].col_offset = col->offset;
+      chk[k].expect = hint;
+      chk[k].ends_only = 0;
+      int guess = -1;
+      predictable = predictable && hint < 0 && col->offset == 0 && g_utf8_memo.get(plan_hash_, input, scols[k], guess);
+      if (predictable) chk[k].expect = guess;
+    }
+    if (predictable) {
+      spec->active = true;
+      spec->input = input;
+      spec->col = scols;
+      spec->chk = chk;
+      for (size_t k = 0; k < scols.size(); k++) views[scols[k]].fixed_len = chk[k].expect;
+      return true;
+    }
+    for (size_t k = 0; k < scols.size(); k++) chk[k].expect = input < fixed_len_hint_.size() && scols[k] < fixed_len_hint_[input].size() ? fixed_len_hint_[input][scols[k]] : -1;
+    verify_utf8_lengths(input, rows, scols, chk, views);
+  }
+  return true;
+}
+
+void ExecutionContext::verify_utf8_lengths(size_t input, int64_t rows, const std::vector<size_t>& scols, std::vector<CometUtf8Check>& chk,
+                                           std::vector<DeviceColumnView>& views) {
+  const bool memo = utf8_predictable_plan();
+  std::vector<int> round(scols.size(), 0);
+  for (size_t k = 0; k < scols.size(); k++) {
+    views[scols[k]].fixed_len = -1;
+    chk[k].ends_only = chk[k].expect >= 0 && uniform_verdict_seen((const int32_t*)chk[k].offsets + chk[k].col_offset, rows, chk[k].expect) ? 1 : 0;
+  }
+  for (int r = 0; r < 2; r++) {
+    std::vector<CometUtf8Check> now;
+    std::vector<size_t> who;
+    for (size_t k = 0; k < scols.size(); k++)
+      if (round[k] == r) { now.push_back(chk[k]); who.push_back(k); }
+    if (now.empty()) break;
+    uint32_t rec[COMET_UTF8_MAX_COLS * COMET_UTF8_REC_WORDS];
+    run_utf8_check(now.data(), (int)now.size(), rec);
+    for (size_t j = 0; j < who.size(); j++) {
+      const size_t k = who[j], c = scols[k];
+      const uint32_t* q = rec + j * COMET_UTF8_REC_WORDS;
+      const int32_t first = (int32_t)q[1], last = (int32_t)q[2], len = (int32_t)q[3];
+      const int hint = chk[k].expect;
+      const int64_t col_offset = chk[k].col_offset;
+      round[k] = -1;
       if (hint >= 0) {
-        if (total != (int64_t)hint * rows)
-          throw CometError("device input column " + std::to_string(scols[k]) + " is declared comet:utf8_fixed_len=" + std::to_string(hint) + " but holds " +
-                           std::to_string(total) + " bytes in " + std::to_string(rows) + " rows");
-        if ((int64_t)first[k] != (int64_t)col->offset * hint) continue;
-        if (uniform_verdict_known(off, rows, hint, first[k])) {
-          views[scols[k]].fixed_len = hint;
+        if (q[0] & 2u)
+          throw CometError("device input column " + std::to_string(c) + " is declared comet:utf8_fixed_len=" + std::to_string(hint) + " but holds " +
+                           std::to_string((int64_t)last - first) + " bytes in " + std::to_string(rows) + " rows");
+        if ((int64_t)first != col_offset * hint) continue;
+        const int32_t* off = (const int32_t*)chk[k].offsets + col_offset;
+        if (now[j].ends_only) {
+          if (uniform_verdict_known(off, rows, hint, first)) views[c].fixed_len = hint;
+          else { chk[k].ends_only = 0; round[k] = r + 1; }
           continue;
         }
-        if (comet_launch_utf8_uniform(off, rows, hint, flags + k, stream_) != 0) continue;
-        aux_launched++;
-        len[k] = hint;
-        declared[k] = true;
-        any = true;
+        if (q[0] & 1u)
+          throw CometError("device input column " + std::to_string(c) + " is declared comet:utf8_fixed_len=" + std::to_string(hint) +
+                           " but its offsets are not " + std::to_string(hint) + " bytes apart (the byte total alone matches)");
+        remember_uniform_verdict(off, rows, hint, first);
+        views[c].fixed_len = hint;
         continue;
       }
-      if (total % rows != 0 || total / rows > 15 || total < 0) continue;
-      if (comet_launch_utf8_uniform(off, rows, (int32_t)(total / rows), flags + k, stream_) != 0) continue;
-      aux_launched++;
-      len[k] = (int32_t)(total / rows);
-      any = true;
-    }
-    if (any) {
-      HIP_CHECK(hipEventRecord(aux_ev_[1], stream_));
-      uint32_t f[16];
-      read_small(f, flags, 64);
-      float aux = 0;
-      if (hipEventElapsedTime(&aux, aux_ev_[0], aux_ev_[1]) == hipSuccess) { last_aux_ms += aux; last_aux_launches += aux_launched; }
-      HIP_CHECK(hipMemsetAsync(flags, 0, 64, stream_));
-      for (size_t k = 0; k < scols.size(); k++) {
-        if (len[k] < 0) continue;
-        const size_t c = scols[k];
-        const ArrowArray* col = da->array.children[c];
-        if (declared[k]) {
-          if (f[k] != 0)
-            throw CometError("device input column " + std::to_string(c) + " is declared comet:utf8_fixed_len=" + std::to_string(len[k]) +
-                             " but its offsets are not " + std::to_string(len[k]) + " bytes apart (the byte total alone matches)");
-          remember_uniform_verdict((const int32_t*)col->buffers[1] + col->offset, rows, len[k], first[k]);
-          views[c].fixed_len = len[k];
-          continue;
-        }
-        if (f[k] != 0) continue;
-        if ((int64_t)first[k] != (int64_t)col->offset * len[k]) continue;
-        views[c].fixed_len = len[k];
-      }
-    }
-  }
-  return true;
+      if (q[0] != 0 || (int64_t)first != col_offset * len) {
+        if (memo) g_utf8_memo.forget(plan_hash_, input, c);
+        continue;
+      }
+      views[c].fixed_len = len;
+      if (memo && col_offset == 0) g_utf8_memo.put(plan_hash_, input, c, len);
+    }
+  }
+}
+
+void ExecutionContext::launch_utf8_check_beside(const Utf8Pending& spec) {
+  const bool beside = utf8_check_stream();
+  if (!aux_ev_[0]) { aux_ev_[0] = pool_get_event(device_id_); aux_ev_[1] = pool_get_event(device_id_); }
+  hipStream_t st = stream_;
+  if (beside) {
+    if (!check_stream_) check_stream_ = pool_get_stream(device_id_);
+    st = check_stream_;
+    HIP_CHECK(hipStreamWaitEvent(st, check_fork_ev_, 0));
+  }
+  HIP_CHECK(hipEventRecord(aux_ev_[0], st));
+  if (comet_launch_utf8_check(spec.chk.data(), (int)spec.chk.size(), utf8_records(), beside ? utf8_check_blocks() : 0, st) != 0)
+    throw CometError("Utf8 length check: launch failed");
+  HIP_CHECK(hipEventRecord(aux_ev_[1], st));
+}
+
+void ExecutionContext::run_utf8_check(const CometUtf8Check* cols, int n, uint32_t* rec) {
+  const size_t bytes = (size_t)n * COMET_UTF8_REC_WORDS * 4;
+  HIP_CHECK(hipMemsetAsync(utf8_records(), 0, bytes, stream_));
+  if (!aux_ev_[0]) { aux_ev_[0] = pool_get_event(device_id_); aux_ev_[1] = pool_get_event(device_id_); }
+  HIP_CHECK(hipEventRecord(aux_ev_[0], stream_));
+  if (comet_launch_utf8_check(cols, n, utf8_records(), 0, stream_) != 0) throw CometError("Utf8 length check: launch failed");
+  HIP_CHECK(hipEventRecord(aux_ev_[1], stream_));
+  read_small(rec, utf8_records(), bytes);
+  float aux = 0;
+  if (hipEventElapsedTime(&aux, aux_ev_[0], aux_ev_[1]) == hipSuccess) { last_aux_ms += aux; last_aux_launches += 1; }
 }
 
 bool ExecutionContext::pull_device_batch() {
@@ -659,17 +716,21 @@
     cur = std::move(dev_pending_);
     dev_pending_ = DevPending();
   } else {
-    if (dev_stream_done_ || !pull_device_table(0, in_types_, cur.views, cur.has_valid, cur.rows, cur.keep)) return false;
+    if (dev_stream_done_ || !pull_device_table(0, in_types_, cur.views, cur.has_valid, cur.rows, cur.keep, &cur.spec)) return false;
   }
   if (sink_ == SinkKind::AggGrouped && dev_chunks_seen_ == 0 && !dev_stream_done_) {
-    dev_pending_.valid = pull_device_table(0, in_types_, dev_pending_.views, dev_pending_.has_valid, dev_pending_.rows, dev_pending_.keep);
+    dev_pending_.valid = pull_device_table(0, in_types_, dev_pending_.views, dev_pending_.has_valid, dev_pending_.rows, dev_pending_.keep, &dev_pending_.spec);
     if (!dev_pending_.valid) dev_stream_done_ = true;
     single_chunk_hint_ = !dev_pending_.valid;
   } else {
     single_chunk_hint_ = false;
   }
   dev_chunks_seen_++;
-  process_chunk(cur.views, cur.has_valid, cur.rows);
+  process_chunk(cur.views, cur.has_valid, cur.rows, &cur.spec);
+  if (cur.spec.voided) {
+    cur.spec.apply_checked(cur.views);
+    process_chunk(cur.views, cur.has_valid, cur.rows);
+  }
   HIP_CHECK(hipStreamSynchronize(stream_));
   return true;
 }
diff --git a/datafusion-comet_amd/csrc/exec_internal.hpp b/datafusion-comet_amd/csrc/exec_internal.hpp
--- a/datafusion-comet_amd/csrc/exec_internal.hpp
+++ b/datafusion-comet_amd/csrc/exec_internal.hpp
@@ -114,8 +114,15 @@
                                         void* stream);
 extern "C" int comet_launch_fix_rescale(uint64_t* base, int64_t count, int64_t stride_words, int32_t word_off, int32_t shift, void* stream);
 extern "C" int comet_launch_utf8_uniform(const int32_t* offsets, int64_t n, int32_t L, uint32_t* flag, void* stream);
+extern "C" int comet_launch_utf8_check(const CometUtf8Check* cols, int ncols, uint32_t* rec, int max_blocks, void* stream);
 
 namespace comet {
+bool utf8_speculate();
+bool utf8_check_stream();
+int utf8_check_blocks();
+void utf8_memo_forget(uint64_t plan_hash, size_t input, size_t column);
+constexpr bool kUtf8CheckStreamDefault = true;
+constexpr int kUtf8CheckBlocksPerCuDefault = 2;
 HostColumn download_column(const DeviceColumnView& v, const DType& t, bool has_valid, int64_t rows, hipStream_t st);
 
 namespace detail {
diff --git a/datafusion-comet_amd/csrc/exec_pipeline.cpp b/datafusion-comet_amd/csrc/exec_pipeline.cpp
--- a/datafusion-comet_amd/csrc/exec_pipeline.cpp
+++ b/datafusion-comet_amd/csrc/exec_pipeline.cpp
@@ -1,12 +1,23 @@
 #include "exec_internal.hpp"
 
 namespace comet {
-void ExecutionContext::process_chunk(const std::vector<DeviceColumnView>& cols, const std::vector<bool>& has_valid, int64_t n) {
+void ExecutionContext::process_chunk(const std::vector<DeviceColumnView>& cols, const std::vector<bool>& has_valid, int64_t n, Utf8Pending* spec) {
   if (n == 0) return;
   std::vector<int> fixed_lens(cols.size(), -1);
   for (size_t i = 0; i < cols.size(); i++) fixed_lens[i] = cols[i].fixed_len;
   Variant& v = variant_for(has_valid, fixed_lens);
   const PipelineDesc& d = v.desc;
+  bool speculative = spec && spec->active;
+  if (speculative && (d.sink != SinkKind::AggGrouped || d.merges_states)) {
+    std::vector<DeviceColumnView> checked = cols;
+    for (CometUtf8Check& c : spec->chk) c.expect = -1;
+    verify_utf8_lengths(spec->input, n, spec->col, spec->chk, checked);
+    spec->active = false;
+    spec->voided = true;
+    spec->checked_len.clear();
+    for (size_t c : spec->col) spec->checked_len.push_back(checked[c].fixed_len);
+    return;
+  }
   if (d.max_rows_exact && input_rows + n > d.max_rows_exact)
     throw CometError("decimal or integer sum over more rows than its static no-overflow proof allows (" + std::to_string(d.max_rows_exact) + ")");
   CometKParams prm;
@@ -60,7 +71,7 @@
     if (agg_variant_ && (agg_variant_->desc.NW != d.NW || agg_variant_->desc.NK != d.NK))
       throw CometError("internal: group slot layout differs between variants");
     agg_variant_ = &v;
-    if (try_partitioned_merge(v, prm, n)) return;
+    if (!speculative && try_partitioned_merge(v, prm, n)) return;
     const size_t slot_bytes = 8 + 8 * (size_t)(d.NK + d.NW);
     auto alloc_table = [&](DevBuf& buf, int64_t cap) {
       buf.ensure((size_t)cap * slot_bytes);
@@ -93,13 +104,64 @@
       prm.out[0] = group_table_.p;
       prm.iarg[0] = group_cap_;
       prm.iarg[kFixScaleArg] = packed_fix_scales(d), prm.iarg[kFixScaleArg2] = packed_fix_scales(d, 4);
-      timed_begin();
-      launch(v, "k_gagg", grid, prm);
-      timed_end();
-      uint64_t head[2 + (kErrBytes - 16) / 8];
+      uint64_t head[2 + (kErrBytes - 16) / 8 + kUtf8RecBytes / 8];
       uint32_t flags[4];
-      read_small(head, err_flags_.p, d.fix_sums.empty() ? 16 : sizeof head);
-      memcpy(flags, head, 16);
+      if (speculative) {
+        uint64_t guard = (uint64_t)spec->col.size();
+        for (size_t k = 0; k < spec->col.size(); k++) guard |= (uint64_t)((uint32_t)spec->col[k] | ((uint32_t)spec->chk[k].expect << 5)) << (3 + 9 * k);
+        prm.iarg[kGuardArg] = (long long)guard;
+        const size_t rec_bytes = spec->col.size() * COMET_UTF8_REC_WORDS * 4;
+        err_snapshot_.ensure(kErrBytes);
+        HIP_CHECK(hipMemcpyAsync(err_snapshot_.p, err_flags_.p, kErrBytes, hipMemcpyDeviceToDevice, stream_));
+        HIP_CHECK(hipMemsetAsync(utf8_records(), 0, rec_bytes, stream_));
+        const bool beside = utf8_check_stream();
+        if (beside) {
+          if (!check_fork_ev_) check_fork_ev_ = pool_get_event(device_id_);
+          HIP_CHECK(hipEventRecord(check_fork_ev_, stream_));
+        } else {
+          launch_utf8_check_beside(*spec);
+        }
+        timed_begin();
+        launch(v, "k_gagg", grid, prm);
+        timed_end();
+        if (beside) {
+          launch_utf8_check_beside(*spec);
+          HIP_CHECK(hipStreamWaitEvent(stream_, aux_ev_[1], 0));
+        }
+        read_small(head, err_flags_.p, kErrBytes + rec_bytes);
+        float aux = 0;
+        if (hipEventElapsedTime(&aux, aux_ev_[0], aux_ev_[1]) == hipSuccess) { last_aux_ms += aux; last_aux_launches += 1; }
+        memcpy(flags, head, 16);
+        const uint32_t* rec = (const uint32_t*)head + kErrBytes / 4;
+        bool miss = (flags[0] & kErrGuardBit) != 0;
+        for (size_t k = 0; k < spec->col.size(); k++) miss = miss || rec[k * COMET_UTF8_REC_WORDS] != 0;
+        if (miss) {
+          if (clear) HIP_CHECK(hipMemsetAsync(group_table_.p, 0, (size_t)group_cap_ * slot_bytes, stream_));
+          else HIP_CHECK(hipMemcpyAsync(group_table_.p, group_backup_.p, (size_t)group_cap_ * slot_bytes, hipMemcpyDeviceToDevice, stream_));
+          HIP_CHECK(hipMemcpyAsync(err_flags_.p, err_snapshot_.p, kErrBytes, hipMemcpyDeviceToDevice, stream_));
+          spec->checked_len.clear();
+          for (size_t k = 0; k < spec->col.size(); k++) {
+            const uint32_t* q = rec + k * COMET_UTF8_REC_WORDS;
+            const bool good = q[0] == 0 && (int32_t)q[3] == spec->chk[k].expect && (int64_t)(int32_t)q[1] == spec->chk[k].col_offset * spec->chk[k].expect;
+            spec->checked_len.push_back(good ? spec->chk[k].expect : -1);
+            if (!good) utf8_memo_forget(plan_hash_, spec->input, spec->col[k]);
+          }
+          spec->active = false;
+          spec->voided = true;
+          if (!has_join_) input_rows -= n;
+          agg_rows_seen_ -= n;
+          return;
+        }
+        speculative = false;
+        spec->active = false;
+        prm.iarg[kGuardArg] = 0;
+      } else {
+        timed_begin();
+        launch(v, "k_gagg", grid, prm);
+        timed_end();
+        read_small(head, err_flags_.p, d.fix_sums.empty() ? 16 : (size_t)kErrBytes);
+        memcpy(flags, head, 16);
+      }
       uint64_t groups_now;
       memcpy(&groups_now, &flags[2], 8);
       const bool full = (flags[0] & 32u) != 0;
diff --git a/datafusion-comet_amd/csrc/kernels_static.hip b/datafusion-comet_amd/csrc/kernels_static.hip
--- a/datafusion-comet_amd/csrc/kernels_static.hip
+++ b/datafusion-comet_amd/csrc/kernels_static.hip
@@ -33,33 +33,76 @@
   for (i64 i = (i64)blockIdx.x * 256 + threadIdx.x; i < n; i += (i64)gridDim.x * 256) out[i] = pmod(hashes[i], np);
 }
 
-__global__ __launch_bounds__(256) void utf8_uniform_kernel(const i32* off, i64 n, i32 L, u32* flag) {
+constexpr int kUtf8Unroll = 8;
+constexpr int kUtf8MaxCols = COMET_UTF8_MAX_COLS;
+constexpr int kUtf8MaxBlocks = 256 * 8;
+struct Utf8CheckCol {
+  const i32* off;
+  i64 rows;
+  i64 col_offset;
+  i32 expect;
+  i32 ends_only;
+};
+struct Utf8CheckArgs { Utf8CheckCol c[kUtf8MaxCols]; };
+typedef int utf8_v4i __attribute__((ext_vector_type(4)));
+
+__global__ __launch_bounds__(256) void utf8_uniform_kernel(const Utf8CheckArgs args, u32* rec, int rec_words) {
+  const Utf8CheckCol c = args.c[blockIdx.y];
+  const i64 n = c.rows;
+  if (n <= 0) return;
+  const COMET_GLOBAL i32* off = (const COMET_GLOBAL i32*)c.off + c.col_offset;
+  u32* r = rec + (size_t)blockIdx.y * rec_words;
+  const i32 o0 = off[0], o_n = off[n];
+  const i64 bytes = (i64)o_n - (i64)o0;
+  i32 L = c.expect;
+  bool ends_bad;
+  if (L >= 0) {
+    ends_bad = bytes != (i64)L * n;
+  } else {
+    ends_bad = bytes < 0 || bytes % n != 0 || bytes / n > 15;
+    L = ends_bad ? -1 : (i32)(bytes / n);
+  }
+  if (blockIdx.x == 0 && threadIdx.x == 0) {
+    if (rec_words >= 4) { r[1] = (u32)o0; r[2] = (u32)o_n; r[3] = (u32)L; }
+    if (ends_bad) atomicOr(r, 2u);
+  }
+  if (ends_bad || c.ends_only) return;
   bool bad = false;
-  const i32 o0 = off[0];
   const i64 total = n + 1;
-  i64 head = 0;
-  while (head < total && ((((uintptr_t)(off + head)) & 15) != 0)) head++;
-  const int4* v4 = (const int4*)(off + head);
+  i64 head = (i64)(((16 - ((uintptr_t)off & 15)) & 15) >> 2);
+  if (head > total) head = total;
+  const COMET_GLOBAL utf8_v4i* v4 = (const COMET_GLOBAL utf8_v4i*)(off + head);
   const i64 ngroups = (total - head) / 4;
-  constexpr int U = 4;
-  for (i64 g0 = ((i64)blockIdx.x * 256 + threadIdx.x) * U; g0 < ngroups; g0 += (i64)gridDim.x * 256 * U) {
-    int4 v[U];
-#pragma unroll
-    for (int u = 0; u < U; u++) v[u] = g0 + u < ngroups ? v4[g0 + u] : make_int4(0, 0, 0, 0);
-#pragma unroll
-    for (int u = 0; u < U; u++) {
-      if (g0 + u < ngroups) {
-        const i64 i = head + 4 * (g0 + u);
-        const i32 e = o0 + (i32)(i * L);
-        bad |= (v[u].x != e) | (v[u].y != e + L) | (v[u].z != e + 2 * L) | (v[u].w != e + 3 * L);
+  constexpr int U = kUtf8Unroll;
+  const u32 uL = (u32)L, u0 = (u32)o0;
+  const int lane = threadIdx.x & 63;
+  const i64 wave = (i64)blockIdx.x * (256 / 64) + (threadIdx.x >> 6), waves = (i64)gridDim.x * (256 / 64);
+  for (i64 g0 = wave * (U * 64); g0 < ngroups; g0 += waves * (U * 64)) {
+    if (g0 + U * 64 <= ngroups) {
+      utf8_v4i v[U];
+#pragma unroll
+      for (int u = 0; u < U; u++) v[u] = __builtin_nontemporal_load(v4 + g0 + u * 64 + lane);
+#pragma unroll
+      for (int u = 0; u < U; u++) {
+        const u32 e = u0 + (u32)(head + 4 * (g0 + u * 64 + lane)) * uL;
+        bad |= ((u32)v[u].x != e) | ((u32)v[u].y != e + uL) | ((u32)v[u].z != e + 2 * uL) | ((u32)v[u].w != e + 3 * uL);
+      }
+    } else {
+      for (int u = 0; u < U; u++) {
+        const i64 g = g0 + u * 64 + lane;
+        if (g < ngroups) {
+          const utf8_v4i v = __builtin_nontemporal_load(v4 + g);
+          const u32 e = u0 + (u32)(head + 4 * g) * uL;
+          bad |= ((u32)v.x != e) | ((u32)v.y != e + uL) | ((u32)v.z != e + 2 * uL) | ((u32)v.w != e + 3 * uL);
+        }
       }
     }
   }
   if (blockIdx.x == 0) {
-    for (i64 i = threadIdx.x; i < head; i += 256) bad |= off[i] != o0 + (i32)(i * L);
-    for (i64 i = head + ngroups * 4 + threadIdx.x; i < total; i += 256) bad |= off[i] != o0 + (i32)(i * L);
-  }
-  if (__any(bad) && lane_id() == 0) atomicOr(flag, 1u);
+    for (i64 i = threadIdx.x; i < head; i += 256) bad |= (u32)off[i] != u0 + (u32)i * uL;
+    for (i64 i = head + ngroups * 4 + threadIdx.x; i < total; i += 256) bad |= (u32)off[i] != u0 + (u32)i * uL;
+  }
+  if (__any(bad) && lane_id() == 0) atomicOr(r, 1u);
 }
 
 __device__ __forceinline__ i64 dict_index(const void* idx, int iw, i64 i) {
@@ -185,9 +228,39 @@
   return hipGetLastError() == hipSuccess ? 0 : -1;
 }
 
+static int utf8_check_grid(i64 rows, int ncols, int max_blocks) {
+  const i64 per_block = (i64)256 * kUtf8Unroll * 4;
+  i64 g = (rows + 1 + per_block - 1) / per_block;
+  const int nc = ncols > 0 ? ncols : 1;
+  i64 cap = kUtf8MaxBlocks / nc;
+  if (max_blocks > 0 && max_blocks / nc < cap) cap = max_blocks / nc;
+  if (cap < 1) cap = 1;
+  return (int)(g < 1 ? 1 : (g > cap ? cap : g));
+}
+extern "C" int comet_launch_utf8_check(const CometUtf8Check* cols, int ncols, uint32_t* rec, int max_blocks, void* stream) {
+  if (ncols <= 0) return 0;
+  if (ncols > kUtf8MaxCols) return -1;
+  Utf8CheckArgs a = {};
+  i64 rows = 0;
+  for (int k = 0; k < ncols; k++) {
+    a.c[k].off = cols[k].offsets;
+    a.c[k].rows = cols[k].rows;
+    a.c[k].col_offset = cols[k].col_offset;
+    a.c[k].expect = cols[k].expect;
+    a.c[k].ends_only = cols[k].ends_only;
+    if (cols[k].rows > rows && !cols[k].ends_only) rows = cols[k].rows;
+  }
+  hipLaunchKernelGGL(utf8_uniform_kernel, dim3((unsigned)utf8_check_grid(rows, ncols, max_blocks), (unsigned)ncols), dim3(256), 0, (hipStream_t)stream, a, rec,
+                     COMET_UTF8_REC_WORDS);
+  return hipGetLastError() == hipSuccess ? 0 : -1;
+}
 extern "C" int comet_launch_utf8_uniform(const int32_t* offsets, int64_t n, int32_t L, uint32_t* flag, void* stream) {
   if (n <= 0) return 0;
-  hipLaunchKernelGGL(utf8_uniform_kernel, grid_for(n), 256, 0, (hipStream_t)stream, offsets, (i64)n, L, flag);
+  Utf8CheckArgs a = {};
+  a.c[0].off = offsets;
+  a.c[0].rows = n;
+  a.c[0].expect = L;
+  hipLaunchKernelGGL(utf8_uniform_kernel, dim3((unsigned)utf8_check_grid(n, 1, 0)), dim3(256), 0, (hipStream_t)stream, a, flag, 1);
   return hipGetLastError() == hipSuccess ? 0 : -1;
 }
 
diff --git a/datafusion-comet_amd/csrc/kparams.h b/datafusion-comet_amd/csrc/kparams.h
--- a/datafusion-comet_amd/csrc/kparams.h
+++ b/datafusion-comet_amd/csrc/kparams.h
@@ -23,4 +23,14 @@
   void* out[COMET_MAX_OUT];
 } CometKParams;
 
+#define COMET_UTF8_REC_WORDS 4
+#define COMET_UTF8_MAX_COLS 16
+typedef struct CometUtf8Check {
+  const int* offsets;
+  long long rows;
+  long long col_offset;
+  int expect;
+  int ends_only;
+} CometUtf8Check;
+
 #endif
diff --git a/datafusion-comet_amd/csrc/utf8_memo.hpp b/datafusion-comet_amd/csrc/utf8_memo.hpp
--- /dev/null
+++ b/datafusion-comet_amd/csrc/utf8_memo.hpp
@@ -0,0 +1,45 @@
+#ifndef COMET_UTF8_MEMO_HPP
+#define COMET_UTF8_MEMO_HPP
+
+#include <cstddef>
+#include <cstdint>
+#include <map>
+#include <mutex>
+#include <tuple>
+
+namespace comet {
+
+class Utf8LengthMemo {
+ public:
+  explicit Utf8LengthMemo(size_t max_entries = 4096) : max_(max_entries) {}
+  bool get(uint64_t plan_hash, size_t input, size_t column, int& len) const {
+    std::lock_guard<std::mutex> g(mu_);
+    auto it = map_.find(Key{plan_hash, input, column});
+    if (it == map_.end()) return false;
+    len = it->second;
+    return true;
+  }
+  void put(uint64_t plan_hash, size_t input, size_t column, int len) {
+    std::lock_guard<std::mutex> g(mu_);
+    if (map_.size() >= max_ && map_.find(Key{plan_hash, input, column}) == map_.end()) map_.clear();
+    map_[Key{plan_hash, input, column}] = len;
+  }
+  void forget(uint64_t plan_hash, size_t input, size_t column) {
+    std::lock_guard<std::mutex> g(mu_);
+    map_.erase(Key{plan_hash, input, column});
+  }
+  size_t size() const {
+    std::lock_guard<std::mutex> g(mu_);
+    return map_.size();
+  }
+
+ private:
+  typedef std::tuple<uint64_t, size_t, size_t> Key;
+  const size_t max_;
+  mutable std::mutex mu_;
+  std::map<Key, int> map_;
+};
+
+}
+
+#endif
```

After: 74.25 billion rows/s, median of 6. 3.9% higher.
